# uw-x/AcousticSwarms-Speech

Hardware: AMD Instinct MI355X
Metric: TDoA candidates/sec (shift+normalise+spot forward+energies) (higher is better)
Workload: dtype f32 via f16x3 split-operand MFMA (fp32 accumulate); 1 GPU; configs[2] scene: 5-speaker reverberant mixture (image sources), 7 mics, T=48000 samples (BASELINE's '3 s @ 16 kHz' sample count; the reference pipeline and this scene generator run at 48 kHz, where it is a 1 s clip -- the reference-native 3 s is extras.T144000), fine-stage (Strict=1) candidate batch of one mixture, FULL spot net 47.27 M params, seeded random weights; internal_batch=256, parallelism=candidate-shard x1

## Files before the change

### acousticswarms-speech_amd/csrc/asw_common.cpp

```cpp
#include "asw_common.h"

#include <cmath>
#include <cstdlib>

namespace asw {
char* err_buf() {
  static thread_local char buf[512] = {0};
  return buf;
}
int set_error(int code, const char* fmt, ...) {
  va_list ap;
  va_start(ap, fmt);
  vsnprintf(err_buf(), 512, fmt, ap);
  va_end(ap);
  return code;
}
int SmemAttr::ensure(const void* kern, size_t want) {
  int dev = 0;
  ASW_HIP(hipGetDevice(&dev));
  if (dev < 0 || dev >= kMaxDev) return set_error(ASW_ERR_ARG, "device ordinal %d out of range", dev);
  if (bytes[dev] >= want) return ASW_OK;
  ASW_HIP(hipFuncSetAttribute(kern, hipFuncAttributeMaxDynamicSharedMemorySize, (int)want));
  bytes[dev] = want;
  return ASW_OK;
}
}

extern "C" const char* asw_last_error(void) { return asw::err_buf(); }
extern "C" int asw_abi_version(void) { return 3; }

extern "C" int asw_split_weights_f16(const float* w, size_t n, uint16_t* hi, uint16_t* lo, int32_t* w_shift) {
  ASW_CHECK_ARG(w && hi && lo && w_shift, "split_weights: null pointer");
  float mx = 0.f;
  for (size_t i = 0; i < n; ++i) { const float a = w[i] < 0 ? -w[i] : w[i]; if (a > mx || a != a) mx = a; }
  ASW_CHECK_ARG(mx == mx && mx < 3.0e38f, "split_weights: non-finite weight");
  int shift = 0;
  if (mx > 0.f) {
    int e;
    (void)frexpf(mx, &e);
    shift = 11 - e;
    if (shift > 24) shift = 24;
    if (shift < -24) shift = -24;
  }
  const float sc = ldexpf(1.0f, shift);
  for (size_t i = 0; i < n; ++i) {
    float c = w[i] * sc;
    if (c > 65504.f) c = 65504.f;
    if (c < -65504.f) c = -65504.f;
    const _Float16 h = (_Float16)c;
    const _Float16 l = (_Float16)(c - (float)h);
    memcpy(hi + i, &h, 2);
    memcpy(lo + i, &l, 2);
  }
  *w_shift = shift;
  return ASW_OK;
}

extern "C" int asw_pack_fragments_f16(const float* Wt, int N, int K, uint16_t* hi, uint16_t* lo, int32_t* w_shift) {
  ASW_CHECK_ARG(Wt && hi && lo && w_shift, "pack_fragments: null pointer");
  ASW_CHECK_ARG(N > 0 && K > 0 && N % 32 == 0 && K % 16 == 0, "pack_fragments: N %% 32, K %% 16 required (N=%d K=%d)", N, K);
  const size_t n = (size_t)N * K;
  uint16_t* th = new uint16_t[2 * n];
  uint16_t* tl = th + n;
  int rc = asw_split_weights_f16(Wt, n, th, tl, w_shift);
  if (rc == ASW_OK) {
    const int NT = N / 32;
    for (int ks = 0; ks < K / 16; ++ks)
      for (int nt = 0; nt < NT; ++nt)
        for (int l = 0; l < 64; ++l) {
          const size_t src = (size_t)(nt * 32 + (l & 31)) * K + ks * 16 + 8 * (l >> 5);
          const size_t dst = (((size_t)ks * NT + nt) * 64 + l) * 8;
          memcpy(hi + dst, th + src, 16);
          memcpy(lo + dst, tl + src, 16);
        }
  }
  delete[] th;
  return rc;
}

namespace asw {
bool residue_feed_on() {
  static const bool off = getenv("ASW_NO_RESIDUE_FEED") != nullptr;
  return !off;
}
}

extern "C" int asw_residue_schedule(int taps, int stride, int dil, int pad, int Cin, int BK, int BM, int m0, int has_skip,
                                    asw_residue_stage* out, int cap, int* n_stages, int* max_shift) {
  ASW_CHECK_ARG(n_stages != nullptr && cap >= 0 && (out != nullptr || cap == 0), "residue_schedule: null pointer");
  ASW_CHECK_ARG(taps > 0 && stride > 0 && dil > 0 && Cin > 0 && BK > 0 && BM > 0, "residue_schedule: bad dims");
  *n_stages = 0;
  if (max_shift) *max_shift = 0;
  if (!asw::residue_feed_applies(taps, stride, dil, Cin, BK, has_skip != 0)) return ASW_OK;
  const asw::ResidueFeed rf{taps, stride, Cin / BK};
  ASW_CHECK_ARG(rf.ntaps(0) <= ASW_RESIDUE_MAX_TAPS, "residue_schedule: %d taps on one image, at most %d", rf.ntaps(0),
                ASW_RESIDUE_MAX_TAPS);
  *n_stages = rf.stages();
  if (max_shift) *max_shift = rf.shifts(0);
  for (int s = 0; s < rf.stages() && s < cap; ++s) {
    asw_residue_stage& d = out[s];
    memset(&d, 0, sizeof d);
    d.residue = s / rf.cpb;
    d.chunk = s - d.residue * rf.cpb;
    d.rows = BM + rf.shifts(d.residue);
    d.first_row = m0 * stride - pad + d.residue;
    d.ntaps = rf.ntaps(d.residue);
    for (int q = 0; q < d.ntaps; ++q) {
      d.tap[q] = rf.tap(d.residue, q);
      d.shift[q] = q;
      d.kstep[q] = rf.kstep(d.tap[q], d.chunk, BK / 16);
    }
  }
  return ASW_OK;
}

#include <map>
#include <mutex>
#include <vector>
namespace asw {
namespace {
struct Rec { std::string name; double work, bytes; hipEvent_t e0, e1; };
std::mutex g_mu;
bool g_on = false;
bool g_detail = false;
std::vector<Rec> g_recs;
std::vector<hipEvent_t> g_pool;
hipEvent_t take_event() {
  if (!g_pool.empty()) { hipEvent_t e = g_pool.back(); g_pool.pop_back(); return e; }
  hipEvent_t e = nullptr;
  (void)hipEventCreate(&e);
  return e;
}
}

std::string prof_name(const char* base, int bm, int bn, int bk, bool ln, bool stats) {
  char b[96];
  snprintf(b, sizeof b, "%s<%d,%d,%d,%s>", base, bm, bn, bk, ln ? "ln" : stats ? "stats" : "plain");
  return b;
}
bool prof_detail() { return g_detail; }
ProfScope::ProfScope(hipStream_t s, const std::string& name, double work, double bytes) : slot(-1), stream(s) {
  if (!g_on) return;
  std::lock_guard<std::mutex> lk(g_mu);
  Rec r{name, work, bytes, take_event(), take_event()};
  (void)hipEventRecord(r.e0, s);
  g_recs.push_back(r);
  slot = (int)g_recs.size() - 1;
}
ProfScope::~ProfScope() {
  if (slot < 0) return;
  std::lock_guard<std::mutex> lk(g_mu);
  if (slot < (int)g_recs.size()) (void)hipEventRecord(g_recs[slot].e1, stream);
}
}

extern "C" int asw_profile_enable(int on) {
  std::lock_guard<std::mutex> lk(asw::g_mu);
  for (auto& r : asw::g_recs) { asw::g_pool.push_back(r.e0); asw::g_pool.push_back(r.e1); }
  asw::g_recs.clear();
  asw::g_on = on != 0;
  asw::g_detail = on == 2;
  return ASW_OK;
}

extern "C" int asw_profile_report(char* buf, size_t cap) {
  if (!buf || cap < 64) return asw::set_error(ASW_ERR_ARG, "profile_report: buffer too small");
  std::lock_guard<std::mutex> lk(asw::g_mu);
  struct Agg { long n = 0; double ms = 0, work = 0, bytes = 0; };
  std::map<std::string, Agg> agg;
  for (auto& r : asw::g_recs) {
    if (hipEventSynchronize(r.e1) != hipSuccess) continue;
    float ms = 0.f;
    if (hipEventElapsedTime(&ms, r.e0, r.e1) != hipSuccess) continue;
    Agg& a = agg[r.name];
    a.n += 1; a.ms += ms; a.work += r.work; a.bytes += r.bytes;
  }
  size_t off = 0;
  off += snprintf(buf + off, cap - off, "{");
  bool first = true;
  for (auto& kv : agg) {
    if (off + 256 >= cap) break;
    off += snprintf(buf + off, cap - off, "%s\"%s\":{\"launches\":%ld,\"ms\":%.6f,\"work\":%.6e,\"bytes\":%.6e}", first ? "" : ",",
                    kv.first.c_str(), kv.second.n, kv.second.ms, kv.second.work, kv.second.bytes);
    first = false;
  }
  snprintf(buf + off, cap - off, "}");
  return ASW_OK;
}
```

### acousticswarms-speech_amd/csrc/model_common.h

```cpp
#pragma once
#include <cstdlib>
#include <iterator>
#include <map>
#include <memory>
#include <string>
#include <vector>

#include "asw_common.h"

namespace asw_model {

struct DevBuf {
  float* p = nullptr;
  size_t n = 0;
  DevBuf() = default;
  DevBuf(const DevBuf&) = delete;
  DevBuf& operator=(const DevBuf&) = delete;
  DevBuf(DevBuf&& o) noexcept : p(o.p), n(o.n) { o.p = nullptr; o.n = 0; }
  ~DevBuf() { if (p) (void)hipFree(p); }
  int upload(const std::vector<float>& h) {
    if (p) { (void)hipFree(p); p = nullptr; }
    n = h.size();
    if (hipMalloc(&p, n * sizeof(float)) != hipSuccess) return asw::set_error(ASW_ERR_NOMEM, "hipMalloc(%zu floats)", n);
    ASW_HIP(hipMemcpy(p, h.data(), n * sizeof(float), hipMemcpyHostToDevice));
    return ASW_OK;
  }
};

struct WBuf {
  DevBuf f32;
  uint16_t* hi = nullptr;
  uint16_t* lo = nullptr;
  int32_t shift = 0;
  WBuf() = default;
  WBuf(const WBuf&) = delete;
  WBuf& operator=(const WBuf&) = delete;
  WBuf(WBuf&& o) noexcept : f32(std::move(o.f32)), hi(o.hi), lo(o.lo), shift(o.shift), fhi(o.fhi), flo(o.flo) {
    o.hi = o.lo = o.fhi = o.flo = nullptr;
  }
  ~WBuf() {
    if (hi) (void)hipFree(hi);
    if (lo) (void)hipFree(lo);
    if (fhi) (void)hipFree(fhi);
    if (flo) (void)hipFree(flo);
  }
  int upload_gemm(const std::vector<float>& h, int N, int K) {
    int rc = upload(h);
    if (rc) return rc;
    if (N % 32 == 0 && K % 16 == 0 && (size_t)N * K == h.size()) return upload_frags(h, N, K);
    return ASW_OK;
  }
  int upload(const std::vector<float>& h) {
    int rc = f32.upload(h);
    if (rc) return rc;
    std::vector<uint16_t> vh(h.size()), vl(h.size());
    if ((rc = asw_split_weights_f16(h.data(), h.size(), vh.data(), vl.data(), &shift))) return rc;
    if (hi) { (void)hipFree(hi); hi = nullptr; }
    if (lo) { (void)hipFree(lo); lo = nullptr; }
    if (hipMalloc(&hi, h.size() * 2) != hipSuccess || hipMalloc(&lo, h.size() * 2) != hipSuccess)
      return asw::set_error(ASW_ERR_NOMEM, "hipMalloc(%zu halves)", h.size());
    ASW_HIP(hipMemcpy(hi, vh.data(), h.size() * 2, hipMemcpyHostToDevice));
    ASW_HIP(hipMemcpy(lo, vl.data(), h.size() * 2, hipMemcpyHostToDevice));
    return ASW_OK;
  }
  uint16_t* fhi = nullptr;
  uint16_t* flo = nullptr;
  int upload_frags(const std::vector<float>& h, int N, int K) {
    std::vector<uint16_t> vh(h.size()), vl(h.size());
    int32_t sh = 0;
    int rc = asw_pack_fragments_f16(h.data(), N, K, vh.data(), vl.data(), &sh);
    if (rc) return rc;
    if (sh != shift) return asw::set_error(ASW_ERR_STATE, "fragment pack: inconsistent weight shift");
    if (fhi) { (void)hipFree(fhi); fhi = nullptr; }
    if (flo) { (void)hipFree(flo); flo = nullptr; }
    if (hipMalloc(&fhi, h.size() * 2) != hipSuccess || hipMalloc(&flo, h.size() * 2) != hipSuccess)
      return asw::set_error(ASW_ERR_NOMEM, "hipMalloc(%zu halves)", h.size());
    ASW_HIP(hipMemcpy(fhi, vh.data(), h.size() * 2, hipMemcpyHostToDevice));
    ASW_HIP(hipMemcpy(flo, vl.data(), h.size() * 2, hipMemcpyHostToDevice));
    return ASW_OK;
  }
  void bind(asw_convgemm_args& a, int precision) const {
    a.Wt = f32.p; a.Wt_hi = hi; a.Wt_lo = lo; a.w_shift = shift; a.precision = precision;
    a.Wf_hi = fhi; a.Wf_lo = flo;
  }
};

struct ResLayer { WBuf wt; DevBuf bias, g, b; int dil = 1; };

inline std::vector<float> pack_conv(const std::vector<float>& w, int N, int Cin, int K, const float* in_gate) {
  std::vector<float> o((size_t)N * Cin * K);
  for (int n = 0; n < N; ++n)
    for (int c = 0; c < Cin; ++c)
      for (int k = 0; k < K; ++k)
        o[((size_t)n * K + k) * Cin + c] = w[((size_t)n * Cin + c) * K + k] * (in_gate ? in_gate[c] : 1.f);
  return o;
}


inline int pack_res_layers(const std::map<std::string, std::vector<float>>& raw, const std::string& p, int ch, int K,
                           int n_layers, int dil_factor, std::vector<ResLayer>& out) {
  out.clear();
  out.resize(n_layers);
  int dil = 1;
  for (int j = 0; j < n_layers; ++j) {
    const std::string q = p + ".res.seq." + std::to_string(j);
    int rc;
    {
      const std::vector<float> packed = pack_conv(raw.at(q + ".conv.weight"), ch, ch, K, nullptr);
      if ((rc = out[j].wt.upload(packed))) return rc;
      if (ch % 32 == 0 && (ch * K) % 16 == 0 && (rc = out[j].wt.upload_frags(packed, ch, ch * K))) return rc;
    }
    if ((rc = out[j].bias.upload(raw.at(q + ".conv.bias")))) return rc;
    if ((rc = out[j].g.upload(raw.at(q + ".norm.weight")))) return rc;
    if ((rc = out[j].b.upload(raw.at(q + ".norm.bias")))) return rc;
    out[j].dil = dil;
    dil *= dil_factor;
  }
  return ASW_OK;
}

struct Arena {
  char* base;
  size_t off = 0, cap;
  bool dry;
  Arena(char* b, size_t c, bool d) : base(b), cap(c), dry(d) {}
  template <typename T>
  T* take(size_t n) {
    off = (off + 255) & ~(size_t)255;
    T* p = reinterpret_cast<T*>(base + off);
    off += n * sizeof(T);
    return p;
  }
};


struct GluSrc { const float* raw; const float* mr; const float* gamma; const float* beta; float* side_out = nullptr; };

inline bool glu_on_load_ok(const std::vector<ResLayer>& res, int prec, int ch) {
  static const int max_c = getenv("ASW_GLU_ON_LOAD_MAX_C") ? atoi(getenv("ASW_GLU_ON_LOAD_MAX_C")) : 512;
  return prec >= 1 && (ch == 64 || ch == 128 || ch == 256 || ch == 512) && ch <= max_c && !res.empty() &&
         res[0].dil == 1 && res[0].wt.fhi && res[0].wt.flo;
}

inline bool resstack_ok(const std::vector<ResLayer>& res, int prec, int ch, int K) {
  static const bool off = getenv("ASW_NO_RESSTACK") != nullptr;
  if (off || prec < 1 || ch != 64 || K % 2 == 0 || K < 3 || K > 15) return false;
  for (const ResLayer& r : res)
    if (!r.wt.fhi || !r.wt.flo) return false;
  return true;
}

inline size_t resstack_fuse_count(const std::vector<ResLayer>& res, size_t j, int K) {
  static const bool nofuse = getenv("ASW_RESSTACK_NOFUSE") != nullptr;
  size_t n = 1;
  int halo = 0;
  while (!nofuse && j + n < res.size() && n < 3) {
    const int pad = res[j + n].dil * (K - 1) / 2;
    if (halo + pad > 64) break;
    halo += pad;
    ++n;
  }
  return n;
}

struct SrcFeed { const void* hi; const void* lo; const WBuf* comp; const WBuf* pre; };

inline int run_res(const std::vector<ResLayer>& res, int prec, int B, int T, int ch, int K, float* x, float* p, float* q,
            float** final_out, hipStream_t s, const GluSrc* glu = nullptr, const SrcFeed* feed = nullptr) {
  const float* in = glu ? glu->raw : x;
  float* outb = p;
  if (feed && !(resstack_ok(res, prec, ch, K) && prec == 1 && resstack_fuse_count(res, 0, K) == 2))
    return asw::set_error(ASW_ERR_STATE, "run_res: the source-fed form needs the fused f16x3 pair");
  if (resstack_ok(res, prec, ch, K)) {
    size_t j = 0;
    while (j < res.size()) {
      const size_t n = resstack_fuse_count(res, j, K);
      asw_resstack_args a = {};
      a.x = ((glu || feed) && j == 0) ? nullptr : in;
      a.out = outb;
      a.B = B; a.T = T; a.C = ch; a.taps = K; a.n_layers = (int)n; a.precision = prec; a.ln_eps = 1e-5f;
      for (size_t i = 0; i < n; ++i) {
        const ResLayer& r = res[j + i];
        a.layer[i].Wf_hi = r.wt.fhi; a.layer[i].Wf_lo = r.wt.flo; a.layer[i].w_shift = r.wt.shift;
        a.layer[i].bias = r.bias.p; a.layer[i].ln_gamma = r.g.p; a.layer[i].ln_beta = r.b.p; a.layer[i].dil = r.dil;
      }
      if (glu && j == 0) {
        a.glu_raw = glu->raw; a.glu_mr = glu->mr; a.glu_gamma = glu->gamma; a.glu_beta = glu->beta; a.glu_out = glu->side_out;
      }
      if (feed && j == 0) {
        a.src_hi = feed->hi; a.src_lo = feed->lo;
        a.layer[0].Wf_hi = feed->comp->fhi; a.layer[0].Wf_lo = feed->comp->flo; a.layer[0].w_shift = feed->comp->shift;
        a.pre_hi = feed->pre->fhi; a.pre_lo = feed->pre->flo; a.pre_shift = feed->pre->shift;
      }
      int rc = asw_resstack64_f16x3(&a, s);
      if (rc) return rc;
      in = outb;
      outb = (outb == p) ? q : p;
      j += n;
    }
    *final_out = const_cast<float*>(in);
    return ASW_OK;
  }
  for (size_t j = 0; j < res.size(); ++j) {
    asw_convgemm_args a = {};
    a.A = in; res[j].wt.bind(a, prec); a.bias = res[j].bias.p; a.resid = in;
    if (glu && j == 0) {
      a.glu_raw = glu->raw; a.glu_mr = glu->mr; a.glu_gamma = glu->gamma; a.glu_beta = glu->beta; a.glu_out = glu->side_out;
    }
    a.ln_gamma = res[j].g.p; a.ln_beta = res[j].b.p; a.out = outb;
    a.B = B; a.M_out = T; a.N = ch; a.Cin = ch; a.taps = K; a.stride = 1; a.dil = res[j].dil;
    a.pad = (res[j].dil * (K - 1) + 1) / 2;
    a.a_row_stride = ch; a.a_batch_stride = (int64_t)T * ch; a.a_len = (int64_t)T * ch;
    a.relu = 1; a.ln_eps = 1e-5f;
    int rc = asw_convgemm_f32(&a, s);
    if (rc) return rc;
    in = outb;
    outb = (outb == p) ? q : p;
  }
  *final_out = const_cast<float*>(in);
  return ASW_OK;
}

inline int linear(const float* A, const WBuf& W, int prec, const float* bias, int rows, int N, int K, int relu, const float* resid,
           const float* g, const float* b, float* out, hipStream_t s) {
  asw_convgemm_args a = {};
  a.A = A; W.bind(a, prec); a.bias = bias; a.resid = resid; a.ln_gamma = g; a.ln_beta = b; a.out = out;
  a.B = 1; a.M_out = rows; a.N = N; a.Cin = K; a.taps = 1; a.stride = 1; a.dil = 1; a.pad = 0;
  a.a_row_stride = K; a.a_batch_stride = (int64_t)rows * K; a.a_len = (int64_t)rows * K;
  a.relu = relu; a.ln_eps = 1e-5f;
  if (g && N >= 1024 && N % 256 == 0 && N <= 2048) {
    a.resid = nullptr; a.ln_gamma = nullptr; a.ln_beta = nullptr;
    int rc = asw_convgemm_f32(&a, s);
    if (rc) return rc;
    return asw_add_layernorm(out, resid, g, b, rows, N, 1e-5f, out, s);
  }
  return asw_convgemm_f32(&a, s);
}

inline void pack_conv_transpose(const std::vector<float>& w, const std::vector<float>& b, int Cin, int N, int S,
                                const float* out_gate, std::vector<float>& wt, std::vector<float>& bb) {
  wt.assign((size_t)S * N * Cin, 0.f);
  bb.assign((size_t)S * N, 0.f);
  for (int r = 0; r < S; ++r)
    for (int n = 0; n < N; ++n) {
      bb[(size_t)r * N + n] = out_gate ? b[n] * out_gate[n] : b[n];
      for (int c = 0; c < Cin; ++c) {
        const float v = w[((size_t)c * N + n) * S + r];
        wt[((size_t)r * N + n) * Cin + c] = out_gate ? v * out_gate[n] : v;
      }
    }
}


#define UP(buf, vec) if ((rc = (buf).upload(vec))) return rc

struct TrunkCfg {
  int n_mics, kernel_size, depth, stride_list[8], channels, growth, encoder_channels, encoder_kernel_size,
      encoder_stride, residual_layers, residual_dilation_factor, ffw_dim;
  template <class Cfg>
  static TrunkCfg of(const Cfg& c) {
    TrunkCfg t = {c.n_mics, c.kernel_size, c.depth, {}, c.channels, c.growth, c.encoder_channels,
                  c.encoder_kernel_size, c.encoder_stride, c.residual_layers, c.residual_dilation_factor, c.ffw_dim};
    for (int i = 0; i < 8; ++i) t.stride_list[i] = c.stride_list[i];
    return t;
  }
};

inline int check_trunk_config(const TrunkCfg& c, const char* who, const char* odd) {
  ASW_CHECK_ARG(c.depth >= 1 && c.depth <= 8, "%s: depth %d", who, c.depth);
  ASW_CHECK_ARG(c.n_mics >= 1 && c.n_mics <= 32, "%s: n_mics %d", who, c.n_mics);
  ASW_CHECK_ARG(c.channels % 64 == 0, "%s: channels=%d must be a multiple of 64 for the MFMA tiles", who, c.channels);
  ASW_CHECK_ARG(c.growth >= 1 && c.residual_layers >= 1, "%s: bad config", who);
  ASW_CHECK_ARG(c.kernel_size % 2 == 1, "%s: %s", who, odd);
  ASW_CHECK_ARG(c.encoder_channels % 128 == 0, "%s: encoder_channels must be a multiple of 128", who);
  ASW_CHECK_ARG(c.encoder_stride % 4 == 0 && c.encoder_kernel_size / 2 == c.encoder_stride && c.encoder_kernel_size <= 64,
                "%s: encoder kernel/stride %d/%d unsupported (the reference's trim [9:-8] assumes 33/16)", who,
                c.encoder_kernel_size, c.encoder_stride);
  ASW_CHECK_ARG(c.ffw_dim % 128 == 0, "%s: ffw_dim must be a multiple of 128", who);
  return ASW_OK;
}

struct EncBlock { std::vector<ResLayer> res; DevBuf bias, gn_g, gn_b; };
struct DecBlock { std::vector<ResLayer> res; DevBuf gn_g, gn_b; };
struct GatedConvs { std::vector<WBuf> down_wt, up_wt; std::vector<DevBuf> up_bias; };
struct Tap { const float* p; size_t numel; };
using ParamList = std::vector<std::pair<std::string, size_t>>;

struct TrunkPlan {
  int B, T, Tp, F, RL;
  std::vector<int> Tl;
  float *mean, *stdv, *refn;
  uint16_t *src_hi = nullptr, *src_lo = nullptr;
  std::vector<float*> X, Pb, Qb, raw_dn, raw_up, st_dn, st_up, mr_dn, mr_up;
  float *Y, *D, *ywave;
};

struct Trunk {
  TrunkCfg tc;
  std::map<std::string, std::vector<float>> raw;
  std::map<std::string, Tap> taps;
  bool finalized = false;
  int device = 0;
  int precision = 0;
  bool exact_raw = false;
  bool fuse_mask = true;
  bool want_src = false;
  bool src_stack = true;

  std::vector<int> enc_cin, enc_cout;
  std::vector<int> dec_cin, dec_cout, dec_stride;
  int stride_product = 1;

  DevBuf pre_w, pre_b;
  WBuf src_wt, src_pre;
  std::vector<EncBlock> enc;
  std::vector<DecBlock> dec;
  WBuf byp_wt, mask_wt, dec_wt;
  WBuf byp_wt48;
  DevBuf byp_b, mask_b;
  float out_bias = 0.f;
  int byp_k = 0;

  const std::vector<float>& P(const std::string& k) const { return raw.at(k); }

  enum class Src { Normed, Raw };
  int site(Src a) const { return !exact_raw ? precision : a == Src::Raw ? 0 : 3; }

  int init_shape(const TrunkCfg& c, const char* who) {
    tc = c;
    ASW_HIP(hipGetDevice(&device));
    int cin = c.channels, ch = c.channels;
    for (int i = 0; i < c.depth; ++i) {
      ASW_CHECK_ARG(c.stride_list[i] >= 1, "%s: stride", who);
      enc_cin.push_back(cin);
      enc_cout.push_back(ch);
      stride_product *= c.stride_list[i];
      cin = ch;
      ch *= c.growth;
    }
    dec_cin.assign(enc_cout.rbegin(), enc_cout.rend());
    dec_cout.assign(enc_cin.rbegin(), enc_cin.rend());
    dec_stride.assign(std::make_reverse_iterator(c.stride_list + c.depth), std::make_reverse_iterator(c.stride_list));
    return ASW_OK;
  }
  int check_level_widths(const char* who) const {
    for (int w : enc_cin) ASW_CHECK_ARG(w <= 512 && (w & (w - 1)) == 0, "%s: level width %d must be a power of two <= 512", who, w);
    return ASW_OK;
  }

  ParamList trunk_params() const {
    ParamList v;
    const size_t K = tc.kernel_size;
    v.push_back({"preproc.weight", (size_t)tc.channels * tc.n_mics});
    v.push_back({"preproc.bias", (size_t)tc.channels});
    auto res = [&](const std::string& p, size_t ch) {
      for (int j = 0; j < tc.residual_layers; ++j) {
        const std::string q = p + ".res.seq." + std::to_string(j);
        v.push_back({q + ".conv.weight", ch * ch * K});
        v.push_back({q + ".conv.bias", ch});
        v.push_back({q + ".norm.weight", ch});
        v.push_back({q + ".norm.bias", ch});
      }
    };
    for (int i = 0; i < tc.depth; ++i) {
      const std::string p = "encoder.module_list." + std::to_string(i);
      const size_t ci = enc_cin[i], co = enc_cout[i];
      res(p, ci);
      v.push_back({p + ".conv1.weight", 2 * co * ci * K});
      v.push_back({p + ".conv1.bias", 2 * co});
      v.push_back({p + ".norm1.weight", 2 * co});
      v.push_back({p + ".norm1.bias", 2 * co});
    }
    for (int i = 0; i < tc.depth; ++i) {
      const std::string p = "decoder.module_list." + std::to_string(i);
      const size_t ci = dec_cin[i], co = dec_cout[i], s = dec_stride[i];
      v.push_back({p + ".upsample.conv.weight", ci * 2 * co * s});
      v.push_back({p + ".upsample.conv.bias", 2 * co});
      v.push_back({p + ".norm1.weight", 2 * co});
      v.push_back({p + ".norm1.bias", 2 * co});
      res(p, co);
    }
    const size_t E = tc.encoder_channels, EK = tc.encoder_kernel_size;
    v.push_back({"reference_bypass.weight", E * EK});
    v.push_back({"reference_bypass.bias", E});
    v.push_back({"mask_encoder.weight", E * tc.channels * EK});
    v.push_back({"mask_encoder.bias", E});
    v.push_back({"output_decoder.weight", E * EK});
    v.push_back({"output_decoder.bias", 1});
    return v;
  }

  int finalize_trunk(const char* who, const ParamList& want) {
    {
      int dev = -1;
      ASW_HIP(hipGetDevice(&dev));
      if (dev != device)
        return asw::set_error(ASW_ERR_STATE, "%s: model was created on HIP device %d, current device is %d", who, device, dev);
    }
    for (const auto& kv : want) {
      auto it = raw.find(kv.first);
      if (it == raw.end()) return asw::set_error(ASW_ERR_STATE, "state dict is missing key %s", kv.first.c_str());
      if (it->second.size() != kv.second)
        return asw::set_error(ASW_ERR_ARG, "%s: %zu elements, expected %zu", kv.first.c_str(), it->second.size(), kv.second);
    }
    if (raw.size() != want.size())
      return asw::set_error(ASW_ERR_ARG, "state dict has %zu unexpected keys", raw.size() - want.size());
    int rc;
    const int K = tc.kernel_size, RL = tc.residual_layers, RD = tc.residual_dilation_factor;
    UP(pre_w, P("preproc.weight"));
    UP(pre_b, P("preproc.bias"));
    enc.clear(); enc.resize(tc.depth);
    dec.clear(); dec.resize(tc.depth);
    for (int i = 0; i < tc.depth; ++i) {
      const std::string p = "encoder.module_list." + std::to_string(i);
      if ((rc = pack_res_layers(raw, p, enc_cin[i], K, RL, RD, enc[i].res))) return rc;
      UP(enc[i].bias, P(p + ".conv1.bias"));
      UP(enc[i].gn_g, P(p + ".norm1.weight"));
      UP(enc[i].gn_b, P(p + ".norm1.bias"));
    }
    if (want_src && tc.channels == 64 && tc.n_mics <= 7 && K <= 7 && enc[0].res[0].wt.fhi) {
      std::vector<float> pre16((size_t)64 * 16), comp((size_t)64 * 64);
      if ((rc = asw_compose_source_weights(P("encoder.module_list.0.res.seq.0.conv.weight").data(), P("preproc.weight").data(),
                                           P("preproc.bias").data(), tc.n_mics, K, comp.data(), pre16.data())))
        return rc;
      if ((rc = src_wt.upload_gemm(comp, 64, 64))) return rc;
      if ((rc = src_pre.upload_gemm(pre16, 64, 16))) return rc;
    }
    for (int i = 0; i < tc.depth; ++i) {
      const std::string p = "decoder.module_list." + std::to_string(i);
      if ((rc = pack_res_layers(raw, p, dec_cout[i], K, RL, RD, dec[i].res))) return rc;
      UP(dec[i].gn_g, P(p + ".norm1.weight"));
      UP(dec[i].gn_b, P(p + ".norm1.bias"));
    }
    const int E = tc.encoder_channels, EK = tc.encoder_kernel_size;
    byp_k = ((EK + 31) / 32) * 32;
    {
      const std::vector<float>& w = P("reference_bypass.weight");
      std::vector<float> wt((size_t)E * byp_k, 0.f);
      for (int n = 0; n < E; ++n)
        for (int k = 0; k < EK; ++k) wt[(size_t)n * byp_k + k] = w[(size_t)n * EK + k];
      UP(byp_wt, wt);
      UP(byp_b, P("reference_bypass.bias"));
      if (E % 32 == 0 && EK <= 48) {
        std::vector<float> w48((size_t)E * 48, 0.f);
        for (int n = 0; n < E; ++n)
          for (int k = 0; k < EK; ++k) w48[(size_t)n * 48 + k] = w[(size_t)n * EK + k];
        if ((rc = byp_wt48.upload_gemm(w48, E, 48))) return rc;
      }
    }
    if ((rc = mask_wt.upload_gemm(pack_conv(P("mask_encoder.weight"), E, tc.channels, EK, nullptr), E, tc.channels * EK))) return rc;
    UP(mask_b, P("mask_encoder.bias"));
    {
      const std::vector<float>& w = P("output_decoder.weight");
      std::vector<float> wt((size_t)64 * E, 0.f);
      for (int j = 0; j < EK; ++j)
        for (int e = 0; e < E; ++e) wt[(size_t)j * E + e] = w[(size_t)e * EK + j];
      if ((rc = dec_wt.upload_gemm(wt, 64, E))) return rc;
      out_bias = P("output_decoder.bias")[0];
    }
    return ASW_OK;
  }

  template <class Gate>
  int pack_gated(GatedConvs& o, Gate gate) const {
    const int K = tc.kernel_size;
    int rc;
    o.down_wt.clear(); o.down_wt.resize(tc.depth);
    o.up_wt.clear(); o.up_wt.resize(tc.depth);
    o.up_bias.clear(); o.up_bias.resize(tc.depth);
    for (int i = 0; i < tc.depth; ++i) {
      const std::string p = "encoder.module_list." + std::to_string(i);
      const std::vector<float> g = gate(p);
      const int n = 2 * enc_cout[i], ci = enc_cin[i];
      if ((rc = o.down_wt[i].upload_gemm(pack_conv(P(p + ".conv1.weight"), n, ci, K, g.empty() ? nullptr : g.data()), n, ci * K)))
        return rc;
    }
    for (int j = 0; j < tc.depth; ++j) {
      const std::string p = "decoder.module_list." + std::to_string(j);
      const std::vector<float> g = gate(p);
      const int ci = dec_cin[j], co2 = 2 * dec_cout[j], s = dec_stride[j];
      std::vector<float> wt, bb;
      pack_conv_transpose(P(p + ".upsample.conv.weight"), P(p + ".upsample.conv.bias"), ci, co2, s,
                          g.empty() ? nullptr : g.data(), wt, bb);
      if ((rc = o.up_wt[j].upload_gemm(wt, s * co2, ci))) return rc;
      UP(o.up_bias[j], bb);
    }
    return ASW_OK;
  }

  bool fused_mask_path() const {
    return fuse_mask && precision >= 1 && tc.encoder_channels % 256 == 0 && tc.channels % 32 == 0 &&
           tc.encoder_kernel_size <= 48 && tc.encoder_stride % 4 == 0 && byp_wt48.fhi && dec_wt.fhi && mask_wt.fhi;
  }
  bool src_path() const {
    return want_src && src_stack && precision == 1 && src_wt.fhi && src_pre.fhi && !enc.empty() &&
           resstack_ok(enc[0].res, precision, enc_cin[0], tc.kernel_size) &&
           resstack_fuse_count(enc[0].res, 0, tc.kernel_size) == 2;
  }
  void layout_levels(int B, int T, Arena& a, TrunkPlan& pl) const {
    const int depth = tc.depth, EK = tc.encoder_kernel_size, ES = tc.encoder_stride;
    pl.B = B; pl.T = T;
    pl.Tp = ((T - 1) / stride_product + 1) * stride_product;
    pl.F = (pl.Tp + 2 * (EK / 2) - EK) / ES + 1;
    pl.RL = ((EK / 2 + pl.Tp + byp_k + 64) + 3) & ~3;
    pl.Tl.assign(depth + 1, pl.Tp);
    for (int i = 0; i < depth; ++i) pl.Tl[i + 1] = pl.Tl[i] / tc.stride_list[i];
    pl.mean = a.take<float>(B);
    pl.stdv = a.take<float>(B);
    pl.refn = a.take<float>((size_t)B * pl.RL);
    if (want_src) {
      pl.src_hi = a.take<uint16_t>((size_t)B * pl.Tp * 8);
      pl.src_lo = a.take<uint16_t>((size_t)B * pl.Tp * 8);
    }
    pl.X.resize(depth + 1); pl.Pb.resize(depth); pl.Qb.resize(depth);
    pl.raw_dn.resize(depth); pl.raw_up.resize(depth); pl.st_dn.resize(depth); pl.st_up.resize(depth);
    pl.mr_up.resize(depth); pl.mr_dn.resize(depth);
    for (int i = 0; i <= depth; ++i) {
      const int ch = i == 0 ? tc.channels : enc_cout[i - 1];
      pl.X[i] = a.take<float>((size_t)B * pl.Tl[i] * ch);
    }
    for (int i = 0; i < depth; ++i) {
      const size_t n = (size_t)B * pl.Tl[i] * enc_cin[i];
      pl.Pb[i] = a.take<float>(n);
      pl.Qb[i] = a.take<float>(n);
      pl.raw_dn[i] = a.take<float>((size_t)B * pl.Tl[i + 1] * 2 * enc_cout[i]);
      pl.st_dn[i] = a.take<float>((size_t)B * 4 * asw_convgemm_stats_tiles(pl.Tl[i + 1], 2 * enc_cout[i]));
      pl.mr_dn[i] = a.take<float>((size_t)B * 4);
    }
    for (int j = 0; j < depth; ++j) {
      const int lvl = depth - j;
      const int s = dec_stride[j], co2 = 2 * dec_cout[j];
      pl.raw_up[j] = a.take<float>((size_t)B * pl.Tl[lvl] * s * co2);
      pl.st_up[j] = a.take<float>((size_t)B * 4 * asw_convgemm_stats_tiles(pl.Tl[lvl], s * co2));
      pl.mr_up[j] = a.take<float>((size_t)B * 4);
    }
  }
  void layout_mask(Arena& a, TrunkPlan& pl) const {
    const int E = tc.encoder_channels;
    const bool fused = fused_mask_path();
    pl.Y = fused ? nullptr : a.take<float>((size_t)pl.B * pl.F * E);
    pl.D = a.take<float>((size_t)(fused ? E / 256 : 1) * pl.B * pl.F * 64);
    pl.ywave = a.take<float>((size_t)pl.B * pl.T);
  }

  int encode(TrunkPlan& pl, const GatedConvs& g, hipStream_t s, bool src0 = false) {
    const int B = pl.B, K = tc.kernel_size;
    taps.clear();
    if (!src0) taps["preproc"] = {pl.X[0], (size_t)B * pl.Tl[0] * tc.channels};
    int rc;
    GluSrc src = {};
    const SrcFeed feed = {pl.src_hi, pl.src_lo, &src_wt, &src_pre};
    bool glu = false;
    for (int i = 0; i < tc.depth; ++i) {
      float* r = nullptr;
      if ((rc = run_res(enc[i].res, precision, B, pl.Tl[i], enc_cin[i], K, pl.X[i], pl.Pb[i], pl.Qb[i], &r, s,
                        glu ? &src : nullptr, (src0 && i == 0) ? &feed : nullptr)))
        return rc;
      asw_convgemm_args a = {};
      a.A = r; g.down_wt[i].bind(a, precision); a.bias = enc[i].bias.p; a.out = pl.raw_dn[i]; a.stats = pl.st_dn[i];
      a.B = B; a.M_out = pl.Tl[i + 1]; a.N = 2 * enc_cout[i]; a.Cin = enc_cin[i]; a.taps = K;
      a.stride = tc.stride_list[i]; a.dil = 1; a.pad = K / 2;
      a.a_row_stride = a.Cin; a.a_batch_stride = (int64_t)pl.Tl[i] * a.Cin; a.a_len = a.a_batch_stride;
      a.chan_mod = a.N;
      if ((rc = asw_convgemm_f32(&a, s))) return rc;
      glu = fuse_mask && i + 1 < tc.depth && glu_on_load_ok(enc[i + 1].res, precision, enc_cout[i]);
      const int tiles = asw_convgemm_stats_tiles(a.M_out, a.N);
      if (glu) {
        if ((rc = asw_gn_finalize(pl.st_dn[i], tiles, B, pl.Tl[i + 1], enc_cout[i], 1e-5f, pl.mr_dn[i], s))) return rc;
        src = {pl.raw_dn[i], pl.mr_dn[i], enc[i].gn_g.p, enc[i].gn_b.p, pl.X[i + 1]};
      } else if ((rc = asw_gn_glu(pl.raw_dn[i], pl.st_dn[i], tiles, enc[i].gn_g.p, enc[i].gn_b.p, B, pl.Tl[i + 1],
                                  enc_cout[i], 1e-5f, pl.X[i + 1], s))) {
        return rc;
      }
      taps["enc" + std::to_string(i)] = {pl.X[i + 1], (size_t)B * pl.Tl[i + 1] * enc_cout[i]};
    }
    return ASW_OK;
  }

  int decode(TrunkPlan& pl, const GatedConvs& g, const float*& x, hipStream_t s) {
    const int B = pl.B, K = tc.kernel_size;
    int rc;
    for (int j = 0; j < tc.depth; ++j) {
      const int lvl = tc.depth - j, ci = dec_cin[j], co = dec_cout[j], st = dec_stride[j];
      asw_convgemm_args a = {};
      a.A = x; a.A2 = pl.X[lvl]; g.up_wt[j].bind(a, precision); a.bias = g.up_bias[j].p; a.out = pl.raw_up[j];
      a.stats = pl.st_up[j];
      a.B = B; a.M_out = pl.Tl[lvl]; a.N = st * 2 * co; a.Cin = ci; a.taps = 1; a.stride = 1; a.dil = 1; a.pad = 0;
      a.a_row_stride = ci; a.a_batch_stride = (int64_t)pl.Tl[lvl] * ci; a.a_len = a.a_batch_stride;
      a.chan_mod = 2 * co;
      if ((rc = asw_convgemm_f32(&a, s))) return rc;
      const int To = pl.Tl[lvl] * st;
      const int tiles = asw_convgemm_stats_tiles(a.M_out, a.N);
      float* gb = pl.Qb[lvl - 1];
      float* r = nullptr;
      if (fuse_mask && glu_on_load_ok(dec[j].res, precision, co)) {
        if ((rc = asw_gn_finalize(pl.st_up[j], tiles, B, To, co, 1e-5f, pl.mr_up[j], s))) return rc;
        const GluSrc src = {pl.raw_up[j], pl.mr_up[j], dec[j].gn_g.p, dec[j].gn_b.p, co > 64 ? gb : nullptr};
        if ((rc = run_res(dec[j].res, precision, B, To, co, K, gb, pl.Pb[lvl - 1], gb, &r, s, &src))) return rc;
      } else {
        if ((rc = asw_gn_glu(pl.raw_up[j], pl.st_up[j], tiles, dec[j].gn_g.p, dec[j].gn_b.p, B, To, co, 1e-5f, gb, s)))
          return rc;
        if ((rc = run_res(dec[j].res, precision, B, To, co, K, gb, pl.Pb[lvl - 1], gb, &r, s))) return rc;
      }
      x = r;
      taps["dec" + std::to_string(j)] = {x, (size_t)B * To * co};
    }
    return ASW_OK;
  }

  int mask_path(TrunkPlan& pl, const float* x, const float* mean, const float* stdv, float* out_wave, hipStream_t s) {
    const int B = pl.B, C = tc.channels, E = tc.encoder_channels, EK = tc.encoder_kernel_size, ES = tc.encoder_stride;
    int rc;
    asw_convgemm_args me = {};
    me.A = x; mask_wt.bind(me, site(Src::Normed)); me.bias = mask_b.p;
    me.B = B; me.M_out = pl.F; me.N = E; me.Cin = C; me.taps = EK; me.stride = ES; me.dil = 1; me.pad = EK / 2;
    me.a_row_stride = C; me.a_batch_stride = (int64_t)pl.Tp * C; me.a_len = me.a_batch_stride;
    if (fused_mask_path()) {
      asw_maskpath_args f = {};
      f.enc = me;
      f.ref = pl.refn; f.ref_batch_stride = pl.RL; f.ref_len = pl.RL; f.ref_hop = ES;
      f.byp_k = 48; f.byp_taps = EK; f.byp_shift = byp_wt48.shift; f.byp_hi = byp_wt48.fhi; f.byp_lo = byp_wt48.flo;
      f.byp_bias = byp_b.p;
      f.dec_hi = dec_wt.fhi; f.dec_lo = dec_wt.flo; f.dec_shift = dec_wt.shift; f.dec_taps = EK;
      f.taps = pl.D;
      f.enc.precision = precision;
      if ((rc = exact_raw ? asw_mask_path_f16x3_scaled(&f, s) : asw_mask_path_f16x3(&f, s))) return rc;
      return asw_overlap_add_parts(pl.D, E / 256, B, pl.F, 64, EK, EK / 2, pl.T, 9, 8, out_bias, mean, stdv, out_wave, s);
    }
    {
      asw_convgemm_args a = {};
      a.A = pl.refn; byp_wt.bind(a, site(Src::Normed)); a.bias = byp_b.p; a.out = pl.Y;
      a.B = B; a.M_out = pl.F; a.N = E; a.Cin = byp_k; a.taps = 1; a.stride = 1; a.dil = 1; a.pad = 0;
      a.a_row_stride = ES; a.a_batch_stride = pl.RL; a.a_len = pl.RL; a.relu = 1;
      if ((rc = asw_convgemm_f32(&a, s))) return rc;
    }
    me.mul = pl.Y; me.out = pl.Y; me.relu = 1;
    if ((rc = asw_convgemm_f32(&me, s))) return rc;
    taps["latent"] = {pl.Y, (size_t)B * pl.F * E};
    {
      asw_convgemm_args a = {};
      a.A = pl.Y; dec_wt.bind(a, site(Src::Raw)); a.out = pl.D;
      a.B = B; a.M_out = pl.F; a.N = 64; a.Cin = E; a.taps = 1; a.stride = 1; a.dil = 1; a.pad = 0;
      a.a_row_stride = E; a.a_batch_stride = (int64_t)pl.F * E; a.a_len = a.a_batch_stride;
      if ((rc = asw_convgemm_f32(&a, s))) return rc;
    }
    return asw_overlap_add_unnorm(pl.D, B, pl.F, 64, EK, EK / 2, pl.T, 9, 8, out_bias, mean, stdv, out_wave, s);
  }
};

struct PostNormLayer { WBuf w_in, w_out, w1, w2; DevBuf b_in, b_out, b1, b2, n1g, n1b, n2g, n2b; };
struct PostNormBufs { float *qkv, *ctx, *x1, *ff; };

template <class Attention>
int run_post_norm(const Trunk& m, const PostNormLayer& t, const PostNormBufs& b, const float* x, float* out, int rows, int d,
                  int ffw, Attention&& attention, hipStream_t s) {
  const int normed = m.site(Trunk::Src::Normed), rawp = m.site(Trunk::Src::Raw);
  int rc;
  if ((rc = linear(x, t.w_in, normed, t.b_in.p, rows, 3 * d, d, 0, nullptr, nullptr, nullptr, b.qkv, s))) return rc;
  if ((rc = attention(b.qkv, b.ctx))) return rc;
  if ((rc = linear(b.ctx, t.w_out, rawp, t.b_out.p, rows, d, d, 0, x, t.n1g.p, t.n1b.p, b.x1, s))) return rc;
  if ((rc = linear(b.x1, t.w1, normed, t.b1.p, rows, ffw, d, 1, nullptr, nullptr, nullptr, b.ff, s))) return rc;
  return linear(b.ff, t.w2, rawp, t.b2.p, rows, d, ffw, 0, b.x1, t.n2g.p, t.n2b.p, out, s);
}

inline int check_ready(const Trunk* m, const char* fin) {
  if (!m) return asw::set_error(ASW_ERR_ARG, "null model handle");
  if (!m->finalized) return asw::set_error(ASW_ERR_STATE, "%s() has not been called", fin);
  int dev = -1;
  ASW_HIP(hipGetDevice(&dev));
  if (dev != m->device)
    return asw::set_error(ASW_ERR_STATE, "model lives on HIP device %d but the current device is %d", m->device, dev);
  return ASW_OK;
}

inline int set_precision(Trunk* m, const char* who, int precision) {
  ASW_CHECK_ARG(m && (precision >= 0 && precision <= 3), "%s: 0 (f32), 1 (f16x3), 2 (single-pass f16) or 3 (f16x3_safe)", who);
  m->exact_raw = precision == 3;
  m->precision = m->exact_raw ? 1 : precision;
  return ASW_OK;
}

inline int set_param(Trunk* m, const char* who, const char* key, const float* host_data, size_t numel) {
  ASW_CHECK_ARG(m && key && host_data, "%s: null pointer", who);
  m->raw[key].assign(host_data, host_data + numel);
  m->finalized = false;
  return ASW_OK;
}

inline int get_tap(const Trunk* m, const char* who, const char* name, float* dst, size_t capacity, size_t* numel,
                   void* stream) {
  ASW_CHECK_ARG(m && name && numel, "%s: null pointer", who);
  auto it = m->taps.find(name);
  if (it == m->taps.end()) return asw::set_error(ASW_ERR_ARG, "%s: no activation named %s", who, name);
  *numel = it->second.numel;
  if (dst) {
    ASW_CHECK_ARG(capacity >= it->second.numel, "%s: buffer too small", who);
    ASW_HIP(hipMemcpyAsync(dst, it->second.p, it->second.numel * sizeof(float), hipMemcpyDeviceToDevice,
                           asw::as_stream(stream)));
  }
  return ASW_OK;
}

}
```

### acousticswarms-speech_amd/csrc/resstack.hip

```cpp
#include <type_traits>

#include "asw_common.h"
#include "f16x3_tile.h"

namespace {
using namespace asw_mfma;

constexpr int C = 64;
constexpr int MAXL = 3;

struct LayerDev {
  const half8* Wh;
  const half8* Wl;
  const float* bias;
  const float* gamma;
  const float* beta;
  int dil, pad;
  int halo;
  int nfrag;
  float scale;
};

#ifdef ASW_PHASE_TIMING
__device__ unsigned long long g_rs_cycles[6] = {0, 0, 0, 0, 0, 0};
#define RS_MARK(var) const unsigned long long var = __builtin_readcyclecounter()
#else
#define RS_MARK(var)
#endif

struct KArgs {
  const float* x;
  float* out;
  const float* glu_raw;
  const float* glu_mr;
  const float* glu_gamma;
  const float* glu_beta;
  float* glu_out;
  const half8* src_h;
  const half8* src_l;
  const half8* Pre_h;
  const half8* Pre_l;
  float pre_up, pre_down;
  int B, T, taps, ntile, BM, img_rows;
  float eps;
  LayerDev L[MAXL];
};

__device__ __forceinline__ __amdgpu_buffer_rsrc_t src_rsrc(const half8* base, long rows) {
  return __builtin_amdgcn_make_buffer_rsrc(const_cast<half8*>(base), 0, (int)(rows * 16), 0x00020000);
}
__device__ __forceinline__ half8 src_load(__amdgpu_buffer_rsrc_t r, int row) {
  return __builtin_bit_cast(half8, __builtin_amdgcn_raw_buffer_load_b128(r, row >= 0 ? row * 16 : (int)0x80000000, 0, 0));
}

template <int NL, int NW, int TM, int PH, bool POLY, bool GLU, int NTERM, int QD, bool SRC = false>
__global__ __launch_bounds__(64 * NW) __attribute__((amdgpu_waves_per_eu(TM >= 4 ? 1 : 2)))
void resstack64_kernel(const KArgs p) {
  static_assert(!POLY || NL == 1, "polyphase row sets: single layers only");
  static_assert(!SRC || (!POLY && !GLU && NTERM == 3), "source-fed layer 0: contiguous tiles, f16x3");
  static_assert(QD == 2 || QD == 4, "weight prefetch depth in k-steps");
  constexpr int NTHR = 64 * NW, SROWS = NTHR / 16;
  constexpr int R0 = 32 * NW * TM;
  constexpr int BMJ = R0 / PH;
  static_assert(BMJ % 32 == 0, "a row fragment must stay inside one phase");

  extern __shared__ __align__(16) char smem[];
  char* img = smem;
  float* tab = reinterpret_cast<float*>(smem + (size_t)p.img_rows * RS);

  const int tid = threadIdx.x, lane = tid & 63, wid = tid >> 6;
  int idx;
  if (!xcd_tile_run(p.B * p.ntile, idx)) return;
  const int b = idx / p.ntile, tile = idx - b * p.ntile;
  const int T = p.T, taps = p.taps;
  const int dil0 = p.L[0].dil, pad0 = p.L[0].pad;
  const int n_pb = POLY ? (dil0 + PH - 1) / PH : 1;
  const int jb = POLY ? tile / n_pb : 0, pb = POLY ? tile - jb * n_pb : 0;
  const int m0 = tile * p.BM;
  const int RJ = BMJ + taps - 1;
  const int R_img = POLY ? PH * RJ : R0 + 2 * pad0;

  RS_MARK(t_start);
  if constexpr (!SRC) {
    for (int i = tid; i < NL * 3 * 16; i += NTHR) {
      const int li = i / 48, w = (i - li * 48) / 16, c4 = i & 15;
      const float* src = w == 0 ? p.L[li].bias : w == 1 ? p.L[li].gamma : p.L[li].beta;
      reinterpret_cast<float4*>(tab)[i] = *reinterpret_cast<const float4*>(src + c4 * 4);
    }
  }
  if constexpr (!SRC) {
    const __amdgpu_buffer_rsrc_t rX = GLU ? act_rsrc(p.glu_raw + (long)b * T * 2 * C, (long)T * 2 * C)
                                          : act_rsrc(p.x + (long)b * T * C, (long)T * C);
    const int srow = tid >> 4, sc4 = tid & 15;
    GluCoef gc;
    if (GLU) {
      gc.stats(p.glu_mr, b);
      gc.affine(p.glu_gamma, p.glu_beta, C, sc4 * 4);
    }
    constexpr int SU = GLU ? 9 : 18;
    for (int r0 = 0; r0 < R_img; r0 += SROWS * SU) {
      float4 buf[SU];
      float4 gate[GLU ? SU : 1];
      bool okr[GLU ? SU : 1];
#pragma unroll
      for (int u = 0; u < SU; ++u) {
        const int row = r0 + u * SROWS + srow;
        int g;
        bool ok = row < R_img;
        if (!POLY) {
          g = m0 - p.L[0].halo - pad0 + row;
        } else {
          const int ph = pb * PH + row / RJ;
          const int jj = jb * BMJ + row % RJ - (taps - 1) / 2;
          g = dil0 * jj + ph;
          ok = ok && ph < dil0 && jj >= 0;
        }
        ok = ok && g >= 0 && g < T;
        if (GLU) {
          buf[u] = act_load4(rX, (long)g * 2 * C + sc4 * 4, ok);
          gate[u] = act_load4(rX, (long)g * 2 * C + C + sc4 * 4, ok);
          okr[u] = ok;
        } else {
          buf[u] = act_load4(rX, (long)g * C + sc4 * 4, ok);
        }
      }
      if (GLU) {
#pragma unroll
        for (int u = 0; u < SU; ++u) {
          const float4 o = gn_glu4(buf[u], gate[u], gc, okr[u]);
          buf[u] = o;
          if (p.glu_out && okr[u]) {
            const int g = m0 - p.L[0].halo - pad0 + r0 + u * SROWS + srow;
            if (g >= m0 && g < m0 + p.BM)
              *reinterpret_cast<float4*>(p.glu_out + ((long)b * T + g) * C + sc4 * 4) = o;
          }
        }
      }
#pragma unroll
      for (int u = 0; u < SU; ++u) {
        const int row = r0 + u * SROWS + srow;
        if (row < R_img) {
          half4 hi, lo;
          split4t<NTERM>(buf[u], hi, lo);
          *reinterpret_cast<half4*>(img + row * RS + IMG_HI + sc4 * 8) = hi;
          *reinterpret_cast<half4*>(img + row * RS + IMG_LO + sc4 * 8) = lo;
        }
      }
    }
  }
  if constexpr (!SRC) __syncthreads();
  RS_MARK(t_staged);
#ifdef ASW_PHASE_TIMING
  unsigned long long t_marks[2 * MAXL + 1];
  t_marks[0] = t_staged;
#endif

  const int h = lane >> 5;
  floatx16 acc[TM][2];
  auto layer = [&](auto lic) {
    constexpr int li = decltype(lic)::value;
    constexpr bool last = li == NL - 1;
    const LayerDev& Ld = p.L[li];
    const int tapstep = (POLY ? 1 : Ld.dil) * RS;
    const int nf = Ld.nfrag - wid * TM;
#pragma unroll
    for (int i = 0; i < TM; ++i)
#pragma unroll
      for (int cb = 0; cb < 2; ++cb)
#pragma unroll
        for (int r = 0; r < 16; ++r) acc[i][cb][r] = 0.f;
    auto img_row = [&](int trow) { return POLY ? (trow / BMJ) * RJ + trow % BMJ : trow; };
    auto run = [&](auto nfc) {
      constexpr int NF = decltype(nfc)::value;
      int xb[NF];
      floatx16 a[NF][2];
#pragma unroll
      for (int i = 0; i < NF; ++i) {
        xb[i] = (img_row((wid * TM + i) * 32) + (lane & 31)) * RS + h * 16;
        a[i][0] = acc[i][0];
        a[i][1] = acc[i][1];
      }
      kloop<NF, 2, QD, NTERM>(
          a, taps, [&](int tap, int i) __attribute__((always_inline)) { return img + xb[i] + tap * tapstep; }, Ld.Wh, Ld.Wl,
          [](int kg, int cb) __attribute__((always_inline)) { return (long)kg * 2 + cb; }, lane);
#pragma unroll
      for (int i = 0; i < NF; ++i) { acc[i][0] = a[i][0]; acc[i][1] = a[i][1]; }
    };
    if constexpr (SRC && li == 0) {
      const __amdgpu_buffer_rsrc_t rH = src_rsrc(p.src_h + (long)b * T, T), rL = src_rsrc(p.src_l + (long)b * T, T);
      const int g0 = m0 - Ld.halo - Ld.pad + wid * TM * 32 + (lane & 31);
      half8 xh[4][TM], xl[4][TM], rh[TM], rl[TM];
#pragma unroll
      for (int ks = 0; ks < 4; ++ks)
#pragma unroll
        for (int i = 0; i < TM; ++i) {
          xh[ks][i] = src_load(rH, g0 + i * 32 + 2 * ks + h);
          xl[ks][i] = src_load(rL, g0 + i * 32 + 2 * ks + h);
        }
#pragma unroll
      for (int i = 0; i < TM; ++i) {
        rh[i] = src_load(rH, g0 + i * 32 + Ld.pad);
        rl[i] = src_load(rL, g0 + i * 32 + Ld.pad);
      }
      half8 wh[2][2], wl[2][2];
      auto wload = [&](auto kgc, int slot) {
        constexpr int kg = decltype(kgc)::value;
#pragma unroll
        for (int cb = 0; cb < 2; ++cb) {
          if constexpr (kg < 4) frag_load<3>(Ld.Wh, Ld.Wl, (long)kg * 2 + cb, lane, wh[slot][cb], wl[slot][cb]);
          else frag_load<3>(p.Pre_h, p.Pre_l, (long)cb, lane, wh[slot][cb], wl[slot][cb]);
        }
      };
      wload(std::integral_constant<int, 0>{}, 0);
      wload(std::integral_constant<int, 1>{}, 1);
      for (int i = tid; i < NL * 3 * 16; i += NTHR) {
        const int lj = i / 48, w = (i - lj * 48) / 16, c4 = i & 15;
        const float* src = w == 0 ? p.L[lj].bias : w == 1 ? p.L[lj].gamma : p.L[lj].beta;
        reinterpret_cast<float4*>(tab)[i] = *reinterpret_cast<const float4*>(src + c4 * 4);
      }
      __syncthreads();
      auto kstep = [&](auto ksc) {
        constexpr int ks = decltype(ksc)::value;
#pragma unroll
        for (int i = 0; i < TM; ++i)
#pragma unroll
          for (int cb = 0; cb < 2; ++cb) mma3<3, true>(acc[i][cb], xh[ks][i], xl[ks][i], wh[ks & 1][cb], wl[ks & 1][cb]);
        if constexpr (ks + 2 <= 4) wload(std::integral_constant<int, ks + 2>{}, ks & 1);
        __builtin_amdgcn_sched_barrier(0);
      };
      kstep(std::integral_constant<int, 0>{});
      kstep(std::integral_constant<int, 1>{});
      kstep(std::integral_constant<int, 2>{});
      kstep(std::integral_constant<int, 3>{});
      const float* tb0 = tab;
#pragma unroll
      for (int i = 0; i < TM; ++i) {
#pragma unroll
        for (int cb = 0; cb < 2; ++cb)
#pragma unroll
          for (int q = 0; q < 4; ++q) {
            const float4 bi = *reinterpret_cast<const float4*>(tb0 + cb * 32 + q * 8 + h * 4);
            const float bv[4] = {bi.x, bi.y, bi.z, bi.w};
#pragma unroll
            for (int j = 0; j < 4; ++j)
              acc[i][cb][q * 4 + j] = fmaxf(acc[i][cb][q * 4 + j] * Ld.scale + bv[j], 0.f) * p.pre_up;
          }
#pragma unroll
        for (int cb = 0; cb < 2; ++cb) mma3<3, true>(acc[i][cb], rh[i], rl[i], wh[0][cb], wl[0][cb]);
      }
    } else {
    if (nf >= TM) run(std::integral_constant<int, TM>{});
    else if constexpr (TM > 1) {
      if (nf == 1) run(std::integral_constant<int, 1>{});
      if constexpr (TM > 2) {
        if (nf == 2) run(std::integral_constant<int, 2>{});
        if (nf == 3) run(std::integral_constant<int, 3>{});
      }
    }
    }
#ifdef ASW_PHASE_TIMING
    {
      float sink = acc[0][0][0];
      asm volatile("" ::"v"(sink));
      t_marks[2 * li + 1] = __builtin_readcyclecounter();
    }
#endif
    const float* tb = tab + li * 192;
    const int cpad = POLY ? (taps - 1) / 2 : Ld.pad;
#pragma unroll
    for (int i = 0; i < TM; ++i) {
      if (i < nf) {
        const int trow = (wid * TM + i) * 32 + (lane & 31);
        const char* rrow = img + (img_row(trow) + cpad) * RS;
        float s = 0.f;
#pragma unroll
        for (int cb = 0; cb < 2; ++cb)
#pragma unroll
          for (int q = 0; q < 4; ++q) {
            const int c0 = cb * 32 + q * 8 + h * 4;
            const float4 bi = *reinterpret_cast<const float4*>(tb + c0);
            const half4 rh = *reinterpret_cast<const half4*>(rrow + IMG_HI + c0 * 2);
            const half4 rl = *reinterpret_cast<const half4*>(rrow + IMG_LO + c0 * 2);
            const float bv[4] = {bi.x, bi.y, bi.z, bi.w};
#pragma unroll
            for (int j = 0; j < 4; ++j) {
              float v;
              if constexpr (SRC && li == 0) {
                v = acc[i][cb][q * 4 + j] * p.pre_down;
              } else {
                v = fmaxf(acc[i][cb][q * 4 + j] * Ld.scale + bv[j], 0.f);
                v += (float)rh[j] + (float)rl[j];
              }
              acc[i][cb][q * 4 + j] = v;
              s += v;
            }
          }
        s += __shfl_xor(s, 32, 64);
        const float mean = s * (1.0f / C);
        float d = 0.f;
#pragma unroll
        for (int cb = 0; cb < 2; ++cb)
#pragma unroll
          for (int r = 0; r < 16; ++r) { const float cx = acc[i][cb][r] - mean; d += cx * cx; }
        d += __shfl_xor(d, 32, 64);
        const float rstd = 1.0f / sqrtf(d * (1.0f / C) + p.eps);
#pragma unroll
        for (int cb = 0; cb < 2; ++cb)
#pragma unroll
          for (int q = 0; q < 4; ++q) {
            const int c0 = cb * 32 + q * 8 + h * 4;
            const float4 g4 = *reinterpret_cast<const float4*>(tb + 64 + c0);
            const float4 b4 = *reinterpret_cast<const float4*>(tb + 128 + c0);
            const float gv[4] = {g4.x, g4.y, g4.z, g4.w}, be[4] = {b4.x, b4.y, b4.z, b4.w};
#pragma unroll
            for (int j = 0; j < 4; ++j) acc[i][cb][q * 4 + j] = (acc[i][cb][q * 4 + j] - mean) * rstd * gv[j] + be[j];
          }
      }
    }
    if constexpr (!last) {
      if constexpr (!(SRC && li == 0)) __syncthreads();
#pragma unroll
      for (int i = 0; i < TM; ++i) {
        if (i < nf) {
          const int trow = (wid * TM + i) * 32 + (lane & 31);
          const int t = m0 - Ld.halo + trow;
          const bool inside = t >= 0 && t < T;
          char* wrow = img + trow * RS;
#pragma unroll
          for (int cb = 0; cb < 2; ++cb)
#pragma unroll
            for (int q = 0; q < 4; ++q) {
              const int c0 = cb * 32 + q * 8 + h * 4;
              float4 v = make_float4(acc[i][cb][q * 4 + 0], acc[i][cb][q * 4 + 1], acc[i][cb][q * 4 + 2], acc[i][cb][q * 4 + 3]);
              if (!inside) v = make_float4(0.f, 0.f, 0.f, 0.f);
              half4 hi, lo;
              split4t<NTERM>(v, hi, lo);
              *reinterpret_cast<half4*>(wrow + IMG_HI + c0 * 2) = hi;
              *reinterpret_cast<half4*>(wrow + IMG_LO + c0 * 2) = lo;
            }
        }
      }
      __syncthreads();
    } else {
      float* __restrict__ ob = p.out + (long)b * T * C;
#pragma unroll
      for (int i = 0; i < TM; ++i) {
        if (i < nf) {
          const int trow = (wid * TM + i) * 32 + (lane & 31);
          int t;
          bool ok;
          if (!POLY) {
            t = m0 + trow;
            ok = trow < p.BM && t < T;
          } else {
            const int ph = pb * PH + trow / BMJ;
            t = dil0 * (jb * BMJ + trow % BMJ) + ph;
            ok = ph < dil0 && t < T;
          }
          if (ok) {
            float* orow = ob + (long)t * C;
#pragma unroll
            for (int cb = 0; cb < 2; ++cb)
#pragma unroll
              for (int q = 0; q < 4; ++q) {
                const int c0 = cb * 32 + q * 8 + h * 4;
                *reinterpret_cast<float4*>(orow + c0) =
                    make_float4(acc[i][cb][q * 4 + 0], acc[i][cb][q * 4 + 1], acc[i][cb][q * 4 + 2], acc[i][cb][q * 4 + 3]);
              }
          }
        }
      }
    }
  };
  layer(std::integral_constant<int, 0>{});
#ifdef ASW_PHASE_TIMING
  t_marks[2] = __builtin_readcyclecounter();
#endif
  if constexpr (NL > 1) layer(std::integral_constant<int, 1>{});
  if constexpr (NL > 2) layer(std::integral_constant<int, 2>{});
#ifdef ASW_PHASE_TIMING
  if (threadIdx.x == 0 && NL <= 2) {
    const unsigned long long t_end = __builtin_readcyclecounter();
    atomicAdd(&g_rs_cycles[0], t_staged - t_start);
    atomicAdd(&g_rs_cycles[1], t_marks[1] - t_marks[0]);
    if (NL == 1) {
      atomicAdd(&g_rs_cycles[4], t_end - t_marks[1]);
    } else {
      atomicAdd(&g_rs_cycles[2], t_marks[2] - t_marks[1]);
      atomicAdd(&g_rs_cycles[3], t_marks[3] - t_marks[2]);
      atomicAdd(&g_rs_cycles[4], t_end - t_marks[3]);
    }
    atomicAdd(&g_rs_cycles[5], 1ull);
  }
#endif
}

template <int NL, int NW, int TM, int PH, bool POLY, bool GLU, int QD, bool SRC = false>
int launch_stack(const KArgs& k, int precision, size_t smem, double flops, const char* tag, hipStream_t s) {
  char nm[128], detail[48] = "";
  snprintf(nm, sizeof nm, "resstack64<%s,%dx%d%s%s%s>", tag, NW, TM, POLY ? (PH == 1 ? ",poly1" : PH == 2 ? ",poly2" : ",poly4") : "",
           GLU ? ",glu" : "", SRC ? ",src" : "");
  if (asw::prof_detail()) snprintf(detail, sizeof detail, "[B%d M%d d%d]", k.B, k.T, k.L[0].dil);
  if constexpr (SRC) {
    return asw::launch_pair<resstack64_kernel<NL, NW, TM, PH, POLY, GLU, 3, QD, true>, resstack64_kernel<NL, NW, TM, PH, POLY, GLU, 3, QD, true>>(
        1, dim3(xcd_grid_run(k.B * k.ntile)), dim3(64 * NW), smem, 160 * 1024, nm, detail, flops,
        (double)k.B * k.T * (32 + C * 4), s, k);
  } else {
  return asw::launch_pair<resstack64_kernel<NL, NW, TM, PH, POLY, GLU, 1, QD>, resstack64_kernel<NL, NW, TM, PH, POLY, GLU, 3, QD>>(
      precision, dim3(xcd_grid_run(k.B * k.ntile)), dim3(64 * NW), smem, 160 * 1024, nm, detail, flops,
      (double)k.B * k.T * C * 4 * (GLU ? 3 : 2), s, k);
  }
}

template <int NW, int TM>
int dispatch(const asw_resstack_args& a, KArgs& k, bool glu, double flops, hipStream_t s) {
  constexpr int R0 = 32 * NW * TM;
  const int dil0 = k.L[0].dil;
  const int rpp = a.T / dil0;
  if (a.n_layers == 1 && dil0 >= 7 && rpp >= 48 && !glu) {
    const int PH = rpp >= R0 - 32 ? 1 : rpp >= R0 / 2 - 32 ? 2 : 4;
    const int BMJ = R0 / PH;
    k.BM = R0;
    k.L[0].nfrag = NW * TM;
    k.ntile = asw::cdiv(asw::cdiv(a.T, dil0), BMJ) * asw::cdiv(dil0, PH);
    k.img_rows = PH * (BMJ + a.taps - 1);
    const size_t smem = (size_t)k.img_rows * RS + 3 * 64 * sizeof(float);
    switch (PH) {
      case 1: return launch_stack<1, NW, TM, 1, true, false, 4>(k, a.precision, smem, flops, "1", s);
      case 2: return launch_stack<1, NW, TM, 2, true, false, 4>(k, a.precision, smem, flops, "1", s);
      default: return launch_stack<1, NW, TM, 4, true, false, 4>(k, a.precision, smem, flops, "1", s);
    }
  }
  k.BM = R0 - 2 * k.L[0].halo;
  ASW_CHECK_ARG(k.BM >= R0 / 2, "resstack: the later layers' halo (%d rows per side) leaves %d of %d rows; fuse fewer layers",
                k.L[0].halo, k.BM, R0);
  k.ntile = asw::cdiv(a.T, k.BM);
  int rows = 0;
  for (int i = 0; i < a.n_layers; ++i) {
    k.L[i].nfrag = asw::cdiv(k.BM + 2 * k.L[i].halo, 32);
    const int r = 32 * k.L[i].nfrag + 2 * k.L[i].pad;
    rows = r > rows ? r : rows;
  }
  k.img_rows = rows;
  const size_t smem = (size_t)rows * RS + (size_t)a.n_layers * 3 * 64 * sizeof(float);
  ASW_CHECK_ARG(smem <= 160 * 1024, "resstack: image of %d rows exceeds LDS (dilation %d x %d taps too wide for a contiguous tile)",
                rows, dil0, a.taps);
  if (k.src_h) {
    ASW_CHECK_ARG(k.L[0].nfrag == NW * TM, "resstack: source-fed layer 0 computes %d of %d fragments", k.L[0].nfrag, NW * TM);
    return launch_stack<2, NW, TM, 1, false, false, 4, true>(k, a.precision, smem, flops, "2", s);
  }
  switch (a.n_layers) {
    case 1: return glu ? launch_stack<1, NW, TM, 1, false, true, 4>(k, a.precision, smem, flops, "1", s)
                       : launch_stack<1, NW, TM, 1, false, false, 4>(k, a.precision, smem, flops, "1", s);
    case 2: return glu ? launch_stack<2, NW, TM, 1, false, true, 4>(k, a.precision, smem, flops, "2", s)
                       : launch_stack<2, NW, TM, 1, false, false, 4>(k, a.precision, smem, flops, "2", s);
    default: return glu ? launch_stack<3, NW, TM, 1, false, true, 4>(k, a.precision, smem, flops, "3", s)
                        : launch_stack<3, NW, TM, 1, false, false, 4>(k, a.precision, smem, flops, "3", s);
  }
}

}

#ifdef ASW_PHASE_TIMING
extern "C" int asw_debug_resstack_cycles(unsigned long long* out6, int reset) {
  ASW_HIP(hipMemcpyFromSymbol(out6, HIP_SYMBOL(g_rs_cycles), 6 * sizeof(unsigned long long)));
  if (reset) {
    const unsigned long long z[6] = {0, 0, 0, 0, 0, 0};
    ASW_HIP(hipMemcpyToSymbol(HIP_SYMBOL(g_rs_cycles), z, sizeof z));
  }
  return ASW_OK;
}
#endif

extern "C" int asw_compose_source_weights(const float* wc, const float* wpre, const float* bpre, int M, int taps, float* comp,
                                          float* pre16) {
  ASW_CHECK_ARG(wc && wpre && bpre && comp && pre16, "compose_source_weights: null pointer");
  ASW_CHECK_ARG(M >= 1 && M <= 7 && taps >= 1 && taps <= 7, "compose_source_weights: M=%d taps=%d (at most 7 each)", M, taps);
  for (int i = 0; i < C * 16; ++i) pre16[i] = 0.f;
  for (int i = 0; i < C * 64; ++i) comp[i] = 0.f;
  for (int c = 0; c < C; ++c) {
    for (int m = 0; m < M; ++m) pre16[c * 16 + m] = wpre[c * M + m];
    pre16[c * 16 + 7] = bpre[c];
  }
  for (int n = 0; n < C; ++n)
    for (int k = 0; k < taps; ++k)
      for (int j = 0; j < 8; ++j) {
        double acc = 0.0;
        for (int c = 0; c < C; ++c) acc += (double)wc[((size_t)n * C + c) * taps + k] * (double)pre16[c * 16 + j];
        comp[n * 64 + k * 8 + j] = (float)acc;
      }
  return ASW_OK;
}

extern "C" int asw_resstack64_f16x3(const asw_resstack_args* args, void* stream) {
  ASW_CHECK_ARG(args != nullptr, "resstack: null args");
  const asw_resstack_args& a = *args;
  hipStream_t s = asw::as_stream(stream);
  ASW_CHECK_ARG(a.C == C, "resstack: C=%d (64 only)", a.C);
  ASW_CHECK_ARG(a.n_layers >= 1 && a.n_layers <= MAXL, "resstack: 1..%d layers", MAXL);
  ASW_CHECK_ARG(a.taps >= 3 && a.taps <= 15 && a.taps % 2 == 1, "resstack: taps=%d (odd, 3..15)", a.taps);
  ASW_CHECK_ARG(a.precision == 1 || a.precision == 2, "resstack: precision 1 (f16x3) or 2 (single-pass f16)");
  ASW_CHECK_ARG(a.B > 0 && a.B <= (1 << 20) && a.T > 0 && (int64_t)a.T * 2 * C < ((int64_t)1 << 29), "resstack: bad B / T");
  ASW_CHECK_ARG(a.out && (a.x || a.glu_raw || a.src_hi), "resstack: null tensor");
  const bool glu = a.glu_raw != nullptr;
  if (glu) ASW_CHECK_ARG(a.glu_mr && a.glu_gamma && a.glu_beta, "resstack: GroupNorm + GLU on load needs the statistics / affine arrays");
  KArgs k = {};
  k.x = a.x; k.out = a.out; k.glu_raw = a.glu_raw; k.glu_mr = a.glu_mr; k.glu_gamma = a.glu_gamma; k.glu_beta = a.glu_beta;
  k.glu_out = glu ? a.glu_out : nullptr;
  k.B = a.B; k.T = a.T; k.taps = a.taps; k.eps = a.ln_eps;
  int halo = 0;
  for (int i = a.n_layers - 1; i >= 0; --i) {
    const asw_reslayer_desc& d = a.layer[i];
    ASW_CHECK_ARG(d.Wf_hi && d.Wf_lo && d.bias && d.ln_gamma && d.ln_beta && d.dil >= 1, "resstack: layer %d incomplete", i);
    LayerDev& L = k.L[i];
    L.Wh = reinterpret_cast<const half8*>(d.Wf_hi); L.Wl = reinterpret_cast<const half8*>(d.Wf_lo);
    L.bias = d.bias; L.gamma = d.ln_gamma; L.beta = d.ln_beta;
    L.dil = d.dil; L.pad = d.dil * (a.taps - 1) / 2; L.halo = halo;
    L.scale = ldexpf(1.0f, -d.w_shift);
    halo += L.pad;
  }
  double flops = 2.0 * a.B * (double)a.T * C * C * a.taps * a.n_layers;
  if (a.src_hi) {
    ASW_CHECK_ARG(a.src_lo && a.pre_hi && a.pre_lo && !a.x && !glu, "resstack: the source-fed form takes src_hi / src_lo / pre_hi / pre_lo and no x");
    ASW_CHECK_ARG(a.precision == 1 && a.n_layers == 2 && a.taps <= 7 && a.layer[0].dil == 1,
                  "resstack: source-fed layer 0 is f16x3, two layers, dilation 1, at most 7 taps");
    k.src_h = reinterpret_cast<const half8*>(a.src_hi); k.src_l = reinterpret_cast<const half8*>(a.src_lo);
    k.Pre_h = reinterpret_cast<const half8*>(a.pre_hi); k.Pre_l = reinterpret_cast<const half8*>(a.pre_lo);
    k.pre_up = ldexpf(1.0f, a.pre_shift); k.pre_down = ldexpf(1.0f, -a.pre_shift);
    flops = 2.0 * a.B * (double)a.T * C * (64 + 16 + C * a.taps);
  }
  return dispatch<4, 2>(a, k, glu, flops, s);
}
```

### acousticswarms-speech_amd/csrc/spot_model.hip

```cpp
#include <map>
#include <memory>
#include <string>
#include <vector>

#include "model_common.h"

using namespace asw_model;

namespace {

struct GateSet : GatedConvs { uint64_t stamp = 0; };

}

struct asw_spot : Trunk {
  asw_spot_config cfg;
  int batch = 32;
  uint64_t clock = 0;
  std::vector<PostNormLayer> tf;
  std::map<std::pair<float, float>, std::unique_ptr<GateSet>> gates;

  char* ws[2] = {nullptr, nullptr};
  size_t ws_bytes[2] = {0, 0};
  int lanes = 1;
  hipStream_t side = nullptr;
  hipEvent_t ev_fork = nullptr, ev_join = nullptr;

  asw_spot() { want_src = true; }
  ~asw_spot() {
    for (char* w : ws) if (w) (void)hipFree(w);
    if (side) (void)hipStreamDestroy(side);
    if (ev_fork) (void)hipEventDestroy(ev_fork);
    if (ev_join) (void)hipEventDestroy(ev_join);
  }
};

namespace {

ParamList expected_params(const asw_spot* m) {
  const asw_spot_config& c = m->cfg;
  ParamList v = m->trunk_params();
  for (int i = 0; i < c.depth; ++i) {
    const std::string p = "encoder.module_list." + std::to_string(i);
    v.push_back({p + ".embed1.weight", (size_t)m->enc_cin[i] * 2});
    v.push_back({p + ".embed1.bias", (size_t)m->enc_cin[i]});
  }
  for (int i = 0; i < c.depth; ++i) {
    const std::string p = "decoder.module_list." + std::to_string(i);
    v.push_back({p + ".embed1.weight", (size_t)2 * m->dec_cout[i] * 2});
    v.push_back({p + ".embed1.bias", (size_t)2 * m->dec_cout[i]});
  }
  const size_t d = m->enc_cout.back(), f = c.ffw_dim;
  for (int l = 0; l < c.num_transformer_layers; ++l) {
    const std::string p = "bottleneck.transf.layers." + std::to_string(l);
    v.push_back({p + ".self_attn.in_proj_weight", 3 * d * d});
    v.push_back({p + ".self_attn.in_proj_bias", 3 * d});
    v.push_back({p + ".self_attn.out_proj.weight", d * d});
    v.push_back({p + ".self_attn.out_proj.bias", d});
    v.push_back({p + ".linear1.weight", f * d});
    v.push_back({p + ".linear1.bias", f});
    v.push_back({p + ".linear2.weight", d * f});
    v.push_back({p + ".linear2.bias", d});
    v.push_back({p + ".norm1.weight", d});
    v.push_back({p + ".norm1.bias", d});
    v.push_back({p + ".norm2.weight", d});
    v.push_back({p + ".norm2.bias", d});
  }
  return v;
}

std::vector<float> gate_of(const std::vector<float>& w, const std::vector<float>& b, float w0, float w1) {
  std::vector<float> g(b.size());
  for (size_t c = 0; c < b.size(); ++c) g[c] = w[2 * c] * w0 + w[2 * c + 1] * w1 + b[c];
  return g;
}

int get_gates(asw_spot* m, float w0, float w1, GateSet** out) {
  auto key = std::make_pair(w0, w1);
  auto it = m->gates.find(key);
  if (it != m->gates.end()) { it->second->stamp = ++m->clock; *out = it->second.get(); return ASW_OK; }
  if (m->gates.size() >= 8) {
    auto lru = m->gates.begin();
    for (auto g = m->gates.begin(); g != m->gates.end(); ++g)
      if (g->second->stamp < lru->second->stamp) lru = g;
    m->gates.erase(lru);
  }
  std::unique_ptr<GateSet> gs(new GateSet());
  gs->stamp = ++m->clock;
  int rc = m->pack_gated(*gs, [&](const std::string& p) {
    return gate_of(m->P(p + ".embed1.weight"), m->P(p + ".embed1.bias"), w0, w1);
  });
  if (rc) return rc;
  *out = gs.get();
  m->gates[key] = std::move(gs);
  return ASW_OK;
}

struct Plan : TrunkPlan {
  float *qkv, *ctx, *x1, *ff, *ha, *hb;
};

void layout(const asw_spot* m, int B, int T, Arena& a, Plan& pl) {
  m->layout_levels(B, T, a, pl);
  const size_t L = pl.Tl[m->cfg.depth], d = m->enc_cout.back(), rows = (size_t)B * L;
  pl.qkv = a.take<float>(rows * 3 * d);
  pl.ctx = a.take<float>(rows * d);
  pl.x1 = a.take<float>(rows * d);
  pl.ff = a.take<float>(rows * m->cfg.ffw_dim);
  pl.ha = a.take<float>(rows * d);
  pl.hb = a.take<float>(rows * d);
  m->layout_mask(a, pl);
}

int ensure_ws(asw_spot* m, int B, int T, Plan& pl, int lane = 0) {
  Arena dry(nullptr, 0, true);
  layout(m, B, T, dry, pl);
  const size_t need = dry.off + 4096;
  if (need > m->ws_bytes[lane]) {
    size_t want = need;
    if (B < m->batch) {
      Plan full;
      Arena dry_full(nullptr, 0, true);
      layout(m, m->batch, T, dry_full, full);
      want = dry_full.off + 4096;
    }
    if (m->ws[lane]) { ASW_HIP(hipDeviceSynchronize()); (void)hipFree(m->ws[lane]); m->ws[lane] = nullptr; m->ws_bytes[lane] = 0; }
    if (hipMalloc(&m->ws[lane], want) != hipSuccess) {
      (void)hipGetLastError();
      want = need;
      if (hipMalloc(&m->ws[lane], want) != hipSuccess)
        return asw::set_error(ASW_ERR_NOMEM, "workspace of %.1f MiB for batch %d, T=%d", need / 1048576.0, B, T);
    }
    m->ws_bytes[lane] = want;
  }
  Arena real(m->ws[lane], m->ws_bytes[lane], false);
  layout(m, B, T, real, pl);
  return ASW_OK;
}

int run_network(asw_spot* m, Plan& pl, GateSet* gs, const float* mean, const float* stdv, float* out_wave,
                hipStream_t s, bool src0 = false) {
  const asw_spot_config& c = m->cfg;
  int rc;
  if ((rc = m->encode(pl, *gs, s, src0))) return rc;
  const int L = pl.Tl[c.depth], d = m->enc_cout.back(), rows = pl.B * L;
  const float* h = pl.X[c.depth];
  const int rawp = m->site(Trunk::Src::Raw);
  auto attention = [&](const float* qkv, float* ctx) { return asw_attention_prec(qkv, pl.B, L, d, c.num_head, rawp, ctx, s); };
  for (int l = 0; l < c.num_transformer_layers; ++l) {
    float* hout = (l % 2 == 0) ? pl.ha : pl.hb;
    if ((rc = run_post_norm(*m, m->tf[l], {pl.qkv, pl.ctx, pl.x1, pl.ff}, h, hout, rows, d, c.ffw_dim, attention, s))) return rc;
    h = hout;
  }
  m->taps["bottleneck"] = {h, (size_t)rows * d};
  if ((rc = m->decode(pl, *gs, h, s))) return rc;
  return m->mask_path(pl, h, mean, stdv, out_wave, s);
}

}

extern "C" int asw_spot_create(const asw_spot_config* cfg, asw_spot** out) {
  ASW_CHECK_ARG(cfg && out, "spot_create: null pointer");
  const asw_spot_config& c = *cfg;
  const TrunkCfg tc = TrunkCfg::of(c);
  int rc = check_trunk_config(tc, "spot_create", "kernel_size must be odd");
  if (rc) return rc;
  ASW_CHECK_ARG(c.num_transformer_layers >= 0, "spot_create: bad config");
  std::unique_ptr<asw_spot> m(new asw_spot());
  m->cfg = c;
  if ((rc = m->init_shape(tc, "spot_create"))) return rc;
  const int d = m->enc_cout.back();
  ASW_CHECK_ARG(d <= 1024 && (d & (d - 1)) == 0, "spot_create: bottleneck width %d must be a power of two <= 1024", d);
  ASW_CHECK_ARG(d % c.num_head == 0 && (d / c.num_head) % 16 == 0 && d / c.num_head <= 128,
                "spot_create: head_dim %d unsupported", d / (c.num_head ? c.num_head : 1));
  if ((rc = m->check_level_widths("spot_create"))) return rc;
  *out = m.release();
  return ASW_OK;
}

extern "C" void asw_spot_destroy(asw_spot* m) { delete m; }

extern "C" int asw_spot_set_precision(asw_spot* m, int precision) { return set_precision(m, "set_precision", precision); }

extern "C" int asw_spot_set_batch(asw_spot* m, int batch) {
  ASW_CHECK_ARG(m && batch >= 1 && batch <= 4096, "set_batch: bad argument");
  m->batch = batch;
  return ASW_OK;
}

extern "C" int asw_spot_set_param(asw_spot* m, const char* key, const float* host_data, size_t numel) {
  return set_param(m, "set_param", key, host_data, numel);
}

extern "C" int asw_spot_finalize(asw_spot* m) {
  ASW_CHECK_ARG(m, "finalize: null handle");
  const asw_spot_config& c = m->cfg;
  int rc = m->finalize_trunk("finalize", expected_params(m));
  if (rc) return rc;
  m->tf.clear(); m->tf.resize(c.num_transformer_layers);
  for (int l = 0; l < c.num_transformer_layers; ++l) {
    const std::string p = "bottleneck.transf.layers." + std::to_string(l);
    PostNormLayer& t = m->tf[l];
    {
      const int dm = m->enc_cout.back(), ff = c.ffw_dim;
      if ((rc = t.w_in.upload_gemm(m->P(p + ".self_attn.in_proj_weight"), 3 * dm, dm))) return rc;
      if ((rc = t.w_out.upload_gemm(m->P(p + ".self_attn.out_proj.weight"), dm, dm))) return rc;
      if ((rc = t.w1.upload_gemm(m->P(p + ".linear1.weight"), ff, dm))) return rc;
      if ((rc = t.w2.upload_gemm(m->P(p + ".linear2.weight"), dm, ff))) return rc;
    }
    UP(t.b_in, m->P(p + ".self_attn.in_proj_bias"));
    UP(t.b_out, m->P(p + ".self_attn.out_proj.bias"));
    UP(t.b1, m->P(p + ".linear1.bias"));
    UP(t.b2, m->P(p + ".linear2.bias"));
    UP(t.n1g, m->P(p + ".norm1.weight")); UP(t.n1b, m->P(p + ".norm1.bias"));
    UP(t.n2g, m->P(p + ".norm2.weight")); UP(t.n2b, m->P(p + ".norm2.bias"));
  }
  m->gates.clear();
  m->finalized = true;
  return ASW_OK;
}

extern "C" int asw_spot_shift_and_sep(asw_spot* m, const float* mix, int M, int T, const int32_t* offsets, int N,
                                      int strict, int circular, float* out_wave, double* out_energy,
                                      int energy_window, void* stream) {
  return asw_spot_shift_and_sep_multi(m, mix, 1, M, T, offsets, nullptr, N, strict, circular, out_wave, out_energy,
                                      energy_window, stream);
}

extern "C" int asw_spot_shift_and_sep_multi(asw_spot* m, const float* mix, int K, int M, int T, const int32_t* offsets,
                                            const int32_t* mix_index, int N, int strict, int circular, float* out_wave,
                                            double* out_energy, int energy_window, void* stream) {
  int rc = check_ready(m, "asw_spot_finalize");
  ASW_CHECK_ARG(K >= 1 && (K == 1 || mix_index != nullptr), "shift_and_sep: K=%d mixtures need a mix_index array", K);
  if (rc) return rc;
  ASW_CHECK_ARG(N >= 0, "shift_and_sep: N=%d", N);
  if (N == 0) return ASW_OK;
  ASW_CHECK_ARG(mix && offsets, "shift_and_sep: null pointer");
  ASW_CHECK_ARG(M == m->cfg.n_mics, "shift_and_sep: mixture has %d channels, model expects %d", M, m->cfg.n_mics);
  ASW_CHECK_ARG(T >= 2, "shift_and_sep: T=%d", T);
  ASW_CHECK_ARG(out_energy == nullptr || energy_window > 0, "shift_and_sep: energy_window");
  hipStream_t s = asw::as_stream(stream);
  GateSet* gs = nullptr;
  if ((rc = get_gates(m, strict == 1 ? 1.f : 0.f, strict == 1 ? 0.f : 1.f, &gs))) return rc;
  const int Bmax = N < m->batch ? N : m->batch;
  const int n_batches = (N + Bmax - 1) / Bmax;
  const int lanes = (m->lanes == 2 && n_batches >= 2) ? 2 : 1;
  Plan pl[2];
  for (int l = 0; l < lanes; ++l)
    if ((rc = ensure_ws(m, Bmax, T, pl[l], l))) return rc;
  hipStream_t st[2] = {s, s};
  if (lanes == 2) {
    if (!m->side) {
      ASW_HIP(hipStreamCreateWithFlags(&m->side, hipStreamNonBlocking));
      ASW_HIP(hipEventCreateWithFlags(&m->ev_fork, hipEventDisableTiming));
      ASW_HIP(hipEventCreateWithFlags(&m->ev_join, hipEventDisableTiming));
    }
    st[1] = m->side;
    ASW_HIP(hipEventRecord(m->ev_fork, s));
    ASW_HIP(hipStreamWaitEvent(m->side, m->ev_fork, 0));
  }
  const int C = m->cfg.channels, pad_l = m->cfg.encoder_kernel_size / 2;
  const bool src0 = m->src_path();
  auto batches = [&]() -> int {
    int k = 0;
    for (int i0 = 0; i0 < N; i0 += Bmax, ++k) {
      const int B = N - i0 < Bmax ? N - i0 : Bmax;
      Plan& p = pl[k % lanes];
      hipStream_t q = st[k % lanes];
      p.B = B;
      const int32_t* off = offsets + (size_t)i0 * (M - 1);
      const int32_t* mi = mix_index ? mix_index + i0 : nullptr;
      ASW_HIP(hipMemsetAsync(p.refn, 0, (size_t)B * p.RL * sizeof(float), q));
      int r;
      if ((r = asw_shift_stats_multi(mix, M, T, off, mi, B, circular, p.mean, p.stdv, q))) return r;
      if (src0) {
        if ((r = asw_shift_norm_src_multi(mix, M, T, p.Tp, off, mi, B, circular, p.mean, p.stdv, p.src_hi, p.src_lo,
                                          p.refn + pad_l, p.RL, q)))
          return r;
      } else if ((r = asw_shift_norm_preproc_multi(mix, M, T, p.Tp, off, mi, B, circular, p.mean, p.stdv, m->pre_w.p,
                                                   m->pre_b.p, C, p.X[0], p.refn + pad_l, p.RL, q))) {
        return r;
      }
      float* y = out_wave ? out_wave + (size_t)i0 * T : p.ywave;
      if ((r = run_network(m, p, gs, p.mean, p.stdv, y, q, src0))) return r;
      if (out_energy && (r = asw_energies(y, B, T, energy_window, nullptr, out_energy + (size_t)i0 * 2, q))) return r;
    }
    return ASW_OK;
  };
  rc = batches();
  if (lanes == 2) {
    if (hipEventRecord(m->ev_join, m->side) != hipSuccess || hipStreamWaitEvent(s, m->ev_join, 0) != hipSuccess) {
      (void)hipStreamSynchronize(m->side);
      if (!rc) rc = asw::set_error(ASW_ERR_HIP, "shift_and_sep: joining the side lane failed");
    }
  }
  return rc;
}

extern "C" int asw_spot_set_lanes(asw_spot* m, int lanes) {
  ASW_CHECK_ARG(m && (lanes == 1 || lanes == 2), "set_lanes: 1 or 2");
  m->lanes = lanes;
  return ASW_OK;
}

extern "C" int asw_spot_forward(asw_spot* m, const float* mix_norm, int B, int M, int t,
                                const float* window_embedding_host, float* out, void* stream) {
  int rc = check_ready(m, "asw_spot_finalize");
  if (rc) return rc;
  ASW_CHECK_ARG(B >= 0, "forward: B=%d", B);
  if (B == 0) return ASW_OK;
  ASW_CHECK_ARG(mix_norm && window_embedding_host && out, "forward: null pointer");
  ASW_CHECK_ARG(M == m->cfg.n_mics && t >= 1, "forward: bad shape");
  hipStream_t s = asw::as_stream(stream);
  GateSet* gs = nullptr;
  if ((rc = get_gates(m, window_embedding_host[0], window_embedding_host[1], &gs))) return rc;
  const int Bmax = B < m->batch ? B : m->batch;
  Plan pl;
  if ((rc = ensure_ws(m, Bmax, t, pl))) return rc;
  const int C = m->cfg.channels, pad_l = m->cfg.encoder_kernel_size / 2;
  for (int i0 = 0; i0 < B; i0 += Bmax) {
    const int b = B - i0 < Bmax ? B - i0 : Bmax;
    pl.B = b;
    ASW_HIP(hipMemsetAsync(pl.refn, 0, (size_t)b * pl.RL * sizeof(float), s));
    if ((rc = asw_pad_preproc(mix_norm + (size_t)i0 * M * t, b, M, t, pl.Tp, m->pre_w.p, m->pre_b.p, C, pl.X[0],
                              pl.refn + pad_l, pl.RL, s)))
      return rc;
    if ((rc = run_network(m, pl, gs, nullptr, nullptr, out + (size_t)i0 * t, s))) return rc;
  }
  return ASW_OK;
}

extern "C" int asw_spot_set_fused_mask(asw_spot* m, int on) {
  ASW_CHECK_ARG(m, "set_fused_mask: null model handle");
  m->fuse_mask = on != 0;
  return ASW_OK;
}

extern "C" int asw_spot_set_source_stack(asw_spot* m, int on) {
  ASW_CHECK_ARG(m, "set_source_stack: null model handle");
  m->src_stack = on != 0;
  return ASW_OK;
}

extern "C" int asw_spot_get_tap(asw_spot* m, const char* name, float* dst, size_t capacity, size_t* numel,
                                void* stream) {
  return get_tap(m, "get_tap", name, dst, capacity, numel, stream);
}
```

### acousticswarms-speech_amd/native.py

```python
import ctypes
import glob
import os
import subprocess
import sys
from ctypes import (POINTER, Structure, c_char_p, c_double, c_float, c_int, c_int32, c_int64,
                    c_long, c_size_t, c_void_p)

_HERE = os.path.dirname(os.path.abspath(__file__))
LIB_PATH = os.environ.get("ASW_LIB_PATH") or os.path.join(_HERE, "libasw_hip.so")
CSRC = os.path.join(_HERE, "csrc")
SOURCES = ["asw_common.cpp", "convgemm.hip", "resconv.hip", "pipegemm.hip", "resstack.hip", "downconv.hip", "prep_kernels.hip",
           "misc_kernels.hip", "attention.hip", "srp_kernels.hip",
           "pruner_kernels.hip", "geometry_kernels.hip", "cluster_kernels.hip",
           "search_host.cpp", "sep_kernels.hip", "spot_model.hip", "sep_model.hip", "bss_kernels.hip"]
EXTRA_FLAGS = {"geometry_kernels.hip": ["-ffp-contract=off"], "cluster_kernels.hip": ["-ffp-contract=off"]}
OPS_PATH = os.path.join(_HERE, "libasw_torch_ops.so")
OPS_SOURCE = "torch_ops.cpp"


def build(force: bool = False, verbose: bool = False) -> str:
    from concurrent.futures import ThreadPoolExecutor
    hdrs = glob.glob(os.path.join(CSRC, "*.h")) + [os.path.join(os.path.dirname(_HERE), "include", "asw_hip.h")]
    hdr_time = max(os.path.getmtime(h) for h in hdrs)
    objdir = os.path.join(_HERE, "build")
    os.makedirs(objdir, exist_ok=True)
    jobs, objs = [], []
    for src in SOURCES:
        sp = os.path.join(CSRC, src)
        op = os.path.join(objdir, os.path.splitext(src)[0] + ".o")
        objs.append(op)
        if force or not os.path.exists(op) or os.path.getmtime(op) < max(os.path.getmtime(sp), hdr_time):
            jobs.append(["hipcc", "-O3", "--offload-arch=gfx950", "-std=c++17", "-fPIC"] + EXTRA_FLAGS.get(src, [])
                        + ["-c", sp, "-o", op])
    if not jobs and os.path.exists(LIB_PATH) and all(os.path.getmtime(LIB_PATH) >= os.path.getmtime(o) for o in objs):
        return LIB_PATH

    def run(cmd):
        if verbose:
            print(" ".join(cmd), file=sys.stderr)
        subprocess.run(cmd, check=True)
    with ThreadPoolExecutor(max_workers=min(6, max(1, len(jobs)))) as ex:
        list(ex.map(run, jobs))
    run(["hipcc", "--offload-arch=gfx950", "-fPIC", "-shared", "-o", LIB_PATH] + objs)
    return LIB_PATH


def build_torch_ops(force: bool = False, verbose: bool = False) -> str:
    import torch
    src = os.path.join(CSRC, OPS_SOURCE)
    hdr = os.path.join(os.path.dirname(_HERE), "include", "asw_hip.h")
    if not force and os.path.exists(OPS_PATH) and os.path.getmtime(OPS_PATH) >= max(
            os.path.getmtime(src), os.path.getmtime(hdr), os.path.getmtime(LIB_PATH)):
        return OPS_PATH
    ti = os.path.dirname(torch.__file__)
    cmd = ["hipcc", "-O2", "-std=c++17", "-fPIC", "-shared", "-D__HIP_PLATFORM_AMD__=1", "-DUSE_ROCM=1",
           f"-D_GLIBCXX_USE_CXX11_ABI={int(torch._C._GLIBCXX_USE_CXX11_ABI)}", "-w",
           f"-I{ti}/include", f"-I{ti}/include/torch/csrc/api/include", "-I/opt/rocm/include", src, "-o", OPS_PATH,
           f"-L{_HERE}", "-lasw_hip", f"-L{ti}/lib", "-ltorch", "-ltorch_cpu", "-lc10", "-lc10_hip", "-ltorch_hip",
           "-Wl,-rpath,$ORIGIN", f"-Wl,-rpath,{ti}/lib"]
    if verbose:
        print(" ".join(cmd), file=sys.stderr)
    subprocess.run(cmd, check=True)
    return OPS_PATH


class SpotConfigC(Structure):
    _fields_ = [("n_mics", c_int32), ("kernel_size", c_int32), ("depth", c_int32),
                ("stride_list", c_int32 * 8), ("channels", c_int32), ("growth", c_int32),
                ("encoder_channels", c_int32), ("encoder_kernel_size", c_int32),
                ("encoder_stride", c_int32), ("residual_layers", c_int32),
                ("residual_dilation_factor", c_int32), ("num_head", c_int32), ("ffw_dim", c_int32),
                ("num_transformer_layers", c_int32)]

    @classmethod
    def from_config(cls, cfg):
        s = cls()
        s.n_mics, s.kernel_size, s.depth = cfg.n_mics, cfg.kernel_size, cfg.depth
        for i, v in enumerate(cfg.stride_list):
            s.stride_list[i] = v
        s.channels, s.growth = cfg.channels, int(cfg.growth)
        s.encoder_channels, s.encoder_kernel_size = cfg.encoder_channels, cfg.encoder_kernel_size
        s.encoder_stride, s.residual_layers = cfg.encoder_stride, cfg.residual_layers
        s.residual_dilation_factor, s.num_head = cfg.residual_dilation_factor, cfg.num_head
        s.ffw_dim, s.num_transformer_layers = cfg.ffw_dim, cfg.num_transformer_layers
        return s


class SepConfigC(Structure):
    _fields_ = [("n_mics", c_int32), ("max_speakers", c_int32), ("kernel_size", c_int32), ("depth", c_int32),
                ("stride_list", c_int32 * 8), ("channels", c_int32), ("growth", c_int32),
                ("encoder_channels", c_int32), ("encoder_kernel_size", c_int32), ("encoder_stride", c_int32),
                ("residual_layers", c_int32), ("residual_dilation_factor", c_int32), ("num_head", c_int32),
                ("ffw_dim", c_int32), ("bottleneck_layers", c_int32), ("bottleneck_ksize", c_int32)]

    @classmethod
    def from_config(cls, cfg):
        s = cls()
        s.n_mics, s.max_speakers, s.kernel_size, s.depth = cfg.n_mics, cfg.max_speakers, cfg.kernel_size, cfg.depth
        for i, v in enumerate(cfg.stride_list):
            s.stride_list[i] = v
        s.channels, s.growth = cfg.channels, int(cfg.growth)
        s.encoder_channels, s.encoder_kernel_size = cfg.encoder_channels, cfg.encoder_kernel_size
        s.encoder_stride, s.residual_layers = cfg.encoder_stride, cfg.residual_layers
        s.residual_dilation_factor, s.num_head = cfg.residual_dilation_factor, cfg.num_head
        s.ffw_dim, s.bottleneck_layers, s.bottleneck_ksize = cfg.ffw_dim, cfg.bottleneck_layers, cfg.bottleneck_ksize
        return s


class ConvGemmArgs(Structure):
    _fields_ = [("A", c_void_p), ("A2", c_void_p), ("Wt", c_void_p), ("bias", c_void_p),
                ("resid", c_void_p), ("mul", c_void_p), ("ln_gamma", c_void_p), ("ln_beta", c_void_p),
                ("out", c_void_p), ("stats", c_void_p),
                ("B", c_int32), ("M_out", c_int32), ("N", c_int32), ("Cin", c_int32), ("taps", c_int32),
                ("stride", c_int32), ("dil", c_int32), ("pad", c_int32), ("a_row_stride", c_int32),
                ("a_batch_stride", c_int64), ("a_len", c_int64), ("chan_mod", c_int32), ("relu", c_int32),
                ("ln_eps", c_float), ("precision", c_int32), ("w_shift", c_int32), ("Wt_hi", c_void_p),
                ("Wt_lo", c_void_p), ("Wf_hi", c_void_p), ("Wf_lo", c_void_p), ("stats_stride", c_int32),
                ("glu_raw", c_void_p), ("glu_mr", c_void_p), ("glu_gamma", c_void_p), ("glu_beta", c_void_p),
                ("glu_out", c_void_p)]


class MaskPathArgs(Structure):
    _fields_ = [("enc", ConvGemmArgs), ("ref", c_void_p), ("ref_batch_stride", c_int64), ("ref_len", c_int64),
                ("ref_hop", c_int32), ("byp_k", c_int32), ("byp_taps", c_int32), ("byp_shift", c_int32),
                ("byp_hi", c_void_p), ("byp_lo", c_void_p), ("byp_bias", c_void_p), ("dec_hi", c_void_p),
                ("dec_lo", c_void_p), ("dec_shift", c_int32), ("dec_taps", c_int32), ("taps", c_void_p)]


class ResLayerDesc(Structure):
    _fields_ = [("Wf_hi", c_void_p), ("Wf_lo", c_void_p), ("bias", c_void_p), ("ln_gamma", c_void_p),
                ("ln_beta", c_void_p), ("dil", c_int32), ("w_shift", c_int32)]


class ResStackArgs(Structure):
    _fields_ = [("x", c_void_p), ("out", c_void_p), ("B", c_int32), ("T", c_int32), ("C", c_int32), ("taps", c_int32),
                ("n_layers", c_int32), ("precision", c_int32), ("ln_eps", c_float), ("layer", ResLayerDesc * 3),
                ("glu_raw", c_void_p), ("glu_mr", c_void_p), ("glu_gamma", c_void_p), ("glu_beta", c_void_p),
                ("glu_out", c_void_p), ("src_hi", c_void_p), ("src_lo", c_void_p), ("pre_hi", c_void_p), ("pre_lo", c_void_p),
                ("pre_shift", c_int32)]


RESIDUE_MAX_TAPS = 8


class ResidueStage(Structure):
    _fields_ = [("residue", c_int32), ("chunk", c_int32), ("rows", c_int32), ("first_row", c_int32), ("ntaps", c_int32),
                ("tap", c_int32 * RESIDUE_MAX_TAPS), ("shift", c_int32 * RESIDUE_MAX_TAPS),
                ("kstep", c_int32 * RESIDUE_MAX_TAPS)]


SIGNATURES = {
    "asw_last_error": (c_char_p, []),
    "asw_abi_version": (c_int, []),
    "asw_profile_enable": (c_int, [c_int]),
    "asw_profile_report": (c_int, [c_char_p, c_size_t]),
    "asw_spot_create": (c_int, [POINTER(SpotConfigC), POINTER(c_void_p)]),
    "asw_spot_destroy": (None, [c_void_p]),
    "asw_spot_set_param": (c_int, [c_void_p, c_char_p, c_void_p, c_size_t]),
    "asw_spot_finalize": (c_int, [c_void_p]),
    "asw_spot_set_batch": (c_int, [c_void_p, c_int]),
    "asw_spot_set_precision": (c_int, [c_void_p, c_int]),
    "asw_spot_set_lanes": (c_int, [c_void_p, c_int]),
    "asw_split_weights_f16": (c_int, [c_void_p, c_size_t, c_void_p, c_void_p, POINTER(c_int32)]),
    "asw_pack_fragments_f16": (c_int, [c_void_p, c_int, c_int, c_void_p, c_void_p, POINTER(c_int32)]),
    "asw_spot_shift_and_sep": (c_int, [c_void_p, c_void_p, c_int, c_int, c_void_p, c_int, c_int, c_int,
                                       c_void_p, c_void_p, c_int, c_void_p]),
    "asw_spot_shift_and_sep_multi": (c_int, [c_void_p, c_void_p, c_int, c_int, c_int, c_void_p, c_void_p, c_int, c_int, c_int,
                                             c_void_p, c_void_p, c_int, c_void_p]),
    "asw_spot_forward": (c_int, [c_void_p, c_void_p, c_int, c_int, c_int, POINTER(c_float), c_void_p, c_void_p]),
    "asw_spot_set_fused_mask": (c_int, [c_void_p, c_int]),
    "asw_spot_set_source_stack": (c_int, [c_void_p, c_int]),
    "asw_spot_get_tap": (c_int, [c_void_p, c_char_p, c_void_p, c_size_t, POINTER(c_size_t), c_void_p]),
    "asw_sep_create": (c_int, [POINTER(SepConfigC), POINTER(c_void_p)]),
    "asw_sep_destroy": (None, [c_void_p]),
    "asw_sep_set_param": (c_int, [c_void_p, c_char_p, c_void_p, c_size_t]),
    "asw_sep_finalize": (c_int, [c_void_p]),
    "asw_sep_set_precision": (c_int, [c_void_p, c_int]),
    "asw_sep_infer": (c_int, [c_void_p, c_void_p, c_int, c_int, c_void_p, c_int, c_void_p, c_void_p]),
    "asw_sep_infer_batch": (c_int, [c_void_p, c_void_p, c_int, c_int, c_int, c_void_p, c_void_p, c_void_p, c_void_p]),
    "asw_sep_forward": (c_int, [c_void_p, c_void_p, c_int, c_int, c_int, c_int, c_void_p, c_void_p]),
    "asw_sep_forward_counts": (c_int, [c_void_p, c_void_p, c_int, c_int, c_int, c_int, c_void_p, c_void_p, c_void_p]),
    "asw_sep_get_config": (c_int, [c_void_p, POINTER(SepConfigC)]),
    "asw_sep_get_tap": (c_int, [c_void_p, c_char_p, c_void_p, c_size_t, POINTER(c_size_t), c_void_p]),
    "asw_joint_shift_stats": (c_int, [c_void_p, c_int, c_int, c_void_p, c_int, c_void_p, c_void_p, c_void_p, c_void_p]),
    "asw_joint_shift_stats_scratch_doubles": (c_int, []),
    "asw_joint_shift_stats_groups": (c_int, [c_void_p, c_int, c_int, c_void_p, c_void_p, c_int, c_void_p, c_void_p, c_void_p,
                                             c_void_p, c_void_p]),
    "asw_add_layernorm2": (c_int, [c_void_p, c_void_p, c_float, c_void_p, c_void_p, c_int, c_int, c_float, c_int,
                                   c_void_p, c_void_p, c_void_p]),
    "asw_glu_rows": (c_int, [c_void_p, c_long, c_int, c_void_p, c_void_p]),
    "asw_dwconv_ln_swish": (c_int, [c_void_p, c_void_p, c_void_p, c_void_p, c_void_p, c_int, c_int, c_int, c_int,
                                    c_float, c_void_p, c_void_p]),
    "asw_relpos_attention": (c_int, [c_void_p, c_void_p, c_void_p, c_void_p, c_int, c_int, c_int, c_int, c_float,
                                     c_void_p, c_void_p]),
    "asw_inter_attention": (c_int, [c_void_p, c_int, c_int, c_int, c_int, c_int, c_void_p, c_void_p]),
    "asw_inter_attention_groups": (c_int, [c_void_p, c_void_p, c_int, c_int, c_int, c_int, c_void_p, c_void_p]),
    "asw_shift_stats": (c_int, [c_void_p, c_int, c_int, c_void_p, c_int, c_int, c_void_p, c_void_p, c_void_p]),
    "asw_shift_norm_preproc": (c_int, [c_void_p, c_int, c_int, c_int, c_void_p, c_int, c_int, c_void_p, c_void_p,
                                       c_void_p, c_void_p, c_int, c_void_p, c_void_p, c_long, c_void_p]),
    "asw_shift_stats_multi": (c_int, [c_void_p, c_int, c_int, c_void_p, c_void_p, c_int, c_int, c_void_p, c_void_p, c_void_p]),
    "asw_shift_norm_preproc_multi": (c_int, [c_void_p, c_int, c_int, c_int, c_void_p, c_void_p, c_int, c_int, c_void_p,
                                             c_void_p, c_void_p, c_void_p, c_int, c_void_p, c_void_p, c_long, c_void_p]),
    "asw_shift_norm_src_multi": (c_int, [c_void_p, c_int, c_int, c_int, c_void_p, c_void_p, c_int, c_int, c_void_p,
                                         c_void_p, c_void_p, c_void_p, c_void_p, c_long, c_void_p]),
    "asw_pad_preproc": (c_int, [c_void_p, c_int, c_int, c_int, c_int, c_void_p, c_void_p, c_int, c_void_p,
                                c_void_p, c_long, c_void_p]),
    "asw_convgemm_f32": (c_int, [POINTER(ConvGemmArgs), c_void_p]),
    "asw_mask_path_f16x3": (c_int, [POINTER(MaskPathArgs), c_void_p]),
    "asw_mask_path_f16x3_scaled": (c_int, [POINTER(MaskPathArgs), c_void_p]),
    "asw_resstack64_f16x3": (c_int, [POINTER(ResStackArgs), c_void_p]),
    "asw_compose_source_weights": (c_int, [c_void_p, c_void_p, c_void_p, c_int, c_int, c_void_p, c_void_p]),
    "asw_convgemm_stats_tiles": (c_int, [c_int, c_int]),
    "asw_f16x3_overflow_count": (c_int, [c_int, POINTER(c_int32)]),
    "asw_residue_schedule": (c_int, [c_int, c_int, c_int, c_int, c_int, c_int, c_int, c_int, c_int,
                                     POINTER(ResidueStage), c_int, POINTER(c_int), POINTER(c_int)]),
    "asw_gn_glu": (c_int, [c_void_p, c_void_p, c_int, c_void_p, c_void_p, c_int, c_int, c_int, c_float, c_void_p,
                           c_void_p]),
    "asw_gn_finalize": (c_int, [c_void_p, c_int, c_int, c_int, c_int, c_float, c_void_p, c_void_p]),
    "asw_attention": (c_int, [c_void_p, c_int, c_int, c_int, c_int, c_void_p, c_void_p]),
    "asw_attention_prec": (c_int, [c_void_p, c_int, c_int, c_int, c_int, c_int, c_void_p, c_void_p]),
    "asw_overlap_add_unnorm": (c_int, [c_void_p, c_int, c_int, c_int, c_int, c_int, c_int, c_int, c_int, c_float,
                                       c_void_p, c_void_p, c_void_p, c_void_p]),
    "asw_overlap_add_parts": (c_int, [c_void_p, c_int, c_int, c_int, c_int, c_int, c_int, c_int, c_int, c_int, c_float,
                                      c_void_p, c_void_p, c_void_p, c_void_p]),
    "asw_energies": (c_int, [c_void_p, c_int, c_int, c_int, c_void_p, c_void_p, c_void_p]),
    "asw_pair_sisdr": (c_int, [c_void_p, c_int, c_int, c_void_p, c_void_p]),
    "asw_center_rows": (c_int, [c_void_p, c_int, c_int, c_void_p]),
    "asw_segment_sisdr": (c_int, [c_void_p, c_int, c_int, c_void_p, c_void_p, c_int, c_void_p, c_void_p]),
    "asw_voiced_segments_workspace_bytes": (c_size_t, [c_int, c_int]),
    "asw_voiced_segments": (c_int, [c_void_p, c_int, c_int, c_double, c_double, c_void_p, c_int, c_void_p, c_void_p,
                                    c_void_p, c_size_t, c_void_p]),
    "asw_fine_clusters_workspace_bytes": (c_size_t, [c_void_p, c_int]),
    "asw_fine_clusters": (c_int, [c_void_p, c_int, c_int, c_void_p, c_int, c_void_p, c_void_p, c_void_p, c_double,
                                  c_double, c_void_p, c_size_t, c_void_p, c_void_p, c_void_p, c_void_p]),
    "asw_global_clusters_workspace_bytes": (c_size_t, [c_int]),
    "asw_global_clusters": (c_int, [c_void_p, c_void_p, c_void_p, c_void_p, c_int, c_int, c_double, c_double, c_double,
                                    c_double, c_double, c_void_p, c_size_t, c_void_p, c_void_p, c_void_p]),
    "asw_coarse_select_workspace_bytes": (c_size_t, [c_int, c_int]),
    "asw_coarse_select": (c_int, [c_void_p, c_void_p, c_void_p, c_int, c_double, c_int, c_double, c_int, c_void_p, c_size_t,
                                  c_void_p, c_void_p, c_void_p, c_void_p]),
    "asw_bss_eval_sdr_workspace_bytes": (c_size_t, [c_void_p, c_int, c_int, c_int, c_int]),
    "asw_bss_eval_sdr": (c_int, [c_void_p, c_void_p, c_void_p, c_int, c_int, c_int, c_int, c_void_p, c_void_p, c_void_p,
                                 c_size_t, c_void_p]),
    "asw_add_layernorm": (c_int, [c_void_p, c_void_p, c_void_p, c_void_p, c_int, c_int, c_float, c_void_p, c_void_p]),
    "asw_search_area": (c_int, [c_void_p, c_int, c_void_p, c_int, c_void_p, c_void_p, c_void_p, c_double, c_double,
                                POINTER(c_int), POINTER(c_void_p), POINTER(c_void_p), POINTER(c_void_p),
                                POINTER(c_void_p)]),
    "asw_free": (None, [c_void_p]),
    "asw_cube_select": (c_int, [c_void_p, c_int, c_int, c_int, c_int, c_int, c_int, c_int, c_int, c_void_p, c_void_p,
                                c_void_p, c_int64, POINTER(c_int64)]),
    "asw_cube_select_planes": (c_int, [c_void_p, c_int, c_int, c_int, c_int, c_int, c_int, c_int, c_int, c_void_p, c_void_p,
                                c_void_p, c_int64, POINTER(c_int64)]),
    "asw_srp_frames": (c_int, [c_int, c_int, c_int]),
    "asw_srp_cross_spectra": (c_int, [c_void_p, c_int, c_int, c_int, c_int, c_int, c_int, c_int, c_int, c_int,
                                      c_float, c_void_p, c_void_p, c_void_p, c_int, c_void_p, c_void_p, c_void_p]),
    "asw_srp_map": (c_int, [c_void_p, c_int, c_int, c_int, c_void_p, c_int, c_int, c_void_p, c_void_p, c_void_p,
                            c_void_p, c_void_p, c_void_p]),
    "asw_pruner_covariance": (c_int, [c_void_p, c_int, c_int, c_int, c_int, c_int, c_int, c_int, c_int, c_int,
                                      c_void_p, c_void_p, c_void_p]),
    "asw_hermitian_eigh": (c_int, [c_void_p, c_int, c_int, c_void_p, c_void_p, c_void_p]),
    "asw_music_map": (c_int, [c_void_p, c_int, c_int, c_int, c_void_p, c_int, c_void_p, c_void_p, c_void_p, c_void_p,
                              c_void_p]),
    "asw_tops_map": (c_int, [c_void_p, c_void_p, c_int, c_int, c_int, c_int, c_void_p, c_int, c_double, c_void_p,
                             c_void_p, c_void_p, c_void_p]),
    "asw_geom_lookup_planes": (c_int, [c_void_p, c_int, c_void_p, c_int, c_void_p, c_int, c_void_p, c_int, c_double, c_double,
                                       c_void_p, c_void_p]),
    "asw_geom_voxel_map": (c_int, [c_void_p, c_int, c_void_p, c_int, c_void_p, c_int, c_void_p, c_int, c_void_p, c_void_p,
                                   c_double, c_double, c_double, c_void_p, c_void_p, c_void_p, c_void_p]),
    "asw_geom_label": (c_int, [c_void_p, c_void_p, c_int, c_int, c_int, c_int, c_void_p, c_void_p, c_void_p, POINTER(c_int),
                               c_void_p]),
    "asw_geom_workspace_bytes": (c_int64, [c_int]),
    "asw_geom_compact": (c_int, [c_void_p, c_void_p, c_void_p, c_int, c_void_p, c_int, c_void_p, c_int, c_void_p, c_int,
                                 c_void_p, c_double, c_void_p, c_int64, c_void_p, c_void_p, c_void_p, c_void_p, c_void_p,
                                 c_void_p, c_void_p, c_void_p, c_void_p, POINTER(c_int), c_void_p]),
    "asw_geom_lattice_workspace_bytes": (c_int64, [c_int, c_int]),
    "asw_geom_lattice": (c_int, [c_void_p, c_int, c_int, c_int, c_int, c_void_p, c_void_p, c_void_p, c_void_p, c_double,
                                 c_void_p, c_int64, c_void_p, c_void_p, c_void_p, c_void_p, POINTER(c_int), c_void_p]),
    "asw_lattice_nms_workspace_bytes": (c_int64, [c_int, c_int]),
    "asw_lattice_nms": (c_int, [c_void_p, c_int, c_int, c_void_p, c_int, c_void_p, c_int64, c_void_p, c_void_p, c_void_p]),
}

_lib = None


def lib():
    global _lib
    if _lib is None:
        if not os.path.exists(LIB_PATH):
            raise RuntimeError(
                f"{LIB_PATH} is missing: run `python -c 'import __graft_entry__ as g; g.build()'` "
                "(hipcc --offload-arch=gfx950).  There is no CPU fallback for the hot path.")
        import torch
        L = ctypes.CDLL(LIB_PATH)
        for name, (res, args) in SIGNATURES.items():
            fn = getattr(L, name)
            fn.restype = res
            fn.argtypes = args
        _lib = L
    return _lib


_ops = None


def torch_ops():
    global _ops
    if _ops is None:
        lib()
        if not os.path.exists(OPS_PATH):
            raise RuntimeError(f"{OPS_PATH} is missing: run `python -c 'import __graft_entry__ as g; g.build()'`.  "
                               "The hot path is exposed only through these custom ops; there is no fallback.")
        import torch
        torch.ops.load_library(OPS_PATH)
        _ops = torch.ops.asw
    return _ops


def residue_schedule(taps, stride, Cin, BK=32, BM=256, m0=0, dil=1, pad=0, has_skip=False):
    n, mx = c_int(), c_int()
    L = lib()
    check(L.asw_residue_schedule(taps, stride, dil, pad, Cin, BK, BM, m0, int(has_skip), None, 0, ctypes.byref(n),
                                 ctypes.byref(mx)))
    if n.value == 0:
        return None
    buf = (ResidueStage * n.value)()
    check(L.asw_residue_schedule(taps, stride, dil, pad, Cin, BK, BM, m0, int(has_skip), buf, n.value, ctypes.byref(n),
                                 ctypes.byref(mx)))
    stages = [{"residue": d.residue, "chunk": d.chunk, "rows": d.rows, "first_row": d.first_row,
               "taps": [(d.tap[q], d.shift[q], d.kstep[q]) for q in range(d.ntaps)]} for d in buf]
    return stages, mx.value


def check(status: int):
    if status != 0:
        msg = lib().asw_last_error()
        raise RuntimeError(f"libasw_hip: status {status}: {msg.decode() if msg else ''}")


def ptr(t):
    return None if t is None else c_void_p(t.data_ptr())


def current_stream():
    import torch
    return c_void_p(torch.cuda.current_stream().cuda_stream)


def to_device(a, device):
    import torch
    src = torch.from_numpy(a)
    host = torch.empty(src.shape, dtype=src.dtype, pin_memory=True)
    host.copy_(src)
    return host.to(device, non_blocking=True)


def to_host(t):
    import torch
    if not t.is_cuda:
        return t.numpy()
    host = torch.empty(t.shape, dtype=t.dtype, pin_memory=True)
    host.copy_(t)
    return host.numpy()


def read_back(*tensors):
    import torch
    if not tensors:
        return []
    flat = [t.contiguous().reshape(-1).view(torch.uint8) for t in tensors]
    back = torch.cat(flat).cpu()
    out, pos = [], 0
    for t, f in zip(tensors, flat):
        piece = back[pos:pos + f.numel()].clone()
        out.append(piece.view(t.dtype).reshape(t.shape).numpy())
        pos += f.numel()
    return out
```

### acousticswarms-speech_amd/ops.py

```python
from ctypes import byref

import torch

from .native import ConvGemmArgs, MaskPathArgs, ResStackArgs, check, current_stream, lib, ptr


def _f32(t):
    assert t.is_cuda and t.dtype == torch.float32 and t.is_contiguous(), "need contiguous float32 CUDA tensor"
    return t


def pack_conv_weight(w: torch.Tensor) -> torch.Tensor:
    N, Cin, K = w.shape
    return w.permute(0, 2, 1).reshape(N, K * Cin).contiguous()


def convgemm(A, Wt, M_out, N, Cin, taps=1, stride=1, dil=1, pad=0, bias=None, relu=False, resid=None, mul=None,
             ln=None, stats_chan_mod=0, A2=None, B=None, a_row_stride=None, a_batch_stride=None, a_len=None,
             out=None, ln_eps=1e-5, precision="f32", use_fragments=True, glu=None, glu_out=None):
    _f32(A); _f32(Wt)
    if B is None:
        B = A.shape[0]
    a_row_stride = Cin if a_row_stride is None else a_row_stride
    if a_batch_stride is None:
        a_batch_stride = A[0].numel()
    if a_len is None:
        a_len = a_batch_stride
    if out is None:
        out = torch.empty((B, M_out, N), dtype=torch.float32, device=A.device)
    stats = None
    if stats_chan_mod:
        tiles = lib().asw_convgemm_stats_tiles(M_out, N)
        stats = torch.zeros((B, tiles, 4), dtype=torch.float32, device=A.device)
    a = ConvGemmArgs()
    a.A, a.A2, a.Wt = A.data_ptr(), (A2.data_ptr() if A2 is not None else None), Wt.data_ptr()
    a.bias = bias.data_ptr() if bias is not None else None
    a.resid = resid.data_ptr() if resid is not None else None
    a.mul = mul.data_ptr() if mul is not None else None
    a.ln_gamma = ln[0].data_ptr() if ln is not None else None
    a.ln_beta = ln[1].data_ptr() if ln is not None else None
    a.out = out.data_ptr()
    a.stats = stats.data_ptr() if stats is not None else None
    a.B, a.M_out, a.N, a.Cin, a.taps, a.stride, a.dil, a.pad = B, M_out, N, Cin, taps, stride, dil, pad
    a.a_row_stride, a.a_batch_stride, a.a_len = a_row_stride, a_batch_stride, a_len
    a.chan_mod, a.relu, a.ln_eps = stats_chan_mod, int(relu), ln_eps
    if glu is not None:
        a.glu_raw, a.glu_mr, a.glu_gamma, a.glu_beta = (_f32(t).data_ptr() for t in glu)
        if glu_out is not None:
            a.glu_out = _f32(glu_out).data_ptr()
    keep = None
    if precision in ("f16x3", "f16"):
        hi, lo, shift = split_weights_f16(Wt)
        keep = (hi, lo)
        a.precision, a.w_shift, a.Wt_hi, a.Wt_lo = (1 if precision == "f16x3" else 2), shift, hi.data_ptr(), lo.data_ptr()
        if use_fragments and N % 32 == 0 and (taps * Cin) % 16 == 0:
            fh, fl, sh2 = pack_fragments_f16(Wt, N, taps * Cin)
            assert sh2 == shift
            keep = keep + (fh, fl)
            a.Wf_hi, a.Wf_lo = fh.data_ptr(), fl.data_ptr()
    check(lib().asw_convgemm_f32(byref(a), current_stream()))
    torch.cuda.current_stream().synchronize() if keep is not None else None
    return out, stats


def resstack(x, layers, taps=7, precision="f16x3", eps=1e-5, glu=None, out=None, glu_out=None):
    src = x if glu is None else glu[0]
    B, T = src.shape[0], src.shape[1]
    if out is None:
        out = torch.empty((B, T, 64), dtype=torch.float32, device=src.device)
    a = ResStackArgs()
    a.x = _f32(x).data_ptr() if x is not None else None
    a.out = out.data_ptr()
    a.B, a.T, a.C, a.taps, a.n_layers = B, T, 64, taps, len(layers)
    a.precision, a.ln_eps = (1 if precision == "f16x3" else 2), eps
    keep = []
    for i, (Wt, bias, gamma, beta, dil) in enumerate(layers):
        fh, fl, sh = pack_fragments_f16(_f32(Wt), 64, taps * 64)
        keep.append((fh, fl))
        d = a.layer[i]
        d.Wf_hi, d.Wf_lo, d.w_shift, d.dil = fh.data_ptr(), fl.data_ptr(), sh, dil
        d.bias, d.ln_gamma, d.ln_beta = _f32(bias).data_ptr(), _f32(gamma).data_ptr(), _f32(beta).data_ptr()
    if glu is not None:
        a.glu_raw, a.glu_mr, a.glu_gamma, a.glu_beta = (_f32(t).data_ptr() for t in glu)
        if glu_out is not None:
            a.glu_out = _f32(glu_out).data_ptr()
    check(lib().asw_resstack64_f16x3(byref(a), current_stream()))
    torch.cuda.current_stream().synchronize()
    return out


def resstack_src(src_hi, src_lo, pre_w, pre_b, layers, taps=7, eps=1e-5, out=None):
    import ctypes
    import numpy as np
    B, T = src_hi.shape[0], src_hi.shape[1]
    dev = src_hi.device
    if out is None:
        out = torch.empty((B, T, 64), dtype=torch.float32, device=dev)
    M = pre_w.shape[1]
    wc = np.ascontiguousarray(layers[0][0].detach().cpu().numpy(), dtype=np.float32)
    wp = np.ascontiguousarray(pre_w.detach().cpu().numpy(), dtype=np.float32).reshape(64, M)
    bp = np.ascontiguousarray(pre_b.detach().cpu().numpy(), dtype=np.float32)
    comp, pre16 = np.empty((64, 64), dtype=np.float32), np.empty((64, 16), dtype=np.float32)
    check(lib().asw_compose_source_weights(ctypes.c_void_p(wc.ctypes.data), ctypes.c_void_p(wp.ctypes.data),
                                           ctypes.c_void_p(bp.ctypes.data), M, taps, ctypes.c_void_p(comp.ctypes.data),
                                           ctypes.c_void_p(pre16.ctypes.data)))
    a = ResStackArgs()
    a.out = out.data_ptr()
    a.B, a.T, a.C, a.taps, a.n_layers, a.precision, a.ln_eps = B, T, 64, taps, len(layers), 1, eps
    keep = []
    for i, (w, bias, gamma, beta, dil) in enumerate(layers):
        Wt = torch.from_numpy(comp).to(dev) if i == 0 else pack_conv_weight(w).to(dev)
        fh, fl, sh = pack_fragments_f16(Wt, 64, Wt.shape[1])
        keep.append((fh, fl))
        d = a.layer[i]
        d.Wf_hi, d.Wf_lo, d.w_shift, d.dil = fh.data_ptr(), fl.data_ptr(), sh, dil
        d.bias, d.ln_gamma, d.ln_beta = _f32(bias).data_ptr(), _f32(gamma).data_ptr(), _f32(beta).data_ptr()
    ph, pl, psh = pack_fragments_f16(torch.from_numpy(pre16).to(dev), 64, 16)
    a.src_hi, a.src_lo, a.pre_hi, a.pre_lo, a.pre_shift = src_hi.data_ptr(), src_lo.data_ptr(), ph.data_ptr(), pl.data_ptr(), psh
    check(lib().asw_resstack64_f16x3(byref(a), current_stream()))
    torch.cuda.current_stream().synchronize()
    return out


def pack_fragments_f16(Wt, N, K):
    import ctypes
    import numpy as np
    w = np.ascontiguousarray(Wt.detach().cpu().numpy(), dtype=np.float32).reshape(N, K)
    hi = np.empty(w.size, dtype=np.uint16)
    lo = np.empty(w.size, dtype=np.uint16)
    sh = ctypes.c_int32()
    check(lib().asw_pack_fragments_f16(ctypes.c_void_p(w.ctypes.data), N, K, ctypes.c_void_p(hi.ctypes.data),
                                       ctypes.c_void_p(lo.ctypes.data), byref(sh)))
    dev = Wt.device
    return (torch.from_numpy(hi.view(np.int16)).to(dev), torch.from_numpy(lo.view(np.int16)).to(dev), sh.value)


def split_weights_f16(Wt):
    import ctypes
    import numpy as np
    w = np.ascontiguousarray(Wt.detach().cpu().numpy(), dtype=np.float32)
    hi = np.empty(w.size, dtype=np.uint16)
    lo = np.empty(w.size, dtype=np.uint16)
    sh = ctypes.c_int32()
    check(lib().asw_split_weights_f16(ctypes.c_void_p(w.ctypes.data), w.size, ctypes.c_void_p(hi.ctypes.data),
                                      ctypes.c_void_p(lo.ctypes.data), byref(sh)))
    dev = Wt.device
    return (torch.from_numpy(hi.view(np.int16)).to(dev), torch.from_numpy(lo.view(np.int16)).to(dev), sh.value)


def gn_glu(raw, stats, gamma, beta, eps=1e-5):
    B, T, C2 = raw.shape
    C = C2 // 2
    out = torch.empty((B, T, C), dtype=torch.float32, device=raw.device)
    check(lib().asw_gn_glu(ptr(_f32(raw)), ptr(_f32(stats)), stats.shape[1], ptr(_f32(gamma)), ptr(_f32(beta)),
                           B, T, C, eps, ptr(out), current_stream()))
    return out


def gn_finalize(stats, T, C, eps=1e-5):
    B = stats.shape[0]
    mr = torch.empty((B, 4), dtype=torch.float32, device=stats.device)
    check(lib().asw_gn_finalize(ptr(_f32(stats)), stats.shape[1], B, T, C, eps, ptr(mr), current_stream()))
    return mr


def add_layernorm(x, resid, gamma, beta, eps=1e-5):
    rows, N = x.shape
    out = torch.empty_like(x)
    check(lib().asw_add_layernorm(ptr(_f32(x)), ptr(_f32(resid)), ptr(_f32(gamma)), ptr(_f32(beta)), rows, N, eps,
                                  ptr(out), current_stream()))
    return out


def attention(qkv, nhead, precision="f32"):
    B, L, d3 = qkv.shape
    d = d3 // 3
    ctx = torch.empty((B, L, d), dtype=torch.float32, device=qkv.device)
    check(lib().asw_attention_prec(ptr(_f32(qkv)), B, L, d, nhead, {"f32": 0, "f16x3": 1, "f16": 2}[precision], ptr(ctx),
                                   current_stream()))
    return ctx


def shift_stats(mix, offsets, circular=True):
    M, T = mix.shape
    N = offsets.shape[0]
    mean = torch.empty((N,), dtype=torch.float32, device=mix.device)
    std = torch.empty((N,), dtype=torch.float32, device=mix.device)
    check(lib().asw_shift_stats(ptr(_f32(mix)), M, T, ptr(offsets), N, int(circular), ptr(mean), ptr(std),
                                current_stream()))
    return mean, std


def shift_norm_preproc(mix, offsets, mean, std, w, b, T_pad, circular=True):
    M, T = mix.shape
    N = offsets.shape[0]
    C = w.shape[0]
    x0 = torch.empty((N, T_pad, C), dtype=torch.float32, device=mix.device)
    refn = torch.zeros((N, T_pad), dtype=torch.float32, device=mix.device)
    check(lib().asw_shift_norm_preproc(ptr(_f32(mix)), M, T, T_pad, ptr(offsets), N, int(circular), ptr(mean),
                                       ptr(std), ptr(_f32(w)), ptr(_f32(b)), C, ptr(x0), ptr(refn), T_pad,
                                       current_stream()))
    return x0, refn


def shift_norm_src(mix, offsets, mean, std, T_pad, circular=True):
    M, T = mix.shape
    N = offsets.shape[0]
    hi = torch.empty((N, T_pad, 8), dtype=torch.float16, device=mix.device)
    lo = torch.empty((N, T_pad, 8), dtype=torch.float16, device=mix.device)
    refn = torch.zeros((N, T_pad), dtype=torch.float32, device=mix.device)
    check(lib().asw_shift_norm_src_multi(ptr(_f32(mix)), M, T, T_pad, ptr(offsets), None, N, int(circular), ptr(mean),
                                         ptr(std), ptr(hi), ptr(lo), ptr(refn), T_pad, current_stream()))
    return hi, lo, refn


def overlap_add_unnorm(D, taps, hop, t, trim_left, trim_right, bias, mean=None, std=None):
    B, F, ldd = D.shape
    out = torch.empty((B, t), dtype=torch.float32, device=D.device)
    check(lib().asw_overlap_add_unnorm(ptr(_f32(D)), B, F, ldd, taps, hop, t, trim_left, trim_right, float(bias),
                                       ptr(mean), ptr(std), ptr(out), current_stream()))
    return out


def overlap_add_parts(Dp, taps, hop, t, trim_left, trim_right, bias, mean=None, std=None):
    nparts, B, F, ldd = Dp.shape
    out = torch.empty((B, t), dtype=torch.float32, device=Dp.device)
    check(lib().asw_overlap_add_parts(ptr(_f32(Dp)), nparts, B, F, ldd, taps, hop, t, trim_left, trim_right,
                                      float(bias), ptr(mean), ptr(std), ptr(out), current_stream()))
    return out


def mask_path(x, ref, ref_hop, enc_w, enc_b, byp_w, byp_b, dec_w, frames, stride, pad, precision="f16x3", scaled=False):
    B, Tp, C = x.shape
    E, _, EK = enc_w.shape
    dev = x.device
    Wt = pack_conv_weight(enc_w).to(dev)
    fh, fl, sh = pack_fragments_f16(Wt, E, EK * C)
    wb = torch.zeros((E, 48), dtype=torch.float32)
    wb[:, :byp_w.shape[-1]] = byp_w[:, 0].cpu()
    bh, bl, bsh = pack_fragments_f16(wb.to(dev), E, 48)
    wd = torch.zeros((64, E), dtype=torch.float32)
    wd[:dec_w.shape[-1]] = dec_w[:, 0].t().cpu()
    dh, dl, dsh = pack_fragments_f16(wd.to(dev), 64, E)
    parts = torch.zeros((E // 256, B, frames, 64), dtype=torch.float32, device=dev)
    m = MaskPathArgs()
    a = m.enc
    a.A, a.bias = _f32(x).data_ptr(), (_f32(enc_b).data_ptr() if enc_b is not None else None)
    a.B, a.M_out, a.N, a.Cin, a.taps, a.stride, a.dil, a.pad = B, frames, E, C, EK, stride, 1, pad
    a.a_row_stride, a.a_batch_stride, a.a_len = C, Tp * C, Tp * C
    a.precision, a.w_shift, a.Wf_hi, a.Wf_lo = {"f16x3": 1, "f16": 2}[precision], sh, fh.data_ptr(), fl.data_ptr()
    m.ref, m.ref_batch_stride, m.ref_len, m.ref_hop = _f32(ref).data_ptr(), ref.shape[1], ref.shape[1], ref_hop
    m.byp_k, m.byp_taps, m.byp_shift = 48, byp_w.shape[-1], bsh
    m.byp_hi, m.byp_lo = bh.data_ptr(), bl.data_ptr()
    m.byp_bias = _f32(byp_b).data_ptr() if byp_b is not None else None
    m.dec_hi, m.dec_lo, m.dec_shift, m.dec_taps = dh.data_ptr(), dl.data_ptr(), dsh, dec_w.shape[-1]
    m.taps = parts.data_ptr()
    check((lib().asw_mask_path_f16x3_scaled if scaled else lib().asw_mask_path_f16x3)(byref(m), current_stream()))
    torch.cuda.current_stream().synchronize()
    return parts


def energies(y, window=12000):
    B, T = y.shape
    out = torch.empty((B, 2), dtype=torch.float64, device=y.device)
    check(lib().asw_energies(ptr(_f32(y)), B, T, window, None, ptr(out), current_stream()))
    return out


def pair_sisdr(y):
    n, T = y.shape
    out = torch.empty((n, n), dtype=torch.float64, device=y.device)
    check(lib().asw_pair_sisdr(ptr(_f32(y)), n, T, ptr(out), current_stream()))
    return out


def srp_cross_spectra(mix, twiddle, pair_i, pair_j, nbins, window, step, n_windows, nfft, hop, tol=1e-8):
    M, T = mix.shape
    P = pair_i.shape[0]
    nb_pad = twiddle.shape[0] // 2
    assert twiddle.shape == (2 * nb_pad, nfft), "twiddle must be [2*nb_pad, nfft]"
    for t in (pair_i, pair_j):
        assert t.is_cuda and t.dtype == torch.int32 and t.is_contiguous() and t.numel() == P, "pair tables: int32 [P]"
    F = lib().asw_srp_frames(window, nfft, hop)
    xf = torch.empty((M, max(F, 1), 2 * nb_pad), dtype=torch.float32, device=mix.device)
    cc = torch.full((n_windows, nbins, P, 2), float("nan"), dtype=torch.float32, device=mix.device)
    check(lib().asw_srp_cross_spectra(ptr(_f32(mix)), M, T, window, step, n_windows, nfft, hop, nbins, nb_pad, tol,
                                      ptr(_f32(twiddle)), ptr(pair_i), ptr(pair_j), P, ptr(xf), ptr(cc),
                                      current_stream()))
    return cc


def srp_map(cc, tau, omega, pair_i, pair_j):
    n_windows, nbins, P, _ = cc.shape
    G, M = tau.shape
    for t, dt, n in ((tau, torch.float64, G * M), (omega, torch.float64, nbins), (pair_i, torch.int32, P),
                     (pair_j, torch.int32, P)):
        assert t.is_cuda and t.dtype == dt and t.is_contiguous() and t.numel() == n, "srp_map: operand dtype / size"
    part = torch.empty((8 * 8 * G,), dtype=torch.float32, device=cc.device)
    out = torch.empty((G,), dtype=torch.float32, device=cc.device)
    check(lib().asw_srp_map(ptr(_f32(cc)), n_windows, nbins, P, ptr(tau), G, M, ptr(omega), ptr(pair_i), ptr(pair_j),
                            ptr(part), ptr(out), current_stream()))
    return out


def joint_shift_stats(mix, offsets):
    M, T = mix.shape
    S = offsets.shape[0]
    scratch = torch.empty((lib().asw_joint_shift_stats_scratch_doubles(),), dtype=torch.float64, device=mix.device)
    mean = torch.empty((S,), dtype=torch.float32, device=mix.device)
    std = torch.empty((S,), dtype=torch.float32, device=mix.device)
    check(lib().asw_joint_shift_stats(ptr(_f32(mix)), M, T, ptr(offsets), S, ptr(scratch), ptr(mean), ptr(std),
                                      current_stream()))
    return mean, std


def _group_tables(counts):
    import ctypes
    bounds, items = [0], []
    for k, c in enumerate(counts):
        if int(c) > 0:
            bounds.append(bounds[-1] + int(c))
            items.append(k)
    return (ctypes.c_int32 * len(bounds))(*bounds), (ctypes.c_int32 * max(1, len(items)))(*items), len(items)


def joint_shift_stats_groups(mix_stack, offsets, counts):
    K, M, T = mix_stack.shape
    N = offsets.shape[0]
    assert len(counts) == K and sum(int(c) for c in counts) == N and all(int(c) >= 0 for c in counts)
    assert offsets.is_cuda and offsets.dtype == torch.int32 and offsets.is_contiguous() and offsets.shape[1] == M - 1
    bounds, items, G = _group_tables(counts)
    scratch = torch.empty((max(1, G) * lib().asw_joint_shift_stats_scratch_doubles(),), dtype=torch.float64,
                          device=mix_stack.device)
    mean = torch.empty((N,), dtype=torch.float32, device=mix_stack.device)
    std = torch.empty((N,), dtype=torch.float32, device=mix_stack.device)
    check(lib().asw_joint_shift_stats_groups(ptr(_f32(mix_stack)), M, T, ptr(offsets), bounds, G, items, ptr(scratch),
                                             ptr(mean), ptr(std), current_stream()))
    return mean, std


def add_layernorm2(x, y=None, alpha=1.0, gamma=None, beta=None, eps=1e-5, act=0, want_sum=False, want_ln=True):
    rows, N = x.shape
    s = torch.empty_like(x) if want_sum else None
    o = torch.empty_like(x) if want_ln else None
    check(lib().asw_add_layernorm2(ptr(_f32(x)), ptr(y), float(alpha), ptr(gamma), ptr(beta), rows, N, eps, act, ptr(s),
                                   ptr(o), current_stream()))
    return s, o


def glu_rows(raw):
    rows, C2 = raw.shape
    out = torch.empty((rows, C2 // 2), dtype=torch.float32, device=raw.device)
    check(lib().asw_glu_rows(ptr(_f32(raw)), rows, C2 // 2, ptr(out), current_stream()))
    return out


def dwconv_ln_swish(u, w, bias, gamma, beta, eps=1e-5):
    BS, L, d = u.shape
    K = w.shape[-1]
    wT = w.reshape(d, K).t().contiguous()
    out = torch.empty_like(u)
    check(lib().asw_dwconv_ln_swish(ptr(_f32(u)), ptr(_f32(wT)), ptr(_f32(bias)), ptr(_f32(gamma)), ptr(_f32(beta)),
                                    BS, L, d, K, eps, ptr(out), current_stream()))
    return out


def relpos_attention(qkv, P, bias_u, bias_v, nhead, scale):
    BS, L, d3 = qkv.shape
    d = d3 // 3
    ctx = torch.empty((BS, L, d), dtype=torch.float32, device=qkv.device)
    check(lib().asw_relpos_attention(ptr(_f32(qkv)), ptr(_f32(P)), ptr(_f32(bias_u)), ptr(_f32(bias_v)), BS, L, d, nhead,
                                     float(scale), ptr(ctx), current_stream()))
    return ctx


def inter_attention(qkv, nhead):
    NB, S, L, d3 = qkv.shape
    d = d3 // 3
    ctx = torch.empty((NB, S, L, d), dtype=torch.float32, device=qkv.device)
    check(lib().asw_inter_attention(ptr(_f32(qkv)), NB, S, L, d, nhead, ptr(ctx), current_stream()))
    return ctx


def inter_attention_groups(qkv, counts, nhead, out=None):
    N, L, d3 = qkv.shape
    d = d3 // 3
    assert sum(int(c) for c in counts) == N and all(int(c) >= 0 for c in counts)
    bounds, _items, G = _group_tables(counts)
    ctx = torch.empty((N, L, d), dtype=torch.float32, device=qkv.device) if out is None else out
    assert ctx.shape == (N, L, d)
    check(lib().asw_inter_attention_groups(ptr(_f32(qkv)), bounds, G, L, d, nhead, ptr(_f32(ctx)), current_stream()))
    return ctx


def f16x3_overflow_count(reset=True) -> int:
    import ctypes
    c = ctypes.c_int32()
    check(lib().asw_f16x3_overflow_count(int(reset), byref(c)))
    return int(c.value) & 0xFFFFFFFF
```

### acousticswarms-speech_amd/spot.py

```python
import numpy as np

from . import native
from .config import FULL, SpotConfig, spot_param_shapes
from .device_model import DeviceModel
from .scorer import DeviceScorer


def offsets_from_patches(patch_list, n_pairs: int = None) -> np.ndarray:
    if len(patch_list) == 0:
        return np.zeros((0, n_pairs or 0), dtype=np.int32)
    offs = np.stack([np.asarray(getattr(p, "sample_offset", p), dtype=np.float64) for p in patch_list])
    if n_pairs is not None and offs.shape[1] != n_pairs:
        raise RuntimeError(f"candidate has {offs.shape[1]} offsets, mixture has {n_pairs + 1} channels")
    return np.rint(offs.astype(np.float32)).astype(np.int32)


class SpotModel(DeviceModel, DeviceScorer):
    C_PREFIX, CONFIG_C, NAME, HOT_PATH = "spot", native.SpotConfigC, "SpotModel", "spot hot path"
    param_shapes = staticmethod(spot_param_shapes)

    def __init__(self, cfg: SpotConfig = FULL, state_dict=None, batch_size: int = 32, precision: str = "f32",
                 lanes: int = 1):
        DeviceModel.__init__(self, cfg, precision)
        self.batch_size = batch_size
        self.lanes = int(lanes)
        self.last_waveforms = None
        if state_dict is not None:
            self.load_state_dict(state_dict)

    def _reload_context(self):
        import contextlib
        import torch
        return torch.cuda.device(self.device) if self.device is not None else contextlib.nullcontext()

    def _configure(self):
        native.check(self._c("set_batch")(self._h, int(self.batch_size)))
        DeviceModel._configure(self)
        native.check(self._c("set_lanes")(self._h, self.lanes))

    def set_lanes(self, lanes: int):
        self.lanes = int(lanes)
        if self._h is not None:
            native.check(native.lib().asw_spot_set_lanes(self._h, self.lanes))

    def set_batch_size(self, b: int):
        self.batch_size = int(b)
        if self._h is not None:
            native.check(native.lib().asw_spot_set_batch(self._h, int(b)))

    def shift_and_sep_device(self, mix_dev, offsets_dev, strict: int = 0, want_wave: bool = True,
                             want_energy: bool = False, window: int = 12000, circular: bool = True):
        import torch
        self._need()
        M, T = mix_dev.shape
        N = offsets_dev.shape[0]
        assert mix_dev.dtype == torch.float32 and mix_dev.is_contiguous() and mix_dev.is_cuda
        assert offsets_dev.dtype == torch.int32 and offsets_dev.is_contiguous() and offsets_dev.is_cuda
        wave, en = native.torch_ops().spot_shift_and_sep(self._h.value, mix_dev, offsets_dev, int(strict), bool(circular),
                                                         bool(want_wave), bool(want_energy), int(window))
        return (wave if want_wave else None), (en if want_energy else None)

    def shift_and_sep_device_multi(self, mix_stack, offsets_dev, mix_index_dev, strict: int = 0, want_wave: bool = True,
                                   want_energy: bool = False, window: int = 12000, circular: bool = True):
        import torch
        self._need()
        assert mix_stack.dim() == 3 and mix_stack.dtype == torch.float32 and mix_stack.is_contiguous() and mix_stack.is_cuda
        assert offsets_dev.dtype == torch.int32 and offsets_dev.is_contiguous() and offsets_dev.is_cuda
        assert mix_index_dev.dtype == torch.int32 and mix_index_dev.is_contiguous() and mix_index_dev.is_cuda
        wave, en = native.torch_ops().spot_shift_and_sep_multi(self._h.value, mix_stack, offsets_dev, mix_index_dev,
                                                               int(strict), bool(circular), bool(want_wave),
                                                               bool(want_energy), int(window))
        return (wave if want_wave else None), (en if want_energy else None)

    def shift_and_sep(self, input_channels, patch_list, Strict: int = 0, save_input: bool = False) -> np.ndarray:
        import torch
        self._need()
        if save_input:
            raise RuntimeError("save_input=True is a debugging path of the reference that materialises every "
                               "shifted mixture; it is not provided (the shifted tensor never exists here)")
        mix = torch.as_tensor(input_channels)
        T = mix.shape[-1]
        if len(patch_list) == 0:
            return np.empty((0, T), dtype=np.float32)
        offs = offsets_from_patches(patch_list, mix.shape[0] - 1)
        mix_d = mix.to(self.device, dtype=torch.float32).contiguous()
        off_d = torch.from_numpy(offs).to(self.device)
        wave, _ = self.shift_and_sep_device(mix_d, off_d, Strict, want_wave=True)
        return native.to_host(wave)

    def shift_and_score(self, input_channels, patch_list, Strict: int = 0, window: int = 12000,
                        keep_waveforms: bool = True) -> np.ndarray:
        import torch
        self._need()
        mix = torch.as_tensor(input_channels)
        if len(patch_list) == 0:
            self.last_waveforms = None
            return np.empty((0, 2), dtype=np.float64)
        offs = offsets_from_patches(patch_list, mix.shape[0] - 1)
        mix_d = mix.to(self.device, dtype=torch.float32).contiguous()
        off_d = torch.from_numpy(offs).to(self.device)
        wave, en = self.shift_and_sep_device(mix_d, off_d, Strict, want_wave=keep_waveforms, want_energy=True,
                                             window=window)
        self.last_waveforms = wave
        return en.cpu().numpy()

    def shift_and_sep_resident(self, input_channels, patch_list, Strict: int = 0, window: int = 12000,
                               device_energies: bool = False):
        import torch
        self._need()
        mix = torch.as_tensor(input_channels)
        offs = offsets_from_patches(patch_list, mix.shape[0] - 1)
        mix_d = mix.to(self.device, dtype=torch.float32).contiguous()
        if device_energies:
            off_d = torch.from_numpy(offs).pin_memory().to(self.device, non_blocking=True)
        else:
            off_d = torch.from_numpy(offs).to(self.device)
        wave, en = self.shift_and_sep_device(mix_d, off_d, Strict, want_wave=True, want_energy=True, window=window)
        native.torch_ops().center_rows_(wave)
        return wave, (en if device_energies else en.cpu().numpy())

    def score_offsets(self, input_channels, offsets, Strict: int = 0, window: int = 12000):
        import torch
        self._need()
        mix = torch.as_tensor(input_channels)
        mix_d = mix.to(self.device, dtype=torch.float32).contiguous()
        if isinstance(offsets, torch.Tensor):
            off_d = offsets.to(self.device, dtype=torch.int32).contiguous()
        else:
            off_d = torch.from_numpy(np.ascontiguousarray(offsets, dtype=np.int32)).pin_memory().to(self.device, non_blocking=True)
        if off_d.dim() != 2 or off_d.shape[1] != mix_d.shape[0] - 1:
            raise RuntimeError(f"offsets of shape {tuple(off_d.shape)} do not fit a mixture of {mix_d.shape[0]} channels")
        if off_d.shape[0] == 0:
            return torch.empty((0, 2), dtype=torch.float64, device=self.device)
        _wave, en = self.shift_and_sep_device(mix_d, off_d, Strict, want_wave=False, want_energy=True, window=window)
        return en

    def forward(self, mix, window_embedding):
        import torch
        self._need()
        mix = torch.as_tensor(mix).to(self.device, dtype=torch.float32).contiguous()
        wemb = torch.as_tensor(window_embedding, dtype=torch.float32).cpu().numpy().reshape(mix.shape[0], 2)
        B, M, t = mix.shape
        out = torch.empty((B, 1, t), dtype=torch.float32, device=self.device)
        keys = {}
        for i, row in enumerate(map(tuple, wemb)):
            keys.setdefault(row, []).append(i)
        ops = native.torch_ops()
        for row, idx in keys.items():
            whole = len(idx) == B
            y = ops.spot_forward(self._h.value, mix if whole else mix[idx].contiguous(), float(row[0]), float(row[1]))
            if whole:
                return y.view(B, 1, t)
            out.view(B, t)[idx] = y
        return out

    __call__ = forward

    def set_fused_mask(self, on: bool = True):
        self._need()
        native.check(native.lib().asw_spot_set_fused_mask(self._h, int(bool(on))))
        return self

    def set_source_stack(self, on: bool = True):
        self._need()
        native.check(native.lib().asw_spot_set_source_stack(self._h, int(bool(on))))
        return self
```

### include/asw_hip.h

```cpp
#ifndef ASW_HIP_H
#define ASW_HIP_H

#include <stddef.h>
#include <stdint.h>

#ifdef __cplusplus
extern "C" {
#endif

typedef enum asw_status {
  ASW_OK = 0,
  ASW_ERR_ARG = -1,
  ASW_ERR_HIP = -2,
  ASW_ERR_NOMEM = -3,
  ASW_ERR_STATE = -4
} asw_status;

const char* asw_last_error(void);
int asw_abi_version(void);

int asw_profile_enable(int on);
int asw_profile_report(char* buf, size_t cap);

typedef struct asw_spot_config {
  int32_t n_mics;
  int32_t kernel_size;
  int32_t depth;
  int32_t stride_list[8];
  int32_t channels;
  int32_t growth;
  int32_t encoder_channels;
  int32_t encoder_kernel_size;
  int32_t encoder_stride;
  int32_t residual_layers;
  int32_t residual_dilation_factor;
  int32_t num_head;
  int32_t ffw_dim;
  int32_t num_transformer_layers;
} asw_spot_config;

typedef struct asw_spot asw_spot;

int asw_spot_create(const asw_spot_config* cfg, asw_spot** out);
void asw_spot_destroy(asw_spot* m);

int asw_spot_set_param(asw_spot* m, const char* key, const float* host_data, size_t numel);
int asw_spot_finalize(asw_spot* m);

int asw_spot_set_batch(asw_spot* m, int batch);

int asw_spot_set_lanes(asw_spot* m, int lanes);

int asw_spot_set_precision(asw_spot* m, int precision);

int asw_spot_shift_and_sep(asw_spot* m, const float* mix, int M, int T,
                           const int32_t* offsets, int N, int strict, int circular,
                           float* out_wave, double* out_energy, int energy_window,
                           void* stream);

int asw_spot_shift_and_sep_multi(asw_spot* m, const float* mix, int K, int M, int T, const int32_t* offsets,
                                 const int32_t* mix_index, int N, int strict, int circular, float* out_wave,
                                 double* out_energy, int energy_window, void* stream);

int asw_spot_forward(asw_spot* m, const float* mix_norm, int B, int M, int t,
                     const float* window_embedding_host, float* out, void* stream);

int asw_spot_set_fused_mask(asw_spot* m, int on);

int asw_spot_set_source_stack(asw_spot* m, int on);

int asw_spot_get_tap(asw_spot* m, const char* name, float* dst, size_t capacity, size_t* numel,
                     void* stream);

typedef struct asw_sep_config {
  int32_t n_mics;
  int32_t max_speakers;
  int32_t kernel_size;
  int32_t depth;
  int32_t stride_list[8];
  int32_t channels;
  int32_t growth;
  int32_t encoder_channels;
  int32_t encoder_kernel_size;
  int32_t encoder_stride;
  int32_t residual_layers;
  int32_t residual_dilation_factor;
  int32_t num_head;
  int32_t ffw_dim;
  int32_t bottleneck_layers;
  int32_t bottleneck_ksize;
} asw_sep_config;

typedef struct asw_sep asw_sep;

int asw_sep_create(const asw_sep_config* cfg, asw_sep** out);
void asw_sep_destroy(asw_sep* m);
int asw_sep_set_param(asw_sep* m, const char* key, const float* host_data, size_t numel);
int asw_sep_finalize(asw_sep* m);
int asw_sep_set_precision(asw_sep* m, int precision);

int asw_sep_infer(asw_sep* m, const float* mix, int M, int T, const int32_t* offsets, int S, float* out,
                  void* stream);

int asw_sep_infer_batch(asw_sep* m, const float* mix, int K, int M, int T, const int32_t* offsets,
                        const int32_t* counts, float* out, void* stream);

int asw_sep_forward(asw_sep* m, const float* mix_norm, int B, int S, int M, int t, float* out, void* stream);
int asw_sep_forward_counts(asw_sep* m, const float* mix_norm, int B, int S, int M, int t, const int32_t* counts,
                           float* out, void* stream);
int asw_sep_get_config(const asw_sep* m, asw_sep_config* out);

int asw_sep_get_tap(asw_sep* m, const char* name, float* dst, size_t capacity, size_t* numel, void* stream);

int asw_joint_shift_stats(const float* mix, int M, int T, const int32_t* offsets, int S, double* scratch,
                          float* mean, float* std, void* stream);
int asw_joint_shift_stats_scratch_doubles(void);
int asw_joint_shift_stats_groups(const float* mix, int M, int T, const int32_t* offsets, const int32_t* bounds, int G,
                                 const int32_t* item_of_group, double* scratch, float* mean, float* std, void* stream);

int asw_add_layernorm2(const float* x, const float* y, float alpha, const float* gamma, const float* beta,
                       int rows, int N, float eps, int act, float* sum_out, float* ln_out, void* stream);

int asw_glu_rows(const float* raw, long rows, int C, float* out, void* stream);

int asw_dwconv_ln_swish(const float* u, const float* wT, const float* bias, const float* gamma, const float* beta,
                        int BS, int L, int d, int K, float eps, float* out, void* stream);

int asw_relpos_attention(const float* qkv, const float* P, const float* bias_u, const float* bias_v, int BS, int L,
                         int d, int nhead, float scale, float* ctx, void* stream);

int asw_inter_attention(const float* qkv, int NB, int S, int L, int d, int nhead, float* ctx, void* stream);
int asw_inter_attention_groups(const float* qkv, const int32_t* bounds, int G, int L, int d, int nhead, float* ctx,
                               void* stream);


int asw_shift_stats(const float* mix, int M, int T, const int32_t* offsets, int N,
                    int circular, float* mean, float* std, void* stream);

int asw_shift_norm_preproc(const float* mix, int M, int T, int T_pad, const int32_t* offsets,
                           int N, int circular, const float* mean, const float* std,
                           const float* w, const float* b, int C, float* x0, float* refn,
                           long refn_stride, void* stream);

int asw_shift_stats_multi(const float* mix, int M, int T, const int32_t* offsets, const int32_t* mix_index, int N,
                          int circular, float* mean, float* std, void* stream);
int asw_shift_norm_preproc_multi(const float* mix, int M, int T, int T_pad, const int32_t* offsets,
                                 const int32_t* mix_index, int N, int circular, const float* mean, const float* std,
                                 const float* w, const float* b, int C, float* x0, float* refn, long refn_stride,
                                 void* stream);

int asw_shift_norm_src_multi(const float* mix, int M, int T, int T_pad, const int32_t* offsets,
                             const int32_t* mix_index, int N, int circular, const float* mean, const float* std,
                             void* src_hi, void* src_lo, float* refn, long refn_stride, void* stream);

int asw_pad_preproc(const float* x, int B, int M, int t, int T_pad, const float* w,
                    const float* b, int C, float* x0, float* refn, long refn_stride,
                    void* stream);

typedef struct asw_convgemm_args {
  const float* A;
  const float* A2;
  const float* Wt;
  const float* bias;
  const float* resid;
  const float* mul;
  const float* ln_gamma;
  const float* ln_beta;
  float* out;
  float* stats;
  int32_t B, M_out, N, Cin, taps, stride, dil, pad;
  int32_t a_row_stride;
  int64_t a_batch_stride;
  int64_t a_len;
  int32_t chan_mod;
  int32_t relu;
  float ln_eps;
  int32_t precision;
  int32_t w_shift;
  const void* Wt_hi;
  const void* Wt_lo;
  const void* Wf_hi;
  const void* Wf_lo;
  int32_t stats_stride;
  const float* glu_raw;
  const float* glu_mr;
  const float* glu_gamma;
  const float* glu_beta;
  float* glu_out;
} asw_convgemm_args;
int asw_pack_fragments_f16(const float* Wt, int N, int K, uint16_t* hi, uint16_t* lo, int32_t* w_shift);
int asw_convgemm_f32(const asw_convgemm_args* args, void* stream);
typedef struct asw_maskpath_args {
  asw_convgemm_args enc;
  const float* ref;
  int64_t ref_batch_stride;
  int64_t ref_len;
  int32_t ref_hop;
  int32_t byp_k;
  int32_t byp_taps;
  int32_t byp_shift;
  const void* byp_hi;
  const void* byp_lo;
  const float* byp_bias;
  const void* dec_hi;
  const void* dec_lo;
  int32_t dec_shift;
  int32_t dec_taps;
  float* taps;
} asw_maskpath_args;
int asw_mask_path_f16x3(const asw_maskpath_args* args, void* stream);
int asw_mask_path_f16x3_scaled(const asw_maskpath_args* args, void* stream);
typedef struct asw_reslayer_desc {
  const void* Wf_hi;
  const void* Wf_lo;
  const float* bias;
  const float* ln_gamma;
  const float* ln_beta;
  int32_t dil;
  int32_t w_shift;
} asw_reslayer_desc;
typedef struct asw_resstack_args {
  const float* x;
  float* out;
  int32_t B, T, C, taps, n_layers;
  int32_t precision;
  float ln_eps;
  asw_reslayer_desc layer[3];
  const float* glu_raw;
  const float* glu_mr;
  const float* glu_gamma;
  const float* glu_beta;
  float* glu_out;
  const void* src_hi;
  const void* src_lo;
  const void* pre_hi;
  const void* pre_lo;
  int32_t pre_shift;
} asw_resstack_args;
int asw_resstack64_f16x3(const asw_resstack_args* args, void* stream);
int asw_compose_source_weights(const float* wc, const float* wpre, const float* bpre, int M, int taps, float* comp,
                               float* pre16);
int asw_split_weights_f16(const float* w, size_t n, uint16_t* hi, uint16_t* lo, int32_t* w_shift);
int asw_f16x3_overflow_count(int reset, uint32_t* count);
int asw_convgemm_stats_tiles(int M_out, int N);
#define ASW_RESIDUE_MAX_TAPS 8
#define ASW_RESIDUE_MAX_SHIFT 2
typedef struct asw_residue_stage {
  int32_t residue;
  int32_t chunk;
  int32_t rows;
  int32_t first_row;
  int32_t ntaps;
  int32_t tap[ASW_RESIDUE_MAX_TAPS];
  int32_t shift[ASW_RESIDUE_MAX_TAPS];
  int32_t kstep[ASW_RESIDUE_MAX_TAPS];
} asw_residue_stage;
int asw_residue_schedule(int taps, int stride, int dil, int pad, int Cin, int BK, int BM, int m0, int has_skip,
                         asw_residue_stage* out, int cap, int* n_stages, int* max_shift);

int asw_gn_glu(const float* raw, const float* stats, int n_partials, const float* gamma,
               const float* beta, int B, int T, int C, float eps, float* out, void* stream);
int asw_gn_finalize(const float* stats, int n_partials, int B, int T, int C, float eps, float* mr, void* stream);

int asw_attention(const float* qkv, int B, int L, int d, int nhead, float* ctx, void* stream);
int asw_attention_prec(const float* qkv, int B, int L, int d, int nhead, int precision, float* ctx, void* stream);

int asw_overlap_add_unnorm(const float* D, int B, int F, int ldd, int taps, int hop,
                           int t, int trim_left, int trim_right, float bias, const float* mean,
                           const float* std, float* out, void* stream);
int asw_overlap_add_parts(const float* D, int nparts, int B, int F, int ldd, int taps, int hop,
                          int t, int trim_left, int trim_right, float bias, const float* mean,
                          const float* std, float* out, void* stream);

int asw_energies(const float* y, int B, int T, int window, double* scratch, double* out,
                 void* stream);

int asw_add_layernorm(const float* x, const float* resid, const float* gamma, const float* beta,
                      int rows, int N, float eps, float* out, void* stream);

int asw_center_rows(float* y, int B, int T, void* stream);

int asw_pair_sisdr(const float* y, int n, int T, double* out, void* stream);

int asw_segment_sisdr(const float* y, int n, int T, const int32_t* segments, const int32_t* seg_count,
                      int kmax, double* out, void* stream);

size_t asw_voiced_segments_workspace_bytes(int n, int T);
int asw_voiced_segments(const float* y, int n, int T, double thr, double Q, int32_t* segments, int kcap,
                        int32_t* counts, double* ms, void* workspace, size_t workspace_bytes, void* stream);

size_t asw_fine_clusters_workspace_bytes(const int32_t* bounds_host, int G);
int asw_fine_clusters(const float* y, int N, int T, const int32_t* bounds_host, int G, const double* energies,
                      const double* gate, const double* group_gate, double min_trigger, double ratio, void* workspace,
                      size_t workspace_bytes, int32_t* order, int32_t* label, double* gram, void* stream);

size_t asw_global_clusters_workspace_bytes(int n);
int asw_global_clusters(const double* full, const double* seg, const int32_t* counts, const uint8_t* near, int n, int K,
                        double sim_db, double win_hi, double win_lo, double best_hi, double best_lo, void* workspace,
                        size_t workspace_bytes, int32_t* label, uint8_t* merge_or_null, void* stream);

size_t asw_coarse_select_workspace_bytes(int N, int cap);
int asw_coarse_select(const double* energies, const double* dis1, const int32_t* best_or_null, int N, double thr1,
                      int relative, double rel, int cap, void* workspace, size_t workspace_bytes, int32_t* kept,
                      int32_t* counts, double* thr, void* stream);

size_t asw_bss_eval_sdr_workspace_bytes(const int32_t* counts_host, int K, int R, int T, int flen);
int asw_bss_eval_sdr(const float* ref, const float* est, const int32_t* counts_host, int K, int R, int T, int flen,
                     double* sdr, int32_t* status, void* workspace, size_t workspace_bytes, void* stream);

int asw_search_area(const double* points, int n_pts, const double* mic, int M, double* offset,
                    double* width, const double* ub, double sound_speed, double fs, int* n_children,
                    double** child_offset, double** child_width, int** child_count, int** child_index);
void asw_free(void* p);

int asw_cube_select(const double* offsets, int ny, int nx, int nz, int P, int y0, int y1, int x0, int x1,
                    const double* lo, const double* hi, int32_t* out_idx, int64_t cap, int64_t* count);
int asw_cube_select_planes(const double* planes, int ny, int nx, int nz, int P, int y0, int y1, int x0, int x1,
                    const double* lo, const double* hi, int32_t* out_idx, int64_t cap, int64_t* count);

int asw_srp_frames(int window, int nfft, int hop);
int asw_srp_cross_spectra(const float* mix, int M, int T, int window, int step, int n_windows,
                          int nfft, int hop, int nbins, int nb_pad, float tol,
                          const float* twiddle, const int32_t* pair_i, const int32_t* pair_j,
                          int P, float* xf_scratch, float* cc, void* stream);
int asw_srp_map(const float* cc, int n_windows, int nbins, int P, const double* tau, int G, int M,
                const double* omega, const int32_t* pair_i, const int32_t* pair_j,
                float* part_scratch, float* out, void* stream);

int asw_pruner_covariance(const float* mix, int M, int T, int window, int step, int n_windows,
                          int nfft, int hop, int bin0, int nbins, double* cov, double* magsum,
                          void* stream);
int asw_hermitian_eigh(const double* a, int n, int M, double* evals, double* evecs, void* stream);
int asw_music_map(const double* evecs, int n_windows, int nbins, int M, const double* tau, int G,
                  const double* omega, double* p_scratch, double* max_scratch, float* out,
                  void* stream);
int asw_tops_map(const double* evecs, const double* magsum, int n_windows, int nbins, int bin0,
                 int M, const double* delta, int G, double coef, double* q_scratch,
                 int32_t* max_bin, float* out, void* stream);

int asw_geom_lookup_planes(const double* ys, int ny, const double* xs, int nx, const double* zs, int nz,
                           const double* mics, int M, double C, double FS, double* planes, void* stream);
int asw_geom_voxel_map(const double* xs, int Lx, const double* ys, int Ly, const double* zs, int Lz,
                       const double* mics, int M, const double* border, const double* centre, double C,
                       double FS, double resolution, int32_t* q, uint8_t* valid, double* dis_matrix,
                       void* stream);
int asw_geom_label(const int32_t* q, const uint8_t* valid, int Lx, int Ly, int Lz, int P,
                   uint32_t* adj_scratch, int32_t* flag_scratch, int32_t* labels, int* sweeps, void* stream);
int64_t asw_geom_workspace_bytes(int n_voxels);
int asw_geom_compact(const int32_t* labels, const int32_t* q, const double* xs, int Lx, const double* ys, int Ly,
                     const double* zs, int Lz, const double* mics, int M, const double* centre, double C,
                     void* workspace, int64_t workspace_bytes, int32_t* power_index, int32_t* valid_flat,
                     int32_t* valid_cid, int32_t* members, int32_t* bounds, int32_t* offsets, double* centres,
                     double* tau, double* delta, int* counts, void* stream);
int64_t asw_geom_lattice_workspace_bytes(int n_points, int P);
int asw_geom_lattice(const double* planes, int P, int ny, int nx, int nz, const double* xs, const double* ys,
                     const double* zs, const double* border, double width, void* workspace,
                     int64_t workspace_bytes, int32_t* cells, int32_t* bounds, int32_t* members, double* centres,
                     int* counts, void* stream);
int64_t asw_lattice_nms_workspace_bytes(int N, int P);
int asw_lattice_nms(const int32_t* cells, int N, int P, const double* scores, int radius, void* workspace,
                    int64_t workspace_bytes, int32_t* best, int32_t* degree, void* stream);

#ifdef __cplusplus
}
#endif
#endif
```

Baseline: 2374 candidates/s.

## Fuse next decoder upsample GEMM and GN stats into residual-stack epilogue

The last residual-stack launch of decoder level j now adds the skip tensor, splits the result to f16 hi/lo in registers and runs the next level's 64->256 transposed-conv upsample GEMM with MFMA. It writes raw upsample output and group-norm partial stats directly. This removes writing and re-reading the decoder activation and drops a separate convgemm launch per qualifying level. In exchange it adds a K-permuted weight packing, extra register pressure in the stack kernel, and skips the intermediate decoder tap.

```diff
diff --git a/acousticswarms-speech_amd/csrc/asw_common.cpp b/acousticswarms-speech_amd/csrc/asw_common.cpp
--- a/acousticswarms-speech_amd/csrc/asw_common.cpp
+++ b/acousticswarms-speech_amd/csrc/asw_common.cpp
@@ -75,6 +75,18 @@
         }
   }
   delete[] th;
+  return rc;
+}
+
+extern "C" int asw_up_feed_kperm(int k) { return (k & ~12) | ((k & 4) << 1) | ((k & 8) >> 1); }
+
+extern "C" int asw_pack_up_feed_f16(const float* Wt, int N, int K, uint16_t* hi, uint16_t* lo, int32_t* w_shift) {
+  ASW_CHECK_ARG(Wt && N > 0 && K > 0 && K % 16 == 0, "pack_up_feed: K %% 16 required (N=%d K=%d)", N, K);
+  float* wp = new float[(size_t)N * K];
+  for (int n = 0; n < N; ++n)
+    for (int k = 0; k < K; ++k) wp[(size_t)n * K + k] = Wt[(size_t)n * K + (k & ~15) + asw_up_feed_kperm(k & 15)];
+  const int rc = asw_pack_fragments_f16(wp, N, K, hi, lo, w_shift);
+  delete[] wp;
   return rc;
 }
 
diff --git a/acousticswarms-speech_amd/csrc/model_common.h b/acousticswarms-speech_amd/csrc/model_common.h
--- a/acousticswarms-speech_amd/csrc/model_common.h
+++ b/acousticswarms-speech_amd/csrc/model_common.h
@@ -79,6 +79,18 @@
     ASW_HIP(hipMemcpy(flo, vl.data(), h.size() * 2, hipMemcpyHostToDevice));
     return ASW_OK;
   }
+  int upload_up_feed(const std::vector<float>& h, int N, int K) {
+    std::vector<uint16_t> vh(h.size()), vl(h.size());
+    int rc = asw_pack_up_feed_f16(h.data(), N, K, vh.data(), vl.data(), &shift);
+    if (rc) return rc;
+    if (fhi) { (void)hipFree(fhi); fhi = nullptr; }
+    if (flo) { (void)hipFree(flo); flo = nullptr; }
+    if (hipMalloc(&fhi, h.size() * 2) != hipSuccess || hipMalloc(&flo, h.size() * 2) != hipSuccess)
+      return asw::set_error(ASW_ERR_NOMEM, "hipMalloc(%zu halves)", h.size());
+    ASW_HIP(hipMemcpy(fhi, vh.data(), h.size() * 2, hipMemcpyHostToDevice));
+    ASW_HIP(hipMemcpy(flo, vl.data(), h.size() * 2, hipMemcpyHostToDevice));
+    return ASW_OK;
+  }
   void bind(asw_convgemm_args& a, int precision) const {
     a.Wt = f32.p; a.Wt_hi = hi; a.Wt_lo = lo; a.w_shift = shift; a.precision = precision;
     a.Wf_hi = fhi; a.Wf_lo = flo;
@@ -165,12 +177,29 @@
 
 struct SrcFeed { const void* hi; const void* lo; const WBuf* comp; const WBuf* pre; };
 
+struct UpFeed { const WBuf* w; const float* bias; const float* skip; float* out; float* stats; int tiles; };
+
+inline void resstack_last_launch(const std::vector<ResLayer>& res, int K, size_t& j0, size_t& n) {
+  j0 = 0;
+  n = resstack_fuse_count(res, 0, K);
+  while (j0 + n < res.size()) { j0 += n; n = resstack_fuse_count(res, j0, K); }
+}
+inline int up_feed_tiles(const std::vector<ResLayer>& res, int K, int T, bool glu) {
+  size_t j0, n;
+  resstack_last_launch(res, K, j0, n);
+  int32_t dil[3] = {1, 1, 1};
+  for (size_t i = 0; i < n; ++i) dil[i] = res[j0 + i].dil;
+  return asw_resstack_tiles(T, K, (int)n, dil, glu && j0 == 0);
+}
+
 inline int run_res(const std::vector<ResLayer>& res, int prec, int B, int T, int ch, int K, float* x, float* p, float* q,
-            float** final_out, hipStream_t s, const GluSrc* glu = nullptr, const SrcFeed* feed = nullptr) {
+            float** final_out, hipStream_t s, const GluSrc* glu = nullptr, const SrcFeed* feed = nullptr, UpFeed* up = nullptr) {
   const float* in = glu ? glu->raw : x;
   float* outb = p;
   if (feed && !(resstack_ok(res, prec, ch, K) && prec == 1 && resstack_fuse_count(res, 0, K) == 2))
     return asw::set_error(ASW_ERR_STATE, "run_res: the source-fed form needs the fused f16x3 pair");
+  if (up && !(resstack_ok(res, prec, ch, K) && prec == 1))
+    return asw::set_error(ASW_ERR_STATE, "run_res: UpFeed needs the f16x3 stack kernel");
   if (resstack_ok(res, prec, ch, K)) {
     size_t j = 0;
     while (j < res.size()) {
@@ -192,6 +221,14 @@
         a.layer[0].Wf_hi = feed->comp->fhi; a.layer[0].Wf_lo = feed->comp->flo; a.layer[0].w_shift = feed->comp->shift;
         a.pre_hi = feed->pre->fhi; a.pre_lo = feed->pre->flo; a.pre_shift = feed->pre->shift;
       }
+      if (up && j + n == res.size()) {
+        a.out = nullptr;
+        a.up_hi = up->w->fhi; a.up_lo = up->w->flo; a.up_shift = up->w->shift; a.up_bias = up->bias; a.up_skip = up->skip;
+        a.up_out = up->out; a.up_stats = up->stats;
+        up->tiles = up_feed_tiles(res, K, T, glu != nullptr);
+        if (up->tiles < 0) return up->tiles;
+        outb = nullptr;
+      }
       int rc = asw_resstack64_f16x3(&a, s);
       if (rc) return rc;
       in = outb;
@@ -282,7 +319,7 @@
 
 struct EncBlock { std::vector<ResLayer> res; DevBuf bias, gn_g, gn_b; };
 struct DecBlock { std::vector<ResLayer> res; DevBuf gn_g, gn_b; };
-struct GatedConvs { std::vector<WBuf> down_wt, up_wt; std::vector<DevBuf> up_bias; };
+struct GatedConvs { std::vector<WBuf> down_wt, up_wt, up_feed; std::vector<DevBuf> up_bias; };
 struct Tap { const float* p; size_t numel; };
 using ParamList = std::vector<std::pair<std::string, size_t>>;
 
@@ -306,6 +343,8 @@
   bool fuse_mask = true;
   bool want_src = false;
   bool src_stack = true;
+  bool want_up = false;
+  bool up_fusion = true;
 
   std::vector<int> enc_cin, enc_cout;
   std::vector<int> dec_cin, dec_cout, dec_stride;
@@ -468,6 +507,7 @@
     o.down_wt.clear(); o.down_wt.resize(tc.depth);
     o.up_wt.clear(); o.up_wt.resize(tc.depth);
     o.up_bias.clear(); o.up_bias.resize(tc.depth);
+    o.up_feed.clear(); o.up_feed.resize(tc.depth);
     for (int i = 0; i < tc.depth; ++i) {
       const std::string p = "encoder.module_list." + std::to_string(i);
       const std::vector<float> g = gate(p);
@@ -483,6 +523,7 @@
       pack_conv_transpose(P(p + ".upsample.conv.weight"), P(p + ".upsample.conv.bias"), ci, co2, s,
                           g.empty() ? nullptr : g.data(), wt, bb);
       if ((rc = o.up_wt[j].upload_gemm(wt, s * co2, ci))) return rc;
+      if (want_up && up_feed_shape(j) && (rc = o.up_feed[j].upload_up_feed(wt, s * co2, ci))) return rc;
       UP(o.up_bias[j], bb);
     }
     return ASW_OK;
@@ -496,6 +537,14 @@
     return want_src && src_stack && precision == 1 && src_wt.fhi && src_pre.fhi && !enc.empty() &&
            resstack_ok(enc[0].res, precision, enc_cin[0], tc.kernel_size) &&
            resstack_fuse_count(enc[0].res, 0, tc.kernel_size) == 2;
+  }
+  bool up_feed_shape(int j) const {
+    return j >= 1 && dec_cin[j] == 64 && dec_cout[j] == 64 && dec_stride[j] == 2 && dec_cout[j - 1] == 64;
+  }
+  bool up_path(const GatedConvs& g, int j) const {
+    static const bool off = getenv("ASW_NO_UP_FUSION") != nullptr;
+    return !off && want_up && up_fusion && precision == 1 && up_feed_shape(j) && g.up_feed[j].fhi &&
+           resstack_ok(dec[j - 1].res, precision, 64, tc.kernel_size);
   }
   void layout_levels(int B, int T, Arena& a, TrunkPlan& pl) const {
     const int depth = tc.depth, EK = tc.encoder_kernel_size, ES = tc.encoder_stride;
@@ -531,7 +580,13 @@
       const int lvl = depth - j;
       const int s = dec_stride[j], co2 = 2 * dec_cout[j];
       pl.raw_up[j] = a.take<float>((size_t)B * pl.Tl[lvl] * s * co2);
-      pl.st_up[j] = a.take<float>((size_t)B * 4 * asw_convgemm_stats_tiles(pl.Tl[lvl], s * co2));
+      int tiles = asw_convgemm_stats_tiles(pl.Tl[lvl], s * co2);
+      if (want_up && up_feed_shape(j))
+        for (int glu = 0; glu < 2; ++glu) {
+          const int t = up_feed_tiles(dec[j - 1].res, tc.kernel_size, pl.Tl[lvl], glu != 0);
+          tiles = t > tiles ? t : tiles;
+        }
+      pl.st_up[j] = a.take<float>((size_t)B * 4 * tiles);
       pl.mr_up[j] = a.take<float>((size_t)B * 4);
     }
   }
@@ -577,33 +632,42 @@
     return ASW_OK;
   }
 
-  int decode(TrunkPlan& pl, const GatedConvs& g, const float*& x, hipStream_t s) {
+  int decode(TrunkPlan& pl, const GatedConvs& g, const float*& x, hipStream_t s, bool up = false) {
     const int B = pl.B, K = tc.kernel_size;
     int rc;
+    int fed_tiles = 0;
     for (int j = 0; j < tc.depth; ++j) {
       const int lvl = tc.depth - j, ci = dec_cin[j], co = dec_cout[j], st = dec_stride[j];
-      asw_convgemm_args a = {};
-      a.A = x; a.A2 = pl.X[lvl]; g.up_wt[j].bind(a, precision); a.bias = g.up_bias[j].p; a.out = pl.raw_up[j];
-      a.stats = pl.st_up[j];
-      a.B = B; a.M_out = pl.Tl[lvl]; a.N = st * 2 * co; a.Cin = ci; a.taps = 1; a.stride = 1; a.dil = 1; a.pad = 0;
-      a.a_row_stride = ci; a.a_batch_stride = (int64_t)pl.Tl[lvl] * ci; a.a_len = a.a_batch_stride;
-      a.chan_mod = 2 * co;
-      if ((rc = asw_convgemm_f32(&a, s))) return rc;
+      int tiles = fed_tiles;
+      if (!fed_tiles) {
+        asw_convgemm_args a = {};
+        a.A = x; a.A2 = pl.X[lvl]; g.up_wt[j].bind(a, precision); a.bias = g.up_bias[j].p; a.out = pl.raw_up[j];
+        a.stats = pl.st_up[j];
+        a.B = B; a.M_out = pl.Tl[lvl]; a.N = st * 2 * co; a.Cin = ci; a.taps = 1; a.stride = 1; a.dil = 1; a.pad = 0;
+        a.a_row_stride = ci; a.a_batch_stride = (int64_t)pl.Tl[lvl] * ci; a.a_len = a.a_batch_stride;
+        a.chan_mod = 2 * co;
+        if ((rc = asw_convgemm_f32(&a, s))) return rc;
+        tiles = asw_convgemm_stats_tiles(a.M_out, a.N);
+      }
       const int To = pl.Tl[lvl] * st;
-      const int tiles = asw_convgemm_stats_tiles(a.M_out, a.N);
       float* gb = pl.Qb[lvl - 1];
       float* r = nullptr;
+      const bool feed_next = up && j + 1 < tc.depth && up_path(g, j + 1);
+      UpFeed uf = {};
+      if (feed_next) uf = {&g.up_feed[j + 1], g.up_bias[j + 1].p, pl.X[lvl - 1], pl.raw_up[j + 1], pl.st_up[j + 1], 0};
+      UpFeed* ufp = feed_next ? &uf : nullptr;
       if (fuse_mask && glu_on_load_ok(dec[j].res, precision, co)) {
         if ((rc = asw_gn_finalize(pl.st_up[j], tiles, B, To, co, 1e-5f, pl.mr_up[j], s))) return rc;
         const GluSrc src = {pl.raw_up[j], pl.mr_up[j], dec[j].gn_g.p, dec[j].gn_b.p, co > 64 ? gb : nullptr};
-        if ((rc = run_res(dec[j].res, precision, B, To, co, K, gb, pl.Pb[lvl - 1], gb, &r, s, &src))) return rc;
+        if ((rc = run_res(dec[j].res, precision, B, To, co, K, gb, pl.Pb[lvl - 1], gb, &r, s, &src, nullptr, ufp))) return rc;
       } else {
         if ((rc = asw_gn_glu(pl.raw_up[j], pl.st_up[j], tiles, dec[j].gn_g.p, dec[j].gn_b.p, B, To, co, 1e-5f, gb, s)))
           return rc;
-        if ((rc = run_res(dec[j].res, precision, B, To, co, K, gb, pl.Pb[lvl - 1], gb, &r, s))) return rc;
+        if ((rc = run_res(dec[j].res, precision, B, To, co, K, gb, pl.Pb[lvl - 1], gb, &r, s, nullptr, nullptr, ufp))) return rc;
       }
       x = r;
-      taps["dec" + std::to_string(j)] = {x, (size_t)B * To * co};
+      fed_tiles = feed_next ? uf.tiles : 0;
+      if (!feed_next) taps["dec" + std::to_string(j)] = {x, (size_t)B * To * co};
     }
     return ASW_OK;
   }
diff --git a/acousticswarms-speech_amd/csrc/resstack.hip b/acousticswarms-speech_amd/csrc/resstack.hip
--- a/acousticswarms-speech_amd/csrc/resstack.hip
+++ b/acousticswarms-speech_amd/csrc/resstack.hip
@@ -46,6 +46,18 @@
   LayerDev L[MAXL];
 };
 
+constexpr int UPN = 256;
+struct UpArgs {
+  const half8* Wh;
+  const half8* Wl;
+  const float* bias;
+  const float* skip;
+  float* out;
+  float* stats;
+  float scale;
+};
+struct KArgsUp : KArgs { UpArgs u; };
+
 __device__ __forceinline__ __amdgpu_buffer_rsrc_t src_rsrc(const half8* base, long rows) {
   return __builtin_amdgcn_make_buffer_rsrc(const_cast<half8*>(base), 0, (int)(rows * 16), 0x00020000);
 }
@@ -53,9 +65,10 @@
   return __builtin_bit_cast(half8, __builtin_amdgcn_raw_buffer_load_b128(r, row >= 0 ? row * 16 : (int)0x80000000, 0, 0));
 }
 
-template <int NL, int NW, int TM, int PH, bool POLY, bool GLU, int NTERM, int QD, bool SRC = false>
+template <int NL, int NW, int TM, int PH, bool POLY, bool GLU, int NTERM, int QD, bool SRC = false, bool UP = false>
 __global__ __launch_bounds__(64 * NW) __attribute__((amdgpu_waves_per_eu(TM >= 4 ? 1 : 2)))
-void resstack64_kernel(const KArgs p) {
+void resstack64_kernel(const std::conditional_t<UP, KArgsUp, KArgs> p) {
+  static_assert(!UP || (!SRC && NTERM == 3), "UpFeed: f16x3, never source-fed");
   static_assert(!POLY || NL == 1, "polyphase row sets: single layers only");
   static_assert(!SRC || (!POLY && !GLU && NTERM == 3), "source-fed layer 0: contiguous tiles, f16x3");
   static_assert(QD == 2 || QD == 4, "weight prefetch depth in k-steps");
@@ -341,6 +354,109 @@
         }
       }
       __syncthreads();
+    } else if constexpr (UP) {
+      const UpArgs& u = p.u;
+      const __amdgpu_buffer_rsrc_t rS = act_rsrc(u.skip + (long)b * T * C, (long)T * C);
+      const int tstep = POLY ? dil0 : 1;
+      const int widu = __builtin_amdgcn_readfirstlane(wid);
+      half8 xh[TM][4], xl[TM][4];
+      int t0[TM], nv[TM];
+#pragma unroll
+      for (int i = 0; i < TM; ++i) {
+        const int f0 = (widu * TM + i) * 32;
+        int lim;
+        if (!POLY) {
+          t0[i] = m0 + f0;
+          lim = min(p.BM, T - m0) - f0;
+        } else {
+          const int ph = pb * PH + f0 / BMJ;
+          t0[i] = dil0 * (jb * BMJ + f0 % BMJ) + ph;
+          lim = (ph < dil0 && t0[i] < T) ? (T - 1 - t0[i]) / dil0 + 1 : 0;
+        }
+        nv[i] = i < Ld.nfrag - widu * TM ? min(max(lim, 0), 32) : 0;
+        const bool ok = (lane & 31) < nv[i];
+        const long e0 = ((long)t0[i] + (long)(lane & 31) * tstep) * C + h * 4;
+        float4 sk[8];
+#pragma unroll
+        for (int c8 = 0; c8 < 8; ++c8) sk[c8] = act_load4(rS, e0 + c8 * 8, ok);
+#pragma unroll
+        for (int cb = 0; cb < 2; ++cb)
+#pragma unroll
+          for (int q = 0; q < 4; ++q) {
+            const float4 s4 = sk[cb * 4 + q];
+            const float4 v = make_float4(acc[i][cb][q * 4 + 0] + s4.x, acc[i][cb][q * 4 + 1] + s4.y,
+                                         acc[i][cb][q * 4 + 2] + s4.z, acc[i][cb][q * 4 + 3] + s4.w);
+            half4 hi, lo;
+            split4t<NTERM>(v, hi, lo);
+#pragma unroll
+            for (int j = 0; j < 4; ++j) {
+              xh[i][cb * 2 + (q >> 1)][(q & 1) * 4 + j] = hi[j];
+              xl[i][cb * 2 + (q >> 1)][(q & 1) * 4 + j] = lo[j];
+            }
+          }
+      }
+      float st0 = 0.f, sq0 = 0.f, st1 = 0.f, sq1 = 0.f;
+      __amdgpu_buffer_rsrc_t rO[TM];
+#pragma unroll
+      for (int i = 0; i < TM; ++i)
+        rO[i] = __builtin_amdgcn_make_buffer_rsrc(u.out + ((long)b * T + t0[i]) * UPN, 0,
+                                                  nv[i] > 0 ? ((nv[i] - 1) * tstep + 1) * UPN * 4 : 0, 0x00020000);
+      const int voff = (4 * h * tstep * UPN + (lane & 31)) * 4;
+      const int rstep = tstep * UPN * 4;
+      half8 wh[2][2], wl[2][2];
+      auto wload = [&](int ks, int nb2, int slot) __attribute__((always_inline)) {
+#pragma unroll
+        for (int e = 0; e < 2; ++e) frag_load<NTERM>(u.Wh, u.Wl, (long)ks * (UPN / 32) + nb2 * 2 + e, lane, wh[slot][e], wl[slot][e]);
+      };
+      wload(0, 0, 0);
+#pragma unroll 1
+      for (int nb2 = 0; nb2 < UPN / 64; ++nb2) {
+        floatx16 y[TM][2];
+#pragma unroll
+        for (int i = 0; i < TM; ++i)
+#pragma unroll
+          for (int e = 0; e < 2; ++e)
+#pragma unroll
+            for (int r = 0; r < 16; ++r) y[i][e][r] = 0.f;
+        const float bv[2] = {u.bias[nb2 * 64 + (lane & 31)], u.bias[nb2 * 64 + 32 + (lane & 31)]};
+#pragma unroll
+        for (int ks = 0; ks < 4; ++ks) {
+          if (ks < 3) wload(ks + 1, nb2, (ks + 1) & 1);
+          else wload(0, nb2 + 1 < UPN / 64 ? nb2 + 1 : nb2, 0);
+#pragma unroll
+          for (int i = 0; i < TM; ++i)
+#pragma unroll
+            for (int e = 0; e < 2; ++e) mma3<NTERM, false>(y[i][e], xh[i][ks], xl[i][ks], wh[ks & 1][e], wl[ks & 1][e]);
+        }
+        float s1 = 0.f, s2 = 0.f;
+#pragma unroll
+        for (int i = 0; i < TM; ++i) {
+          const bool whole = nv[i] == 32;
+#pragma unroll
+          for (int e = 0; e < 2; ++e)
+#pragma unroll
+            for (int r = 0; r < 16; ++r) {
+              const float v = y[i][e][r] * u.scale + bv[e];
+              __builtin_amdgcn_raw_buffer_store_b32(__builtin_bit_cast(int, v), rO[i],
+                                                    voff + ((r & 3) + 8 * (r >> 2)) * rstep + (nb2 * 64 + e * 32) * 4, 0, 0);
+              const float m = (whole || acc_row(r, h) < nv[i]) ? v : 0.f;
+              s1 += m;
+              s2 += m * m;
+            }
+        }
+        if (nb2 & 1) { st1 += s1; sq1 += s2; } else { st0 += s1; sq0 += s2; }
+      }
+      st0 = wave_sum(st0); sq0 = wave_sum(sq0); st1 = wave_sum(st1); sq1 = wave_sum(sq1);
+      __syncthreads();
+      float* red = reinterpret_cast<float*>(smem);
+      if (lane == 0) { red[wid * 4 + 0] = st0; red[wid * 4 + 1] = sq0; red[wid * 4 + 2] = st1; red[wid * 4 + 3] = sq1; }
+      __syncthreads();
+      if (tid < 4) {
+        float s = 0.f;
+#pragma unroll
+        for (int w = 0; w < NW; ++w) s += red[w * 4 + tid];
+        u.stats[((long)b * p.ntile + tile) * 4 + tid] = s;
+      }
     } else {
       float* __restrict__ ob = p.out + (long)b * T * C;
 #pragma unroll
@@ -396,11 +512,21 @@
 }
 
 template <int NL, int NW, int TM, int PH, bool POLY, bool GLU, int QD, bool SRC = false>
-int launch_stack(const KArgs& k, int precision, size_t smem, double flops, const char* tag, hipStream_t s) {
+int launch_stack(const KArgs& k, const UpArgs* up, int precision, size_t smem, double flops, const char* tag, hipStream_t s) {
   char nm[128], detail[48] = "";
-  snprintf(nm, sizeof nm, "resstack64<%s,%dx%d%s%s%s>", tag, NW, TM, POLY ? (PH == 1 ? ",poly1" : PH == 2 ? ",poly2" : ",poly4") : "",
-           GLU ? ",glu" : "", SRC ? ",src" : "");
+  snprintf(nm, sizeof nm, "resstack64<%s,%dx%d%s%s%s%s>", tag, NW, TM, POLY ? (PH == 1 ? ",poly1" : PH == 2 ? ",poly2" : ",poly4") : "",
+           GLU ? ",glu" : "", SRC ? ",src" : "", up ? ",up" : "");
   if (asw::prof_detail()) snprintf(detail, sizeof detail, "[B%d M%d d%d]", k.B, k.T, k.L[0].dil);
+  if constexpr (!SRC) {
+    if (up) {
+      KArgsUp ku;
+      static_cast<KArgs&>(ku) = k;
+      ku.u = *up;
+      return asw::launch_pair<resstack64_kernel<NL, NW, TM, PH, POLY, GLU, 3, QD, false, true>, resstack64_kernel<NL, NW, TM, PH, POLY, GLU, 3, QD, false, true>>(
+          1, dim3(xcd_grid_run(k.B * k.ntile)), dim3(64 * NW), smem, 160 * 1024, nm, detail,
+          flops + 2.0 * k.B * (double)k.T * C * UPN, (double)k.B * k.T * 4 * ((GLU ? 3 : 2) * C + UPN), s, ku);
+    }
+  }
   if constexpr (SRC) {
     return asw::launch_pair<resstack64_kernel<NL, NW, TM, PH, POLY, GLU, 3, QD, true>, resstack64_kernel<NL, NW, TM, PH, POLY, GLU, 3, QD, true>>(
         1, dim3(xcd_grid_run(k.B * k.ntile)), dim3(64 * NW), smem, 160 * 1024, nm, detail, flops,
@@ -412,29 +538,38 @@
   }
 }
 
+struct TilePlan { bool poly; int PH, BM, ntile; };
+TilePlan plan_tiles(int T, int n_layers, int dil0, int halo0, bool glu, int R0) {
+  const int rpp = T / dil0;
+  if (n_layers == 1 && dil0 >= 7 && rpp >= 48 && !glu) {
+    const int PH = rpp >= R0 - 32 ? 1 : rpp >= R0 / 2 - 32 ? 2 : 4;
+    return {true, PH, R0, asw::cdiv(asw::cdiv(T, dil0), R0 / PH) * asw::cdiv(dil0, PH)};
+  }
+  const int BM = R0 - 2 * halo0;
+  return {false, 1, BM, BM > 0 ? asw::cdiv(T, BM) : 0};
+}
+
 template <int NW, int TM>
-int dispatch(const asw_resstack_args& a, KArgs& k, bool glu, double flops, hipStream_t s) {
+int dispatch(const asw_resstack_args& a, KArgs& k, const UpArgs* up, bool glu, double flops, hipStream_t s) {
   constexpr int R0 = 32 * NW * TM;
   const int dil0 = k.L[0].dil;
-  const int rpp = a.T / dil0;
-  if (a.n_layers == 1 && dil0 >= 7 && rpp >= 48 && !glu) {
-    const int PH = rpp >= R0 - 32 ? 1 : rpp >= R0 / 2 - 32 ? 2 : 4;
+  const TilePlan tp = plan_tiles(a.T, a.n_layers, dil0, k.L[0].halo, glu, R0);
+  k.BM = tp.BM;
+  k.ntile = tp.ntile;
+  if (tp.poly) {
+    const int PH = tp.PH;
     const int BMJ = R0 / PH;
-    k.BM = R0;
     k.L[0].nfrag = NW * TM;
-    k.ntile = asw::cdiv(asw::cdiv(a.T, dil0), BMJ) * asw::cdiv(dil0, PH);
     k.img_rows = PH * (BMJ + a.taps - 1);
     const size_t smem = (size_t)k.img_rows * RS + 3 * 64 * sizeof(float);
     switch (PH) {
-      case 1: return launch_stack<1, NW, TM, 1, true, false, 4>(k, a.precision, smem, flops, "1", s);
-      case 2: return launch_stack<1, NW, TM, 2, true, false, 4>(k, a.precision, smem, flops, "1", s);
-      default: return launch_stack<1, NW, TM, 4, true, false, 4>(k, a.precision, smem, flops, "1", s);
-    }
-  }
-  k.BM = R0 - 2 * k.L[0].halo;
+      case 1: return launch_stack<1, NW, TM, 1, true, false, 4>(k, up, a.precision, smem, flops, "1", s);
+      case 2: return launch_stack<1, NW, TM, 2, true, false, 4>(k, up, a.precision, smem, flops, "1", s);
+      default: return launch_stack<1, NW, TM, 4, true, false, 4>(k, up, a.precision, smem, flops, "1", s);
+    }
+  }
   ASW_CHECK_ARG(k.BM >= R0 / 2, "resstack: the later layers' halo (%d rows per side) leaves %d of %d rows; fuse fewer layers",
                 k.L[0].halo, k.BM, R0);
-  k.ntile = asw::cdiv(a.T, k.BM);
   int rows = 0;
   for (int i = 0; i < a.n_layers; ++i) {
     k.L[i].nfrag = asw::cdiv(k.BM + 2 * k.L[i].halo, 32);
@@ -447,15 +582,15 @@
                 rows, dil0, a.taps);
   if (k.src_h) {
     ASW_CHECK_ARG(k.L[0].nfrag == NW * TM, "resstack: source-fed layer 0 computes %d of %d fragments", k.L[0].nfrag, NW * TM);
-    return launch_stack<2, NW, TM, 1, false, false, 4, true>(k, a.precision, smem, flops, "2", s);
+    return launch_stack<2, NW, TM, 1, false, false, 4, true>(k, nullptr, a.precision, smem, flops, "2", s);
   }
   switch (a.n_layers) {
-    case 1: return glu ? launch_stack<1, NW, TM, 1, false, true, 4>(k, a.precision, smem, flops, "1", s)
-                       : launch_stack<1, NW, TM, 1, false, false, 4>(k, a.precision, smem, flops, "1", s);
-    case 2: return glu ? launch_stack<2, NW, TM, 1, false, true, 4>(k, a.precision, smem, flops, "2", s)
-                       : launch_stack<2, NW, TM, 1, false, false, 4>(k, a.precision, smem, flops, "2", s);
-    default: return glu ? launch_stack<3, NW, TM, 1, false, true, 4>(k, a.precision, smem, flops, "3", s)
-                        : launch_stack<3, NW, TM, 1, false, false, 4>(k, a.precision, smem, flops, "3", s);
+    case 1: return glu ? launch_stack<1, NW, TM, 1, false, true, 4>(k, up, a.precision, smem, flops, "1", s)
+                       : launch_stack<1, NW, TM, 1, false, false, 4>(k, up, a.precision, smem, flops, "1", s);
+    case 2: return glu ? launch_stack<2, NW, TM, 1, false, true, 4>(k, up, a.precision, smem, flops, "2", s)
+                       : launch_stack<2, NW, TM, 1, false, false, 4>(k, up, a.precision, smem, flops, "2", s);
+    default: return glu ? launch_stack<3, NW, TM, 1, false, true, 4>(k, up, a.precision, smem, flops, "3", s)
+                        : launch_stack<3, NW, TM, 1, false, false, 4>(k, up, a.precision, smem, flops, "3", s);
   }
 }
 
@@ -492,6 +627,15 @@
   return ASW_OK;
 }
 
+extern "C" int asw_resstack_tiles(int T, int taps, int n_layers, const int32_t* dil, int glu) {
+  ASW_CHECK_ARG(T > 0 && taps >= 3 && taps % 2 == 1 && n_layers >= 1 && n_layers <= MAXL && dil, "resstack_tiles: bad argument");
+  int halo0 = 0;
+  for (int i = 1; i < n_layers; ++i) halo0 += dil[i] * (taps - 1) / 2;
+  const TilePlan t = plan_tiles(T, n_layers, dil[0], halo0, glu != 0, 256);
+  ASW_CHECK_ARG(t.BM >= 128, "resstack_tiles: the later layers' halo (%d rows per side) is too wide", halo0);
+  return t.ntile;
+}
+
 extern "C" int asw_resstack64_f16x3(const asw_resstack_args* args, void* stream) {
   ASW_CHECK_ARG(args != nullptr, "resstack: null args");
   const asw_resstack_args& a = *args;
@@ -501,7 +645,7 @@
   ASW_CHECK_ARG(a.taps >= 3 && a.taps <= 15 && a.taps % 2 == 1, "resstack: taps=%d (odd, 3..15)", a.taps);
   ASW_CHECK_ARG(a.precision == 1 || a.precision == 2, "resstack: precision 1 (f16x3) or 2 (single-pass f16)");
   ASW_CHECK_ARG(a.B > 0 && a.B <= (1 << 20) && a.T > 0 && (int64_t)a.T * 2 * C < ((int64_t)1 << 29), "resstack: bad B / T");
-  ASW_CHECK_ARG(a.out && (a.x || a.glu_raw || a.src_hi), "resstack: null tensor");
+  ASW_CHECK_ARG((a.out || a.up_hi) && (a.x || a.glu_raw || a.src_hi), "resstack: null tensor");
   const bool glu = a.glu_raw != nullptr;
   if (glu) ASW_CHECK_ARG(a.glu_mr && a.glu_gamma && a.glu_beta, "resstack: GroupNorm + GLU on load needs the statistics / affine arrays");
   KArgs k = {};
@@ -529,5 +673,13 @@
     k.pre_up = ldexpf(1.0f, a.pre_shift); k.pre_down = ldexpf(1.0f, -a.pre_shift);
     flops = 2.0 * a.B * (double)a.T * C * (64 + 16 + C * a.taps);
   }
-  return dispatch<4, 2>(a, k, glu, flops, s);
-}
+  UpArgs up = {};
+  if (a.up_hi) {
+    ASW_CHECK_ARG(a.up_lo && a.up_bias && a.up_skip && a.up_out && a.up_stats, "resstack: UpFeed needs up_lo / up_bias / up_skip / up_out / up_stats");
+    ASW_CHECK_ARG(a.precision == 1 && !a.src_hi, "resstack: UpFeed is f16x3 and never source-fed");
+    up.Wh = reinterpret_cast<const half8*>(a.up_hi); up.Wl = reinterpret_cast<const half8*>(a.up_lo);
+    up.bias = a.up_bias; up.skip = a.up_skip; up.out = a.up_out; up.stats = a.up_stats;
+    up.scale = ldexpf(1.0f, -a.up_shift);
+  }
+  return dispatch<4, 2>(a, k, a.up_hi ? &up : nullptr, glu, flops, s);
+}
diff --git a/acousticswarms-speech_amd/csrc/spot_model.hip b/acousticswarms-speech_amd/csrc/spot_model.hip
--- a/acousticswarms-speech_amd/csrc/spot_model.hip
+++ b/acousticswarms-speech_amd/csrc/spot_model.hip
@@ -26,7 +26,7 @@
   hipStream_t side = nullptr;
   hipEvent_t ev_fork = nullptr, ev_join = nullptr;
 
-  asw_spot() { want_src = true; }
+  asw_spot() { want_src = true; want_up = true; }
   ~asw_spot() {
     for (char* w : ws) if (w) (void)hipFree(w);
     if (side) (void)hipStreamDestroy(side);
@@ -139,7 +139,7 @@
 }
 
 int run_network(asw_spot* m, Plan& pl, GateSet* gs, const float* mean, const float* stdv, float* out_wave,
-                hipStream_t s, bool src0 = false) {
+                hipStream_t s, bool src0 = false, bool cand = false) {
   const asw_spot_config& c = m->cfg;
   int rc;
   if ((rc = m->encode(pl, *gs, s, src0))) return rc;
@@ -153,7 +153,7 @@
     h = hout;
   }
   m->taps["bottleneck"] = {h, (size_t)rows * d};
-  if ((rc = m->decode(pl, *gs, h, s))) return rc;
+  if ((rc = m->decode(pl, *gs, h, s, cand))) return rc;
   return m->mask_path(pl, h, mean, stdv, out_wave, s);
 }
 
@@ -282,7 +282,7 @@
         return r;
       }
       float* y = out_wave ? out_wave + (size_t)i0 * T : p.ywave;
-      if ((r = run_network(m, p, gs, p.mean, p.stdv, y, q, src0))) return r;
+      if ((r = run_network(m, p, gs, p.mean, p.stdv, y, q, src0, true))) return r;
       if (out_energy && (r = asw_energies(y, B, T, energy_window, nullptr, out_energy + (size_t)i0 * 2, q))) return r;
     }
     return ASW_OK;
@@ -342,6 +342,12 @@
   return ASW_OK;
 }
 
+extern "C" int asw_spot_set_up_fusion(asw_spot* m, int on) {
+  ASW_CHECK_ARG(m, "set_up_fusion: null model handle");
+  m->up_fusion = on != 0;
+  return ASW_OK;
+}
+
 extern "C" int asw_spot_get_tap(asw_spot* m, const char* name, float* dst, size_t capacity, size_t* numel,
                                 void* stream) {
   return get_tap(m, "get_tap", name, dst, capacity, numel, stream);
diff --git a/acousticswarms-speech_amd/native.py b/acousticswarms-speech_amd/native.py
--- a/acousticswarms-speech_amd/native.py
+++ b/acousticswarms-speech_amd/native.py
@@ -137,7 +137,8 @@
                 ("n_layers", c_int32), ("precision", c_int32), ("ln_eps", c_float), ("layer", ResLayerDesc * 3),
                 ("glu_raw", c_void_p), ("glu_mr", c_void_p), ("glu_gamma", c_void_p), ("glu_beta", c_void_p),
                 ("glu_out", c_void_p), ("src_hi", c_void_p), ("src_lo", c_void_p), ("pre_hi", c_void_p), ("pre_lo", c_void_p),
-                ("pre_shift", c_int32)]
+                ("pre_shift", c_int32), ("up_hi", c_void_p), ("up_lo", c_void_p), ("up_shift", c_int32), ("up_bias", c_void_p),
+                ("up_skip", c_void_p), ("up_out", c_void_p), ("up_stats", c_void_p)]
 
 
 RESIDUE_MAX_TAPS = 8
@@ -170,6 +171,7 @@
     "asw_spot_forward": (c_int, [c_void_p, c_void_p, c_int, c_int, c_int, POINTER(c_float), c_void_p, c_void_p]),
     "asw_spot_set_fused_mask": (c_int, [c_void_p, c_int]),
     "asw_spot_set_source_stack": (c_int, [c_void_p, c_int]),
+    "asw_spot_set_up_fusion": (c_int, [c_void_p, c_int]),
     "asw_spot_get_tap": (c_int, [c_void_p, c_char_p, c_void_p, c_size_t, POINTER(c_size_t), c_void_p]),
     "asw_sep_create": (c_int, [POINTER(SepConfigC), POINTER(c_void_p)]),
     "asw_sep_destroy": (None, [c_void_p]),
@@ -209,6 +211,9 @@
     "asw_mask_path_f16x3": (c_int, [POINTER(MaskPathArgs), c_void_p]),
     "asw_mask_path_f16x3_scaled": (c_int, [POINTER(MaskPathArgs), c_void_p]),
     "asw_resstack64_f16x3": (c_int, [POINTER(ResStackArgs), c_void_p]),
+    "asw_resstack_tiles": (c_int, [c_int, c_int, c_int, POINTER(c_int32), c_int]),
+    "asw_up_feed_kperm": (c_int, [c_int]),
+    "asw_pack_up_feed_f16": (c_int, [c_void_p, c_int, c_int, c_void_p, c_void_p, POINTER(c_int32)]),
     "asw_compose_source_weights": (c_int, [c_void_p, c_void_p, c_void_p, c_int, c_int, c_void_p, c_void_p]),
     "asw_convgemm_stats_tiles": (c_int, [c_int, c_int]),
     "asw_f16x3_overflow_count": (c_int, [c_int, POINTER(c_int32)]),
diff --git a/acousticswarms-speech_amd/ops.py b/acousticswarms-speech_amd/ops.py
--- a/acousticswarms-speech_amd/ops.py
+++ b/acousticswarms-speech_amd/ops.py
@@ -89,6 +89,36 @@
     return out
 
 
+def resstack_up(x, layers, up_wt, up_bias, skip, taps=7, eps=1e-5, glu=None):
+    import ctypes
+    src = x if glu is None else glu[0]
+    B, T = src.shape[0], src.shape[1]
+    dev = src.device
+    a = ResStackArgs()
+    a.x = _f32(x).data_ptr() if x is not None else None
+    a.B, a.T, a.C, a.taps, a.n_layers, a.precision, a.ln_eps = B, T, 64, taps, len(layers), 1, eps
+    keep = []
+    for i, (Wt, bias, gamma, beta, dil) in enumerate(layers):
+        fh, fl, sh = pack_fragments_f16(_f32(Wt), 64, taps * 64)
+        keep.append((fh, fl))
+        d = a.layer[i]
+        d.Wf_hi, d.Wf_lo, d.w_shift, d.dil = fh.data_ptr(), fl.data_ptr(), sh, dil
+        d.bias, d.ln_gamma, d.ln_beta = _f32(bias).data_ptr(), _f32(gamma).data_ptr(), _f32(beta).data_ptr()
+    if glu is not None:
+        a.glu_raw, a.glu_mr, a.glu_gamma, a.glu_beta = (_f32(t).data_ptr() for t in glu)
+    dils = (ctypes.c_int32 * 3)(*([l[4] for l in layers] + [1] * (3 - len(layers))))
+    tiles = lib().asw_resstack_tiles(T, taps, len(layers), dils, int(glu is not None))
+    check(min(tiles, 0))
+    uh, ul, ush = pack_fragments_f16(up_wt, 256, 64, up_feed=True)
+    raw = torch.full((B, T, 256), float("nan"), dtype=torch.float32, device=dev)
+    stats = torch.full((B, tiles, 4), float("nan"), dtype=torch.float32, device=dev)
+    a.up_hi, a.up_lo, a.up_shift = uh.data_ptr(), ul.data_ptr(), ush
+    a.up_bias, a.up_skip, a.up_out, a.up_stats = _f32(up_bias).data_ptr(), _f32(skip).data_ptr(), raw.data_ptr(), stats.data_ptr()
+    check(lib().asw_resstack64_f16x3(byref(a), current_stream()))
+    torch.cuda.current_stream().synchronize()
+    return raw, stats
+
+
 def resstack_src(src_hi, src_lo, pre_w, pre_b, layers, taps=7, eps=1e-5, out=None):
     import ctypes
     import numpy as np
@@ -122,15 +152,16 @@
     return out
 
 
-def pack_fragments_f16(Wt, N, K):
+def pack_fragments_f16(Wt, N, K, up_feed=False):
     import ctypes
     import numpy as np
     w = np.ascontiguousarray(Wt.detach().cpu().numpy(), dtype=np.float32).reshape(N, K)
     hi = np.empty(w.size, dtype=np.uint16)
     lo = np.empty(w.size, dtype=np.uint16)
     sh = ctypes.c_int32()
-    check(lib().asw_pack_fragments_f16(ctypes.c_void_p(w.ctypes.data), N, K, ctypes.c_void_p(hi.ctypes.data),
-                                       ctypes.c_void_p(lo.ctypes.data), byref(sh)))
+    pack = lib().asw_pack_up_feed_f16 if up_feed else lib().asw_pack_fragments_f16
+    check(pack(ctypes.c_void_p(w.ctypes.data), N, K, ctypes.c_void_p(hi.ctypes.data),
+               ctypes.c_void_p(lo.ctypes.data), byref(sh)))
     dev = Wt.device
     return (torch.from_numpy(hi.view(np.int16)).to(dev), torch.from_numpy(lo.view(np.int16)).to(dev), sh.value)
 
diff --git a/acousticswarms-speech_amd/spot.py b/acousticswarms-speech_amd/spot.py
--- a/acousticswarms-speech_amd/spot.py
+++ b/acousticswarms-speech_amd/spot.py
@@ -165,3 +165,8 @@
         self._need()
         native.check(native.lib().asw_spot_set_source_stack(self._h, int(bool(on))))
         return self
+
+    def set_up_fusion(self, on: bool = True):
+        self._need()
+        native.check(native.lib().asw_spot_set_up_fusion(self._h, int(bool(on))))
+        return self
diff --git a/include/asw_hip.h b/include/asw_hip.h
--- a/include/asw_hip.h
+++ b/include/asw_hip.h
@@ -68,6 +68,8 @@
 int asw_spot_set_fused_mask(asw_spot* m, int on);
 
 int asw_spot_set_source_stack(asw_spot* m, int on);
+
+int asw_spot_set_up_fusion(asw_spot* m, int on);
 
 int asw_spot_get_tap(asw_spot* m, const char* name, float* dst, size_t capacity, size_t* numel,
                      void* stream);
@@ -236,8 +238,18 @@
   const void* pre_hi;
   const void* pre_lo;
   int32_t pre_shift;
+  const void* up_hi;
+  const void* up_lo;
+  int32_t up_shift;
+  const float* up_bias;
+  const float* up_skip;
+  float* up_out;
+  float* up_stats;
 } asw_resstack_args;
 int asw_resstack64_f16x3(const asw_resstack_args* args, void* stream);
+int asw_resstack_tiles(int T, int taps, int n_layers, const int32_t* dil, int glu);
+int asw_up_feed_kperm(int k);
+int asw_pack_up_feed_f16(const float* Wt, int N, int K, uint16_t* hi, uint16_t* lo, int32_t* w_shift);
 int asw_compose_source_weights(const float* wc, const float* wpre, const float* bpre, int M, int taps, float* comp,
                                float* pre16);
 int asw_split_weights_f16(const float* w, size_t n, uint16_t* hi, uint16_t* lo, int32_t* w_shift);
```

Measured after the change: 2398 candidates/s (median of 6 runs). +1.0%, better.
